# jamesmshihua/DiffusionPolicyOptimization

Measured on NVIDIA B200. Metric: ppo_logprob_update_samples_per_sec, higher is better.
Workload: dtype bf16x3

## Files before the change

diffusionpolicyoptimization_b200/csrc/common.cuh:

```cuda
#pragma once
#include <cuda_runtime.h>
#include <cuda_bf16.h>
#include <stdint.h>
#include <stdio.h>
#include <string.h>
#include <math.h>
#include <string>
#include <vector>
#include "../../include/dppo_b200.h"

void dppo_set_error(const char* fmt, ...);
#define DPPO_FAIL(code, ...) do { dppo_set_error(__VA_ARGS__); return (code); } while (0)
#define CUDA_TRY(expr) do { cudaError_t _e = (expr); if (_e != cudaSuccess) { \
    dppo_set_error("%s failed at %s:%d: %s", #expr, __FILE__, __LINE__, cudaGetErrorString(_e)); return -2; } } while (0)
#define DPPO_TRY(expr) do { int _r = (expr); if (_r != 0) return _r; } while (0)

enum { SCH_BETAS = 0, SCH_ACP, SCH_SQRT_ACP, SCH_SQRT_1M_ACP, SCH_SQRT_RECIP, SCH_SQRT_RECIPM1,
       SCH_LOGVAR, SCH_COEF1, SCH_COEF2, SCH_ROWS };

static inline int round_up(int x, int m) { return (x + m - 1) / m * m; }

__device__ __forceinline__ float softplus_f(float x) {
    return fmaxf(x, 0.f) + log1pf(expf(-fabsf(x)));
}
// ... 36 lines not shown
    c.x = (uint32_t)(a >> 2) | ((uint32_t)slot << 8);
    c.y = (uint32_t)offset;
    c.z = (uint32_t)(uint64_t)row;
    c.w = (uint32_t)((uint64_t)row >> 32);
    Philox4 r = philox4x32_10(c, (uint32_t)seed, (uint32_t)(seed >> 32) + (uint32_t)(offset >> 32));
    uint32_t b0 = (a & 2) ? r.z : r.x, b1 = (a & 2) ? r.w : r.y;
    float u0 = ((float)b0 + 0.5f) * 2.3283064365386963e-10f;
    float u1 = ((float)b1 + 0.5f) * 2.3283064365386963e-10f;
    u0 = fminf(fmaxf(u0, 1.1754944e-38f), 0.99999994f);
    float rad = sqrtf(-2.f * logf(u0));
    float sn, cs;
    sincospif(2.f * u1, &sn, &cs);
    return (a & 1) ? rad * sn : rad * cs;
}
__device__ __forceinline__ void philox_normal4(uint64_t seed, uint64_t offset, int64_t row, int slot, int blk, float (&out)[4]) {
    Philox4 c;
    c.x = (uint32_t)blk | ((uint32_t)slot << 8);
    c.y = (uint32_t)offset;
    c.z = (uint32_t)(uint64_t)row;
    c.w = (uint32_t)((uint64_t)row >> 32);
    Philox4 r = philox4x32_10(c, (uint32_t)seed, (uint32_t)(seed >> 32) + (uint32_t)(offset >> 32));
#pragma unroll
    for (int hlf = 0; hlf < 2; ++hlf) {
        const uint32_t b0 = hlf ? r.z : r.x, b1 = hlf ? r.w : r.y;
        float u0 = ((float)b0 + 0.5f) * 2.3283064365386963e-10f;
        float u1 = ((float)b1 + 0.5f) * 2.3283064365386963e-10f;
        u0 = fminf(fmaxf(u0, 1.1754944e-38f), 0.99999994f);
        float rad = sqrtf(-2.f * logf(u0));
        float sn, cs;
        sincospif(2.f * u1, &sn, &cs);
        out[hlf * 2 + 0] = rad * cs; out[hlf * 2 + 1] = rad * sn;
    }
}
__device__ __forceinline__ uint32_t philox_uint(uint64_t seed, uint64_t offset, int64_t row, int slot) {
    Philox4 c;
    c.x = ((uint32_t)slot << 8);
    c.y = (uint32_t)offset;
    c.z = (uint32_t)(uint64_t)row;
    c.w = (uint32_t)((uint64_t)row >> 32);
    Philox4 r = philox4x32_10(c, (uint32_t)seed, (uint32_t)(seed >> 32) + (uint32_t)(offset >> 32));
    return r.x;
}

struct ActorOff {
    size_t tw1, tb1, tw2, tb2, win, bin, w1, b1, w2, b2, w3, b3, n;
};
struct CriticOff { size_t win, bin, w1, b1, w2, b2, w3, b3, n; };

struct Geom {
    int Do, A, T, K, td, H, Hc, Din, KP, KPc;
    ActorOff ao; CriticOff co;
};

struct ActorDerived {
    float* sinemb;
    float* thpre;
    float* temb;
    float* bt;
    float* w0p;
    float* w23;
    float* b23;
};

struct OptState { float* m; float* v; int64_t step; size_t n; };

struct Workspace {
    char* base = nullptr; size_t cap = 0, used = 0;
};

struct dppo_handle {
    dppo_cfg cfg; int device; Geom g;
    int sm_count;
    float* params;
    float* net_w[4];
    size_t net_n[4];
    ActorDerived ad[4];
    float* sched;
    float  sched_host[SCH_ROWS * 1024];
    OptState opt[2];
    float* grads;
    float* scalars;
    Workspace ws;
    char* pin = nullptr; size_t pin_cap = 0;
    char* dstage = nullptr; size_t dstage_cap = 0;
    cudaStream_t copy_stream = nullptr; cudaEvent_t copy_ev[9];
    void* comm = nullptr; int rank = 0, world = 1;
    float* grads_buf[2] = {nullptr, nullptr}; int grads_cur = 0; float* gsum = nullptr; size_t grads_floats = 0;
    unsigned long long* flags = nullptr;
    float* peer_grads[2][8] = {}; unsigned long long* peer_flags[8] = {}; int peers_attached = 0;
    unsigned long long epoch = 0;
    int* comm_status = nullptr;
    long long peer_timeout_cycles = 0;
    const int* skip_update = nullptr;
    int64_t launches = 0;
    int64_t tc_launches = 0;
    int w0p_dirty[4] = {1, 1, 1, 1};
    int w23_dirty[4] = {1, 1, 1, 1};
    int peer_two_shot = -1;
    float* peer_gsum[8] = {nullptr};
    cudaStream_t aux_stream = nullptr; cudaEvent_t aux_ev[3] = {nullptr, nullptr, nullptr};
    float grad_clip_norm = 0.f;
    int deterministic = 0;
    int chain_dbg_idx = 0;
    long long* chain_dbg = nullptr;
    int64_t fused_launches = 0;
    int cluster_max = -1;
    int last_path = 0;
    int force_path = 0;
    struct TcState* tc = nullptr;
    float* env_norm = nullptr;
    struct TsState* ts = nullptr;
// ... 19 lines not shown
```

diffusionpolicyoptimization_b200/csrc/dppo_api.cu:

```cuda
#include "common.cuh"
#include "simt_kernels.cuh"
#include "sample_cluster.cuh"
#include "tc_path.cuh"
#include "ts_path.cuh"
#include <stdarg.h>
#include <dlfcn.h>
#include <cmath>

static thread_local char g_err[1024] = "";
void dppo_set_error(const char* fmt, ...) {
    va_list ap; va_start(ap, fmt); vsnprintf(g_err, sizeof(g_err), fmt, ap); va_end(ap);
}
extern "C" const char* dppo_last_error(void) { return g_err; }
extern "C" int dppo_abi_version(void) { return DPPO_ABI_VERSION; }
extern "C" size_t dppo_cfg_size(void) { return sizeof(dppo_cfg); }

#define KLAUNCH(h) do { (h)->launches++; } while (0)
#define KCHECK() do { cudaError_t _e = cudaGetLastError(); if (_e != cudaSuccess) { \
    dppo_set_error("kernel launch failed at %s:%d: %s", __FILE__, __LINE__, cudaGetErrorString(_e)); return -3; } } while (0)

extern "C" void dppo_cfg_default(dppo_cfg* c) {
    memset(c, 0, sizeof(*c));
    c->obs_dim = 11; c->action_dim = 3; c->horizon_steps = 4; c->cond_steps = 1;
    c->denoising_steps = 20; c->ft_denoising_steps = 10; c->time_dim = 16;
// ... 194 lines not shown
    h->w0p_dirty[net] = 1; h->w23_dirty[net] = 1;
    if (net != DPPO_NET_CRITIC) {
        ActorDerived& d = h->ad[net];
        int threads = g.H < 64 ? 64 : (g.H > 512 ? 512 : round_up(g.H, 32));
        if (threads < 2 * g.td) threads = round_up(2 * g.td, 32);
        actor_prep_kernel<<<g.T, threads, 4 * g.td * sizeof(float), s>>>(h->net_w[net], g.ao, g.A, g.td, g.H, d.sinemb, d.thpre, d.temb, d.bt);
        KLAUNCH(h); KCHECK();
    }
    if (h->cfg.precision == DPPO_PREC_FP32) DPPO_TRY(ensure_w0p(h, net, s));
    DPPO_TRY(ts_refresh_net(h, net, s));
    return tc_refresh_net(h, net, s);
}

static int dppo_create_impl(const dppo_cfg* cfg, int device, dppo_handle** out, dppo_handle** partial);
extern "C" int dppo_create(const dppo_cfg* cfg, int device, dppo_handle** out) {
    if (!cfg || !out) DPPO_FAIL(-1, "dppo_create: null argument");
    dppo_handle* partial = nullptr;
    const int r = dppo_create_impl(cfg, device, out, &partial);
    if (r != 0 && partial) { std::string msg = dppo_last_error(); dppo_destroy(partial); dppo_set_error("%s", msg.c_str()); }
    return r;
}
static int dppo_create_impl(const dppo_cfg* cfg, int device, dppo_handle** out, dppo_handle** partial) {
    Geom g;
    if (make_geom(cfg, &g)) DPPO_FAIL(-1, "dppo_create: invalid configuration");
    int ndev = 0;
    cudaError_t e = cudaGetDeviceCount(&ndev);
    if (e != cudaSuccess || ndev == 0) DPPO_FAIL(-4, "dppo_create: no CUDA device (%s); this library has no CPU fallback", cudaGetErrorString(e));
    if (device < 0 || device >= ndev) DPPO_FAIL(-1, "dppo_create: device %d out of range (%d devices)", device, ndev);
    CUDA_TRY(cudaSetDevice(device));
    cudaDeviceProp prop; CUDA_TRY(cudaGetDeviceProperties(&prop, device));
    if (prop.major != 10) DPPO_FAIL(-4, "dppo_create: device %d is sm_%d%d; this library is built for sm_100a (B200) only", device, prop.major, prop.minor);
    dppo_handle* h = new dppo_handle();
    *partial = h;
    h->cfg = *cfg; h->device = device; h->g = g; h->sm_count = prop.multiProcessorCount;
    { const char* tv = getenv("DPPO_PEER_TIMEOUT_S"); double sec = tv ? atof(tv) : 600.0; if (!(sec > 0)) sec = 600.0;
      h->peer_timeout_cycles = (long long)(sec * 1e3 * (double)prop.clockRate); }
    { const char* dv = getenv("DPPO_DETERMINISTIC"); h->deterministic = (dv && dv[0] == '1') ? 1 : 0; }
    const size_t nA = g.ao.n, nC = g.co.n;
    const size_t total = 3 * nA + nC;
    CUDA_TRY(cudaMalloc(&h->params, total * sizeof(float)));
    CUDA_TRY(cudaMemset(h->params, 0, total * sizeof(float)));
    h->net_w[DPPO_NET_ACTOR] = h->params; h->net_n[DPPO_NET_ACTOR] = nA;
    h->net_w[DPPO_NET_ACTOR_FT] = h->params + nA; h->net_n[DPPO_NET_ACTOR_FT] = nA;
    h->net_w[DPPO_NET_CRITIC] = h->params + 2 * nA; h->net_n[DPPO_NET_CRITIC] = nC;
    h->net_w[DPPO_NET_ACTOR_EMA] = h->params + 2 * nA + nC; h->net_n[DPPO_NET_ACTOR_EMA] = nA;
    for (int net = 0; net < 4; ++net) {
        ActorDerived& d = h->ad[net];
        memset(&d, 0, sizeof(d));
        if (net == DPPO_NET_CRITIC) { CUDA_TRY(cudaMalloc(&d.w0p, (size_t)g.KPc * g.Hc * sizeof(float))); continue; }
        CUDA_TRY(cudaMalloc(&d.sinemb, (size_t)g.T * g.td * sizeof(float)));
        CUDA_TRY(cudaMalloc(&d.thpre, (size_t)g.T * 2 * g.td * sizeof(float)));
        CUDA_TRY(cudaMalloc(&d.temb, (size_t)g.T * g.td * sizeof(float)));
        CUDA_TRY(cudaMalloc(&d.bt, (size_t)g.T * g.H * sizeof(float)));
        CUDA_TRY(cudaMalloc(&d.w23, (size_t)g.H * g.A * sizeof(float))); CUDA_TRY(cudaMalloc(&d.b23, (size_t)g.A * sizeof(float)));
        CUDA_TRY(cudaMalloc(&d.w0p, (size_t)g.KP * g.H * sizeof(float)));
    }
    DPPO_TRY(dppo_ddpm_schedule(g.T, h->sched_host));
    CUDA_TRY(cudaMalloc(&h->sched, SCH_ROWS * g.T * sizeof(float)));
    CUDA_TRY(cudaMemcpy(h->sched, h->sched_host, SCH_ROWS * g.T * sizeof(float), cudaMemcpyHostToDevice));
    size_t on[2] = {nA, nA + nC};
    for (int i = 0; i < 2; ++i) {
        h->opt[i].n = on[i]; h->opt[i].step = 0;
        CUDA_TRY(cudaMalloc(&h->opt[i].m, on[i] * sizeof(float))); CUDA_TRY(cudaMemset(h->opt[i].m, 0, on[i] * sizeof(float)));
        CUDA_TRY(cudaMalloc(&h->opt[i].v, on[i] * sizeof(float))); CUDA_TRY(cudaMemset(h->opt[i].v, 0, on[i] * sizeof(float)));
    }
    CUDA_TRY(cudaMalloc(&h->grads, (nA + nC + 16) * sizeof(float)));
    CUDA_TRY(cudaMemset(h->grads, 0, (nA + nC + 16) * sizeof(float)));
    h->grads_buf[0] = h->grads; h->grads_floats = nA + nC + 16;
    CUDA_TRY(cudaMalloc(&h->scalars, 64 * sizeof(float)));
    CUDA_TRY(cudaMemset(h->scalars, 0, 64 * sizeof(float)));
    h->comm_status = reinterpret_cast<int*>(h->scalars + 32);
    DPPO_TRY(tc_init(h));
    DPPO_TRY(ts_init(h));
    for (int net = 0; net < 4; ++net) DPPO_TRY(prep_net(h, net, 0));
    CUDA_TRY(cudaDeviceSynchronize());
    *out = h; *partial = nullptr;
    return 0;
}
extern "C" void dppo_destroy(dppo_handle* h) {
    if (!h) return;
    cudaSetDevice(h->device);
    cudaDeviceSynchronize();
    tc_plan_free(h);
    tc_destroy(h);
    ts_destroy(h);
    for (cudaEvent_t e : h->prof_ev) cudaEventDestroy(e);
    if (h->comm) {
        void* lib = dlopen("libnccl.so.2", RTLD_NOW | RTLD_NOLOAD);
        if (lib) { typedef int (*fn_t)(void*); fn_t f = (fn_t)dlsym(lib, "ncclCommDestroy"); if (f) f(h->comm); }
    }
    if (h->peers_attached) {
        for (int p = 0; p < h->world; ++p) if (p != h->rank) {
            cudaIpcCloseMemHandle(h->peer_grads[0][p]); cudaIpcCloseMemHandle(h->peer_grads[1][p]); cudaIpcCloseMemHandle(h->peer_flags[p]);
        }
    }
    cudaFree(h->env_norm);
    cudaFree(h->params); cudaFree(h->sched); cudaFree(h->grads_buf[0]); cudaFree(h->grads_buf[1]);  cudaFree(h->flags); cudaFree(h->scalars);
    for (int i = 0; i < 2; ++i) { cudaFree(h->opt[i].m); cudaFree(h->opt[i].v); }
    for (int net = 0; net < 4; ++net) { ActorDerived& d = h->ad[net]; cudaFree(d.sinemb); cudaFree(d.thpre); cudaFree(d.temb); cudaFree(d.bt); cudaFree(d.w0p); cudaFree(d.w23); cudaFree(d.b23); }
    if (h->ws.base) cudaFree(h->ws.base);
    if (h->copy_stream) { cudaStreamDestroy(h->copy_stream); for (int i = 0; i < 9; ++i) cudaEventDestroy(h->copy_ev[i]); }
    if (h->aux_stream) { cudaStreamDestroy(h->aux_stream); for (int i = 0; i < 3; ++i) if (h->aux_ev[i]) cudaEventDestroy(h->aux_ev[i]); }
    if (h->pin) cudaFreeHost(h->pin);
    if (h->dstage) cudaFree(h->dstage);
    delete h;
}

#define ENTER(h) do { if (!(h)) DPPO_FAIL(-1, "null handle"); CUDA_TRY(cudaSetDevice((h)->device)); } while (0)

extern "C" int dppo_set_weights(dppo_handle* h, int net, const float* src, size_t n, int is_device, dppo_stream_t st) {
    ENTER(h); cudaStream_t s = (cudaStream_t)st;
    if (net < 0 || net > 3 || !src) DPPO_FAIL(-1, "dppo_set_weights: bad net %d", net);
    if (n != h->net_n[net]) DPPO_FAIL(-1, "dppo_set_weights: net %d has %zu parameters, got %zu", net, h->net_n[net], n);
    CUDA_TRY(cudaMemcpyAsync(h->net_w[net], src, n * sizeof(float), is_device ? cudaMemcpyDeviceToDevice : cudaMemcpyHostToDevice, s));
    if (!is_device) CUDA_TRY(cudaStreamSynchronize(s));
    return prep_net(h, net, s);
}
extern "C" int dppo_get_weights(dppo_handle* h, int net, float* dst, size_t n, int is_device, dppo_stream_t st) {
    ENTER(h); cudaStream_t s = (cudaStream_t)st;
    if (net < 0 || net > 3 || !dst) DPPO_FAIL(-1, "dppo_get_weights: bad net %d", net);
    if (n != h->net_n[net]) DPPO_FAIL(-1, "dppo_get_weights: net %d has %zu parameters, got %zu", net, h->net_n[net], n);
    CUDA_TRY(cudaMemcpyAsync(dst, h->net_w[net], n * sizeof(float), is_device ? cudaMemcpyDeviceToDevice : cudaMemcpyDeviceToHost, s));
    if (!is_device) CUDA_TRY(cudaStreamSynchronize(s));
    return 0;
}
extern "C" int dppo_set_opt_state(dppo_handle* h, int opt, const float* m, const float* v, size_t n, int64_t step, int is_device, dppo_stream_t st) {
    ENTER(h); cudaStream_t s = (cudaStream_t)st;
    if (opt < 0 || opt > 1 || n != h->opt[opt].n) DPPO_FAIL(-1, "dppo_set_opt_state: bad slot/size");
    cudaMemcpyKind k = is_device ? cudaMemcpyDeviceToDevice : cudaMemcpyHostToDevice;
    if (m) CUDA_TRY(cudaMemcpyAsync(h->opt[opt].m, m, n * sizeof(float), k, s));
    if (v) CUDA_TRY(cudaMemcpyAsync(h->opt[opt].v, v, n * sizeof(float), k, s));
    h->opt[opt].step = step;
    if (!is_device) CUDA_TRY(cudaStreamSynchronize(s));
    return 0;
}
extern "C" int dppo_get_opt_state(dppo_handle* h, int opt, float* m, float* v, size_t n, int64_t* step, int is_device, dppo_stream_t st) {
    ENTER(h); cudaStream_t s = (cudaStream_t)st;
    if (opt < 0 || opt > 1 || n != h->opt[opt].n) DPPO_FAIL(-1, "dppo_get_opt_state: bad slot/size");
    cudaMemcpyKind k = is_device ? cudaMemcpyDeviceToDevice : cudaMemcpyDeviceToHost;
    if (m) CUDA_TRY(cudaMemcpyAsync(m, h->opt[opt].m, n * sizeof(float), k, s));
    if (v) CUDA_TRY(cudaMemcpyAsync(v, h->opt[opt].v, n * sizeof(float), k, s));
    if (step) *step = h->opt[opt].step;
    if (!is_device) CUDA_TRY(cudaStreamSynchronize(s));
    return 0;
}
extern "C" int dppo_set_ft_denoising_steps(dppo_handle* h, int K) {
    if (!h) DPPO_FAIL(-1, "null handle");
    if (K < 0 || K > h->g.T) DPPO_FAIL(-1, "dppo_set_ft_denoising_steps: K=%d outside [0,%d]", K, h->g.T);
    h->g.K = K; h->cfg.ft_denoising_steps = K;
    return 0;
}
extern "C" int dppo_set_grad_clip_norm(dppo_handle* h, float clip_norm) {
// ... 63 lines not shown
    int rpb = (N + nb - 1) / nb; nb = (N + rpb - 1) / rpb;
    size_t sm = (size_t)nseg * ncols * sizeof(float);
    if (sm > 48 * 1024) {
        if (sm > 200 * 1024) DPPO_FAIL(-1, "colsum: %d segments x %d columns does not fit in shared memory", nseg, ncols);
        CUDA_TRY(cudaFuncSetAttribute(colsum_kernel, cudaFuncAttributeMaxDynamicSharedMemorySize, (int)sm));
    }
    colsum_kernel<<<nb, 256, sm, s>>>(D, ld, N, ncols, seg, nseg, rpb, part); KLAUNCH(h); KCHECK();
    size_t n = (size_t)nseg * ncols;
    tc_reduce_cols_kernel<<<nblk(n, 8), 256, 0, s>>>(part, nb, n, (int)n, out); KLAUNCH(h); KCHECK();
    return 0;
}
static int gemm_dw(dppo_handle* h, cudaStream_t s, const float* X, int ldx, int aop, const float* D, int ldd,
                   int rows, int M, int N, float* part, float* out) {
    int tiles = ((M + 127) / 128) * ((N + (N <= 32 ? 31 : 127)) / (N <= 32 ? 32 : 128));
    int splits = (2 * h->sm_count + tiles - 1) / tiles;
    if (splits > 40) splits = 40;
    int maxs = (rows + 255) / 256; if (splits > maxs) splits = maxs; if (splits < 1) splits = 1;
    GemmP p = gp(X, ldx, D, ldd, part, N, M, N, rows); p.aop = aop; p.cstride = (size_t)M * N;
    int S = gemm(h, s, true, false, p, splits);
    if (S < 0) return -3;
    size_t n = (size_t)M * N;
    reduce_partials_kernel<<<nblk(n, 256), 256, 0, s>>>(part, S, n, n, out, 1.f); KLAUNCH(h); KCHECK();
    return 0;
}
static int mlp_bwd_fp32(dppo_handle* h, cudaStream_t s, const float* w, size_t ow1, size_t ob1, size_t ow2, size_t ob2,
                        size_t ow3, size_t ob3, int act1, const FwdBufs& f, const float* dout, int N, int KP, int H, int NO,
                        const int* seg, int nseg, BwdBufs& b, float* gnet, float* dw0p, float* Gseg) {
    GemmP p = gp(dout, NO, w + ow3, NO, b.dv, H, N, H, NO);
    DPPO_TRY(gemm(h, s, false, true, p) < 0 ? -3 : 0);
    p = gp(b.dv, H, w + ow2, H, b.dh1, H, N, H, H); p.mask = f.h1; p.ldm = H; p.mask_act = act1;
    DPPO_TRY(gemm(h, s, false, true, p) < 0 ? -3 : 0);
    p = gp(b.dh1, H, w + ow1, H, b.du, H, N, H, H); p.mask = f.u; p.ldm = H; p.mask_act = act1; p.add = b.dv; p.ldadd = H;
    DPPO_TRY(gemm(h, s, false, true, p) < 0 ? -3 : 0);
    DPPO_TRY(gemm_dw(h, s, f.v, H, 0, dout, NO, N, H, NO, b.part, gnet + ow3));
    DPPO_TRY(gemm_dw(h, s, f.h1, H, act1, b.dv, H, N, H, H, b.part, gnet + ow2));
    DPPO_TRY(gemm_dw(h, s, f.u, H, act1, b.dh1, H, N, H, H, b.part, gnet + ow1));
    DPPO_TRY(gemm_dw(h, s, f.h0p, KP, 0, b.du, H, N, KP, H, b.part, dw0p));
    DPPO_TRY(colsum(h, s, dout, NO, N, NO, nullptr, 1, b.part, gnet + ob3));
    DPPO_TRY(colsum(h, s, b.dv, H, N, H, nullptr, 1, b.part, gnet + ob2));
    DPPO_TRY(colsum(h, s, b.dh1, H, N, H, nullptr, 1, b.part, gnet + ob1));
    DPPO_TRY(colsum(h, s, b.du, H, N, H, seg, nseg, b.part, Gseg));
    return 0;
}
static void bwd_take(dppo_handle* h, int N, int KP, int H, int nseg, BwdBufs& b, float** Gseg, float** dw0p) {
    b.dv = ws_take<float>(h, (size_t)N * H); b.dh1 = ws_take<float>(h, (size_t)N * H); b.du = ws_take<float>(h, (size_t)N * H);
    size_t colpart = (size_t)320 * (size_t)nseg * H, gemm_part = (size_t)40 * (size_t)H * H;
    b.part_floats = colpart > gemm_part ? colpart : gemm_part;
    b.part = ws_take<float>(h, b.part_floats);
    *Gseg = ws_take<float>(h, (size_t)nseg * H);
    *dw0p = ws_take<float>(h, (size_t)KP * H);
}
static int actor_bwd_fp32(dppo_handle* h, cudaStream_t s, int net, const FwdBufs& f, const float* deps, int N, const int* trow,
                          BwdBufs& b, float* Gseg, float* dw0p, float* gnet) {
    const Geom& g = h->g; const float* w = h->net_w[net]; const ActorDerived& d = h->ad[net];
    DPPO_TRY(mlp_bwd_fp32(h, s, w, g.ao.w1, g.ao.b1, g.ao.w2, g.ao.b2, g.ao.w3, g.ao.b3, h->cfg.actor_act + 1, f, deps, N,
                          g.KP, g.H, g.A, trow, g.T, b, gnet, dw0p, Gseg));
    size_t sm = (size_t)(g.T * g.td * 3) * sizeof(float);
    time_backward_kernel<<<1, 512, sm, s>>>(w, g.ao, g.A, g.td, g.H, g.T, Gseg, d.sinemb, d.thpre, d.temb, gnet); KLAUNCH(h); KCHECK();
    unpack_dw0_kernel<<<nblk((size_t)(g.A + g.Do) * g.H, 256), 256, 0, s>>>(dw0p, g.A, g.td, g.Do, g.H, gnet + g.ao.win); KLAUNCH(h); KCHECK();
    return 0;
}
static int critic_bwd_fp32(dppo_handle* h, cudaStream_t s, const FwdBufs& f, const float* dval, int N,
                           BwdBufs& b, float* Gseg, float* dw0p, float* gnet) {
    const Geom& g = h->g; const float* w = h->net_w[DPPO_NET_CRITIC];
    DPPO_TRY(mlp_bwd_fp32(h, s, w, g.co.w1, g.co.b1, g.co.w2, g.co.b2, g.co.w3, g.co.b3, h->cfg.critic_act + 1, f, dval, N,
                          g.KPc, g.Hc, 1, nullptr, 1, b, gnet, dw0p, Gseg));
    CUDA_TRY(cudaMemcpyAsync(gnet + g.co.bin, Gseg, g.Hc * sizeof(float), cudaMemcpyDeviceToDevice, s));
    unpack_dw0_kernel<<<nblk((size_t)g.Do * g.Hc, 256), 256, 0, s>>>(dw0p, 0, 0, g.Do, g.Hc, gnet + g.co.win); KLAUNCH(h); KCHECK();
    return 0;
}

static const int ROW_CHUNK = 1 << 18;

extern "C" int dppo_actor_forward(dppo_handle* h, int net, const float* x, const int32_t* t, const float* obs,
                                  int N, float* eps, dppo_stream_t st) {
    ENTER(h); cudaStream_t s = (cudaStream_t)st; const Geom& g = h->g;
    if (net < 0 || net > 3 || net == DPPO_NET_CRITIC || !x || !t || !obs || !eps || N < 0) DPPO_FAIL(-1, "dppo_actor_forward: bad arguments");
    for (int r0 = 0; r0 < N; r0 += ROW_CHUNK) {
        int n = N - r0 < ROW_CHUNK ? N - r0 : ROW_CHUNK;
        if (tc_eligible(h, n)) {
            DPPO_TRY(ws_reserve(h, tc_actor_forward_ws(h, n), s));
            DPPO_TRY(tc_actor_forward(h, s, net, x + (size_t)r0 * g.A, obs + (size_t)r0 * g.Do, 1, n, t + r0, 0, eps + (size_t)r0 * g.A));
            continue;
        }
        if (ts_eligible(h, n)) {
            DPPO_TRY(ws_reserve(h, ts_actor_forward_ws(h, n), s));
            DPPO_TRY(ts_actor_forward(h, s, net, x + (size_t)r0 * g.A, obs + (size_t)r0 * g.Do, 1, n, t + r0, 0, eps + (size_t)r0 * g.A));
            continue;
        }
        DPPO_TRY(ws_reserve(h, fwd_ws_bytes(n, g.KP, g.H, g.A), s));
        FwdBufs b; fwd_take(h, n, g.KP, g.H, g.A, b);
        DPPO_TRY(actor_fwd_fp32(h, s, net, x + (size_t)r0 * g.A, obs + (size_t)r0 * g.Do, 1, n, t + r0, 0, b));
        CUDA_TRY(cudaMemcpyAsync(eps + (size_t)r0 * g.A, b.out, (size_t)n * g.A * sizeof(float), cudaMemcpyDeviceToDevice, s));
    }
    return 0;
}
extern "C" int dppo_value(dppo_handle* h, const float* obs, int N, float* v, dppo_stream_t st) {
    ENTER(h); cudaStream_t s = (cudaStream_t)st; const Geom& g = h->g;
    if (!obs || !v || N < 0) DPPO_FAIL(-1, "dppo_value: bad arguments");
    for (int r0 = 0; r0 < N; r0 += ROW_CHUNK) {
        int n = N - r0 < ROW_CHUNK ? N - r0 : ROW_CHUNK;
        if (tc_eligible(h, n)) { DPPO_TRY(tc_value(h, s, obs + (size_t)r0 * g.Do, n, v + r0)); continue; }
        if (ts_eligible(h, n)) { DPPO_TRY(ts_value(h, s, obs + (size_t)r0 * g.Do, n, v + r0)); continue; }
        DPPO_TRY(ws_reserve(h, fwd_ws_bytes(n, g.KPc, g.Hc, 1), s));
        FwdBufs b; fwd_take(h, n, g.KPc, g.Hc, 1, b);
        DPPO_TRY(critic_fwd_fp32(h, s, obs + (size_t)r0 * g.Do, n, b));
        CUDA_TRY(cudaMemcpyAsync(v + r0, b.out, (size_t)n * sizeof(float), cudaMemcpyDeviceToDevice, s));
    }
    return 0;
}

// ... 330 lines not shown
            if (e != cudaSuccess) DPPO_FAIL(-6, "cudaIpcOpenMemHandle(rank %d, buffer %d) failed: %s", p, k, cudaGetErrorString(e));
        }
        h->peer_grads[0][p] = (float*)ptr[0]; h->peer_grads[1][p] = (float*)ptr[1]; h->peer_flags[p] = (unsigned long long*)ptr[2];
        h->peer_gsum[p] = (float*)ptr[1] + gf4;
    }
    h->rank = rank; h->world = world; h->peers_attached = 1;
    if (h->peer_two_shot < 0) { const char* tv = getenv("DPPO_PEER_TWO_SHOT"); h->peer_two_shot = tv ? (tv[0] == '1') : (world >= 4); }
    return 0;
}
static int peer_allreduce_adamw(dppo_handle* h, cudaStream_t s, int opt, float* w, size_t n_param, size_t n_total, float lr, float wd) {
    OptState& o = h->opt[opt];
    o.step += 1;
    const float b1 = h->cfg.adam_beta1, b2 = h->cfg.adam_beta2;
    const float b1p = powf(b1, (float)o.step), b2p = powf(b2, (float)o.step);
    const float alpha = lr * sqrtf(1.f - b2p) / (1.f - b1p);
    PeerPtrs pp; memset(&pp, 0, sizeof(pp));
    for (int p = 0; p < h->world; ++p) { pp.g[p] = h->peer_grads[h->grads_cur][p]; pp.flags[p] = h->peer_flags[p]; }
    h->epoch += 1;
    peer_barrier_kernel<<<1, 32, 0, s>>>(pp, h->flags, h->rank, h->world, h->epoch, h->peer_timeout_cycles, h->comm_status); KLAUNCH(h); KCHECK();
    if (h->peer_two_shot == 1) {
        PeerSums ps; memset(&ps, 0, sizeof(ps));
        for (int p = 0; p < h->world; ++p) ps.s[p] = h->peer_gsum[p];
        const size_t n4 = (n_total + 3) / 4, per = (n4 + h->world - 1) / h->world;
        int grid = (int)((per + 255) / 256); if (grid > 2 * h->sm_count) grid = 2 * h->sm_count; if (grid < 1) grid = 1;
        peer_reduce_scatter_bcast_kernel<<<grid, 256, 0, s>>>(pp, ps, h->rank, h->world, n4, h->comm_status); KLAUNCH(h); KCHECK();
        h->epoch += 1;
        peer_barrier_kernel<<<1, 32, 0, s>>>(pp, h->flags, h->rank, h->world, h->epoch, h->peer_timeout_cycles, h->comm_status); KLAUNCH(h); KCHECK();
        adamw_kernel<<<nblk(n_param, 256), 256, 0, s>>>(w, h->gsum, o.m, o.v, n_param, lr, alpha, b1, b2, h->cfg.adam_eps, wd, h->skip_update, h->comm_status); KLAUNCH(h); KCHECK();
    } else {
        peer_allreduce_adamw_kernel<<<2 * h->sm_count, 256, 0, s>>>(pp, h->world, h->gsum, w, o.m, o.v, n_param, n_total, lr, alpha, b1, b2, h->cfg.adam_eps, wd,
                                                                  h->skip_update, h->comm_status);
        KLAUNCH(h); KCHECK();
    }
    h->grads_cur ^= 1; h->grads = h->grads_buf[h->grads_cur];
    return 0;
}
static int allreduce_sum(dppo_handle* h, float* buf, size_t n, cudaStream_t s) {
    if (h->world <= 1) return 0;
    if (!h->comm || !g_allreduce) DPPO_FAIL(-6, "all-reduce requested but no communicator attached");
    int r = g_allreduce(buf, buf, n, 7 , 0 , h->comm, s);
    if (r) DPPO_FAIL(-6, "ncclAllReduce failed (%d)", r);
    return 0;
}

extern "C" int dppo_comm_status(dppo_handle* h) {
    ENTER(h);
    int st = 0;
    CUDA_TRY(cudaDeviceSynchronize());
    CUDA_TRY(cudaMemcpy(&st, h->comm_status, sizeof(int), cudaMemcpyDeviceToHost));
    if (st) DPPO_FAIL(-6, "peer-memory gradient exchange: a flag barrier timed out; weights and optimizer state were left untouched since");
    return 0;
}

static int adam_apply(dppo_handle* h, cudaStream_t s, int opt, float* w, const float* g, size_t n, float lr, float wd) {
    OptState& o = h->opt[opt];
    o.step += 1;
    const float b1 = h->cfg.adam_beta1, b2 = h->cfg.adam_beta2;
    float b1p = powf(b1, (float)o.step), b2p = powf(b2, (float)o.step);
    float alpha = lr * sqrtf(1.f - b2p) / (1.f - b1p);
    adamw_kernel<<<nblk(n, 256), 256, 0, s>>>(w, g, o.m, o.v, n, lr, alpha, b1, b2, h->cfg.adam_eps, wd, h->skip_update, nullptr); KLAUNCH(h); KCHECK();
    return 0;
}

static int prep_net(dppo_handle* h, int net, cudaStream_t s);
static int ppo_apply_tail(dppo_handle* h, cudaStream_t s, float lr, int apply, float* metrics8, float* grads_out) {
    const size_t nA = h->g.ao.n, nC = h->g.co.n; float* gr = h->grads;
    if (apply) {
        if (h->grad_clip_norm > 0.f) {
            DPPO_TRY(allreduce_sum(h, gr, nA + nC + 8, s));
            if (grads_out) { CUDA_TRY(cudaMemcpyAsync(grads_out, gr, (nA + nC) * sizeof(float), cudaMemcpyDeviceToDevice, s)); grads_out = nullptr; }
            const ActorOff& a = h->g.ao; const CriticOff& c = h->g.co;
            const size_t offs[21] = {a.tw1, a.tb1, a.tw2, a.tb2, a.win, a.bin, a.w1, a.b1, a.w2, a.b2, a.w3, a.b3,
                                     nA + c.win, nA + c.bin, nA + c.w1, nA + c.b1, nA + c.w2, nA + c.b2, nA + c.w3, nA + c.b3, nA + nC};
            VarSegs segs; segs.n = 20;
            for (int i = 0; i <= 20; ++i) segs.off[i] = (unsigned int)offs[i];
            clip_by_norm_kernel<<<segs.n, 1024, 0, s>>>(gr, segs, h->grad_clip_norm); KLAUNCH(h); KCHECK();
            DPPO_TRY(adam_apply(h, s, DPPO_OPT_FINETUNE, h->net_w[DPPO_NET_ACTOR_FT], gr, nA + nC, lr, h->cfg.weight_decay));
        } else if (h->peers_attached && h->world > 1) {
            DPPO_TRY(peer_allreduce_adamw(h, s, DPPO_OPT_FINETUNE, h->net_w[DPPO_NET_ACTOR_FT], nA + nC, nA + nC + 8, lr, h->cfg.weight_decay));
            gr = h->gsum;
        } else {
            DPPO_TRY(allreduce_sum(h, gr, nA + nC + 8, s));
            DPPO_TRY(adam_apply(h, s, DPPO_OPT_FINETUNE, h->net_w[DPPO_NET_ACTOR_FT], gr, nA + nC, lr, h->cfg.weight_decay));
        }
        if (h->cfg.precision == DPPO_PREC_BF16 && tc_shapes_ok(h) && 2 * h->g.td <= 256) {
            DPPO_TRY(tc_prep_pack_ft_critic(h, s));
        } else {
            DPPO_TRY(prep_net(h, DPPO_NET_ACTOR_FT, s));
            DPPO_TRY(prep_net(h, DPPO_NET_CRITIC, s));
        }
    }
    else if (h->world > 1) {
        DPPO_TRY(allreduce_sum(h, gr, nA + nC + 8, s));
    }
    if (metrics8) CUDA_TRY(cudaMemcpyAsync(metrics8, gr + nA + nC, 8 * sizeof(float), cudaMemcpyDeviceToDevice, s));
    if (grads_out) CUDA_TRY(cudaMemcpyAsync(grads_out, gr, (nA + nC) * sizeof(float), cudaMemcpyDeviceToDevice, s));
    return 0;
}
extern "C" int dppo_ppo_step(dppo_handle* h, const float* obs, const float* prev, const float* nxt,
                             const int32_t* inds, const float* returns, const float* oldvalues,
                             const float* advantages, const float* oldlogp, int N, int64_t N_global,
                             float adv_mean, float adv_std, float lr, int apply,
                             float* metrics8, float* grads_out, dppo_stream_t st) {
    ENTER(h); cudaStream_t s = (cudaStream_t)st; const Geom& g = h->g;
    if (!obs || !prev || !nxt || !inds || !returns || !oldvalues || !advantages || !oldlogp || N < 1 || N_global < N)
        DPPO_FAIL(-1, "dppo_ppo_step: bad arguments");
    if (g.K < 1) DPPO_FAIL(-1, "dppo_ppo_step: ft_denoising_steps must be >= 1");
    if (adv_std < 0.f && N_global != N) DPPO_FAIL(-1, "dppo_ppo_step: global advantage statistics are required when rows are sharded");
    const size_t nA = g.ao.n, nC = g.co.n;
    float* gr = h->grads;
    if (tc_eligible(h, N)) {
        DPPO_TRY(tc_ppo_step(h, s, obs, prev, nxt, inds, returns, oldvalues, advantages, oldlogp, N, N_global, adv_mean, adv_std));
    } else if (ts_eligible(h, N)) {
        DPPO_TRY(ts_ppo_step(h, s, obs, prev, nxt, inds, returns, oldvalues, advantages, oldlogp, N, N_global, adv_mean, adv_std));
    } else {
        const int nlb = nblk(N, 128);
        size_t need = fwd_ws_bytes(N, g.KP, g.H, g.A) + fwd_ws_bytes(N, g.KPc, g.Hc, 1)
                    + bwd_ws_bytes(h, N, g.KP, g.H, g.A, g.T) + bwd_ws_bytes(h, N, g.KPc, g.Hc, 1, 1)
                    + ws_bytes(N, 4) + ws_bytes((size_t)N * g.A, 4) + ws_bytes(N, 4) + ws_bytes((size_t)nlb * 5, 8);
        DPPO_TRY(ws_reserve(h, need, s));
        FwdBufs fa, fc; fwd_take(h, N, g.KP, g.H, g.A, fa); fwd_take(h, N, g.KPc, g.Hc, 1, fc);
        BwdBufs ba, bc; float *Ga, *Gc, *dw0a, *dw0c;
        bwd_take(h, N, g.KP, g.H, g.T, ba, &Ga, &dw0a); bwd_take(h, N, g.KPc, g.Hc, 1, bc, &Gc, &dw0c);
        int* trow = ws_take<int>(h, N);
        float* deps = ws_take<float>(h, (size_t)N * g.A);
        float* dval = ws_take<float>(h, N);
        double* bsum = ws_take<double>(h, (size_t)nlb * 5);

        make_trow_kernel<<<nblk(N, 256), 256, 0, s>>>(inds, N, g.K, 0, trow); KLAUNCH(h); KCHECK();
        if (adv_std < 0.f) { adv_stats_kernel<<<1, 1024, 0, s>>>(advantages, N, h->scalars); KLAUNCH(h); KCHECK(); }
        else { set_scalars_kernel<<<1, 1, 0, s>>>(h->scalars, adv_mean, adv_std); KLAUNCH(h); KCHECK(); }
        DPPO_TRY(actor_fwd_fp32(h, s, DPPO_NET_ACTOR_FT, prev, obs, 1, N, trow, 0, fa));
        DPPO_TRY(critic_fwd_fp32(h, s, obs, N, fc));
        PpoHyper hp;
        hp.A = g.A; hp.Da = h->cfg.action_dim; hp.K = g.K; hp.T = g.T; hp.reward_horizon = h->cfg.reward_horizon; hp.norm_adv = h->cfg.norm_adv;
        hp.dcv = h->cfg.denoised_clip_value; hp.min_lp_std = h->cfg.min_logprob_denoising_std;
        hp.lp_lo = h->cfg.logprob_clip_lo; hp.lp_hi = h->cfg.logprob_clip_hi; hp.gamma_d = h->cfg.gamma_denoising;
        hp.clip_coef = h->cfg.clip_ploss_coef; hp.clip_base = h->cfg.clip_ploss_coef_base; hp.clip_rate = h->cfg.clip_ploss_coef_rate;
// ... 347 lines not shown
```

diffusionpolicyoptimization_b200/csrc/simt_kernels.cuh:

```cuda
#pragma once
#include "common.cuh"

struct GemmP {
    const float* A; int lda;
    const float* B; int ldb;
    float* C; int ldc;
    int M, N, K;
    int kchunk; size_t cstride;
    int vecA, vecB, vecC;
    int aop;
    const float* bias;
    const float* btab; int ldbt;
    const int* trow; int tconst;
    const float* mask; int ldm; int mask_act;
    const float* add; int ldadd;
};

template <bool A_KM, bool B_NK, int BN>
__global__ void __launch_bounds__(256, 2) sgemm_kernel(const GemmP p) {
    constexpr int BM = 128, BK = 16, TN = BN / 16;
    __shared__ __align__(16) float As[2][BK][BM + 4];
    __shared__ __align__(16) float Bs[2][BK][BN + 4];

    const int tid = threadIdx.x, tx = tid & 15, ty = tid >> 4;
// ... 141 lines not shown
            }
#pragma unroll
            for (int i = 0; i < 8; ++i)
#pragma unroll
                for (int j = 0; j < TN; ++j) acc[i][j] = fmaf(a[i], b[j], acc[i][j]);
        }
        if (kt + 1 < nk) { store_a(buf ^ 1); store_b(buf ^ 1); }
        __syncthreads();
    }

#pragma unroll
    for (int i = 0; i < 8; ++i) {
        const int m = m0 + (i < 4 ? ty * 4 + i : 64 + ty * 4 + (i - 4));
        if (m >= p.M) continue;
        const float* btrow = nullptr;
        if (p.btab) { int t = p.trow ? p.trow[m] : p.tconst; btrow = p.btab + (size_t)t * p.ldbt; }
#pragma unroll
        for (int jb = 0; jb < TN; jb += (TN == 8 ? 4 : 2)) {
            constexpr int W = (TN == 8 ? 4 : 2);
            const int n = n0 + (TN == 8 ? (jb < 4 ? tx * 4 : 64 + tx * 4) : tx * 2);
            float v[W];
#pragma unroll
            for (int e = 0; e < W; ++e) {
                float x = acc[i][jb + e];
                int nn = n + e;
                if (nn < p.N) {
                    if (p.bias) x += p.bias[nn];
                    if (btrow) x += btrow[nn];
                    if (p.mask) x *= act_grad_rt(p.mask[(size_t)m * p.ldm + nn], p.mask_act);
                    if (p.add) x += p.add[(size_t)m * p.ldadd + nn];
                }
                v[e] = x;
            }
            float* dst = C + (size_t)m * p.ldc + n;
            if (W == 4 && p.vecC && n + 3 < p.N) {
                *reinterpret_cast<float4*>(dst) = make_float4(v[0], v[1], v[2], v[3]);
            } else {
#pragma unroll
                for (int e = 0; e < W; ++e) if (n + e < p.N) dst[e] = v[e];
            }
        }
    }
}

__global__ void reduce_partials_kernel(const float* __restrict__ part, int S, size_t stride, size_t n,
                                       float* __restrict__ out, float scale) {
    size_t i = (size_t)blockIdx.x * blockDim.x + threadIdx.x;
    if (i >= n) return;
    float s = 0.f;
    for (int k = 0; k < S; ++k) s += part[(size_t)k * stride + i];
    out[i] = s * scale;
}

__device__ __forceinline__ void actor_prep_body(const int t, float* sm, const float* __restrict__ w, ActorOff o, int A, int td, int H,
                                  float* __restrict__ sinemb, float* __restrict__ thpre,
                                  float* __restrict__ temb, float* __restrict__ bt, __nv_bfloat16* __restrict__ bt16) {
    float* se = sm;
    float* hp = se + td;
    float* te = hp + 2 * td;
    const int tid = threadIdx.x;
    const int half = td / 2;
    if (tid < td) {
        int i = tid % half;
        float f = expf((float)i * -(logf(10000.f) / (float)(half - 1)));
        float e = (float)t * f;
        float v = tid < half ? sinf(e) : cosf(e);
        se[tid] = v; sinemb[t * td + tid] = v;
    }
    __syncthreads();
    if (tid < 2 * td) {
        float s = w[o.tb1 + tid];
        for (int j = 0; j < td; ++j) s = fmaf(se[j], w[o.tw1 + (size_t)j * 2 * td + tid], s);
        thpre[t * 2 * td + tid] = s;
        hp[tid] = mish_f(s);
    }
    __syncthreads();
    if (tid < td) {
        float s = w[o.tb2 + tid];
        for (int j = 0; j < 2 * td; ++j) s = fmaf(hp[j], w[o.tw2 + (size_t)j * td + tid], s);
        te[tid] = s; temb[t * td + tid] = s;
    }
    __syncthreads();
    for (int c = tid; c < H; c += blockDim.x) {
        float s = w[o.bin + c];
        for (int j = 0; j < td; ++j) s = fmaf(te[j], w[o.win + (size_t)(A + j) * H + c], s);
        bt[(size_t)t * H + c] = s;
        if (bt16) bt16[(size_t)t * H + c] = __float2bfloat16(s);
    }
}
__global__ void actor_prep_kernel(const float* __restrict__ w, ActorOff o, int A, int td, int H,
                                  float* __restrict__ sinemb, float* __restrict__ thpre,
                                  float* __restrict__ temb, float* __restrict__ bt) {
    extern __shared__ float sm[];
    actor_prep_body(blockIdx.x, sm, w, o, A, td, H, sinemb, thpre, temb, bt, nullptr);
}
__global__ void fold_output_kernel(const float* __restrict__ w2, const float* __restrict__ b2, const float* __restrict__ w3, const float* __restrict__ b3,
                                   int H, int A, float* __restrict__ w23, float* __restrict__ b23) {
    const int i = blockIdx.x * blockDim.x + threadIdx.x;
    if (i >= (H + 1) * A) return;
    const int k = i / A, a = i % A;
    const float* row = k < H ? w2 + (size_t)k * H : b2;
    double acc = k < H ? 0.0 : (double)b3[a];
    for (int j = 0; j < H; ++j) acc += (double)row[j] * (double)w3[(size_t)j * A + a];
    if (k < H) w23[(size_t)k * A + a] = (float)acc; else b23[a] = (float)acc;
}
__global__ void pack_w0_kernel(const float* __restrict__ win, int A, int skip, int Do, int KP, int H,
                               float* __restrict__ w0p) {
    int i = blockIdx.x * blockDim.x + threadIdx.x;
    if (i >= KP * H) return;
    int k = i / H, c = i % H;
    float v = 0.f;
    if (k < A) v = win[(size_t)k * H + c];
    else if (k < A + Do) v = win[(size_t)(k + skip) * H + c];
    w0p[i] = v;
}
__global__ void pack_h0_kernel(const float* __restrict__ x, const float* __restrict__ obs, int N, int A, int Do,
                               int KP, int obs_div, float* __restrict__ h0p) {
    size_t i = (size_t)blockIdx.x * blockDim.x + threadIdx.x;
    if (i >= (size_t)N * KP) return;
    int r = (int)(i / KP), k = (int)(i % KP);
    float v = 0.f;
    if (k < A) v = x[(size_t)r * A + k];
    else if (k < A + Do) v = obs[(size_t)(r / obs_div) * Do + (k - A)];
    h0p[i] = v;
}
__global__ void make_trow_kernel(const int* __restrict__ inds, int N, int K, int mode, int* __restrict__ trow) {
    int r = blockIdx.x * blockDim.x + threadIdx.x;
    if (r >= N) return;
    trow[r] = mode == 0 ? (K - 1 - inds[r]) : (K - 1 - (r % K));
}

struct SampleHyper {
    float dcv, rcv, facv, min_std; int deterministic;
};
struct StepConst { float sr, srm1, c1, c2, sd; };
__device__ __forceinline__ StepConst step_const(const float* __restrict__ sch, int T, int t) {
    StepConst c;
    c.sr = sch[SCH_SQRT_RECIP * T + t]; c.srm1 = sch[SCH_SQRT_RECIPM1 * T + t];
    c.c1 = sch[SCH_COEF1 * T + t]; c.c2 = sch[SCH_COEF2 * T + t];
    c.sd = expf(0.5f * sch[SCH_LOGVAR * T + t]);
    return c;
}
__device__ __forceinline__ float sample_std(const StepConst& c, int t, const SampleHyper& hp) {
    if (hp.deterministic) return (t == 0) ? 0.f : fminf(fmaxf(c.sd, 1e-3f), 1e6f);
    return fminf(fmaxf(c.sd, hp.min_std), 1e6f);
}
__device__ __forceinline__ float ddpm_step_elem_c(float x, float eps, float noise, const StepConst& c, float sd, const SampleHyper& hp, bool last) {
// ... 236 lines not shown
    }
}

__global__ void pretrain_prep_kernel(const float* __restrict__ x0, const int* __restrict__ t_in, const float* __restrict__ noise_in,
                                     int N, int A, int T, const float* __restrict__ sch, uint64_t seed, uint64_t offset,
                                     int64_t row_offset, int* __restrict__ trow, float* __restrict__ noise, float* __restrict__ xn) {
    size_t i = (size_t)blockIdx.x * blockDim.x + threadIdx.x;
    if (i >= (size_t)N * A) return;
    int r = (int)(i / A), a = (int)(i % A);
    int t = t_in ? t_in[r] : (int)(((uint64_t)philox_uint(seed, offset, row_offset + r, 255) * (uint64_t)T) >> 32);
    float nz = noise_in ? noise_in[i] : philox_normal(seed, offset, row_offset + r, 0, a);
    if (a == 0) trow[r] = t;
    noise[i] = nz;
    xn[i] = sch[SCH_SQRT_ACP * T + t] * x0[i] + sch[SCH_SQRT_1M_ACP * T + t] * nz;
}
__global__ void __launch_bounds__(256) mse_loss_kernel(const float* __restrict__ eps, const float* __restrict__ noise, size_t n,
                                                       float scale, float* __restrict__ deps, double* __restrict__ block_sums) {
    size_t i = (size_t)blockIdx.x * blockDim.x + threadIdx.x;
    double a = 0;
    if (i < n) { float d = eps[i] - noise[i]; deps[i] = 2.f * d * scale; a = (double)d * d; }
    __shared__ double red[256];
    red[threadIdx.x] = a;
    __syncthreads();
    for (int o = 128; o > 0; o >>= 1) { if (threadIdx.x < o) red[threadIdx.x] += red[threadIdx.x + o]; __syncthreads(); }
    if (threadIdx.x == 0) block_sums[blockIdx.x] = red[0];
}
__global__ void sum_blocks_kernel(const double* __restrict__ block_sums, int nblocks, float scale, float* __restrict__ dst) {
    __shared__ double red[256];
    double a = 0;
    for (int b = threadIdx.x; b < nblocks; b += blockDim.x) a += block_sums[b];
    red[threadIdx.x] = a;
    __syncthreads();
    for (int o = 128; o > 0; o >>= 1) { if (threadIdx.x < o) red[threadIdx.x] += red[threadIdx.x + o]; __syncthreads(); }
    if (threadIdx.x == 0) dst[0] = (float)(red[0] * scale);
}

__global__ void __launch_bounds__(256) colsum_kernel(const float* __restrict__ D, int ld, int N, int ncols,
                                                     const int* __restrict__ seg, int nseg, int rows_per_block,
                                                     float* __restrict__ part) {
    extern __shared__ float sm[];
    for (int i = threadIdx.x; i < nseg * ncols; i += blockDim.x) sm[i] = 0.f;
    __syncthreads();
    const int r0 = blockIdx.x * rows_per_block, r1 = min(N, r0 + rows_per_block);
    for (int c = threadIdx.x; c < ncols; c += blockDim.x) {
        for (int r = r0; r < r1; ++r) {
            int s = seg ? seg[r] : 0;
            sm[s * ncols + c] += D[(size_t)r * ld + c];
        }
    }
    __syncthreads();
    for (int i = threadIdx.x; i < nseg * ncols; i += blockDim.x) part[(size_t)blockIdx.x * nseg * ncols + i] = sm[i];
}

__device__ __forceinline__ void time_backward_body(const int bid, const int nblk, float* sm, const bool staged,
                                     const float* __restrict__ w, ActorOff o, int A, int td, int H, int T,
                                     const float* __restrict__ G, const float* __restrict__ sinemb,
                                     const float* __restrict__ thpre, const float* __restrict__ temb,
                                     float* __restrict__ g) {
    float* dte = sm;
    float* dh = dte + T * td;
    const int tid = threadIdx.x, nt = blockDim.x;
    if (nblk == 1 || bid > 0) {
        const int c0 = nblk == 1 ? 0 : (bid - 1) * 128, c1 = nblk == 1 ? H : min(H, c0 + 128);
        const int lanes = nblk == 1 ? 1 : 4;
        for (int i = tid; i < (c1 - c0) * lanes; i += nt) {
            const int c = c0 + i / lanes, part = i % lanes;
            float bsum = 0.f;
            float acc[16];
#pragma unroll
            for (int q = 0; q < 16; ++q) acc[q] = 0.f;
            for (int t0 = 0; t0 < T; t0 += 32) {
                float gc[32];
#pragma unroll
                for (int q = 0; q < 32; ++q) gc[q] = (t0 + q < T) ? G[(size_t)(t0 + q) * H + c] : 0.f;
#pragma unroll
                for (int q = 0; q < 32; ++q) bsum += gc[q];
#pragma unroll
                for (int jj = 0; jj < 16; ++jj) {
                    const int j = part + jj * lanes;
                    if (j < td) {
#pragma unroll
                        for (int q = 0; q < 32; ++q) if (t0 + q < T) acc[jj] = fmaf(temb[(t0 + q) * td + j], gc[q], acc[jj]);
                    }
                }
            }
            if (part == 0) g[o.bin + c] = bsum;
            for (int jj = 0; jj < 16; ++jj) {
                const int j = part + jj * lanes;
                if (j < td) g[o.win + (size_t)(A + j) * H + c] = acc[jj];
            }
            for (int j = part + 16 * lanes; j < td; j += lanes) {
                float a = 0.f;
                for (int t = 0; t < T; ++t) a = fmaf(temb[t * td + j], G[(size_t)t * H + c], a);
                g[o.win + (size_t)(A + j) * H + c] = a;
            }
        }
        if (nblk > 1) return;
    }
    if (staged) {
        float* sG = dh + T * 2 * td;
        float* sW = sG + T * H;
        for (int i = tid; i < T * H; i += nt) sG[i] = G[i];
        for (int i = tid; i < td * H; i += nt) sW[i] = w[o.win + (size_t)A * H + i];
        __syncthreads();
        const int lane = tid & 31;
        for (int p = tid >> 5; p < T * td; p += nt >> 5) {
            const int t = p / td, j = p % td;
            float s = 0.f;
            for (int c = lane; c < H; c += 32) s = fmaf(sW[j * H + c], sG[t * H + c], s);
#pragma unroll
            for (int off = 16; off > 0; off >>= 1) s += __shfl_xor_sync(0xffffffffu, s, off);
            if (lane == 0) dte[t * td + j] = s;
        }
    } else
    for (int j = tid >> 5; j < td; j += nt >> 5) {
        const int lane = tid & 31;
        float wr[32];
#pragma unroll
        for (int q = 0; q < 32; ++q) { const int c = lane + q * 32; wr[q] = c < H ? w[o.win + (size_t)(A + j) * H + c] : 0.f; }
        for (int t = 0; t < T; ++t) {
            float s = 0.f;
#pragma unroll
            for (int q = 0; q < 32; ++q) { const int c = lane + q * 32; if (c < H) s = fmaf(wr[q], G[(size_t)t * H + c], s); }
#pragma unroll
            for (int off = 16; off > 0; off >>= 1) s += __shfl_xor_sync(0xffffffffu, s, off);
            if (lane == 0) dte[t * td + j] = s;
        }
    }
    __syncthreads();
    for (int i = tid; i < T * 2 * td; i += nt) {
        int t = i / (2 * td), k = i % (2 * td);
        float s = 0.f;
        for (int j = 0; j < td; ++j) s = fmaf(w[o.tw2 + (size_t)k * td + j], dte[t * td + j], s);
        dh[i] = s * mish_grad_f(thpre[i]);
    }
    __syncthreads();
    for (int i = tid; i < 2 * td * td; i += nt) {
        int k = i / td, j = i % td;
        float s = 0.f;
        for (int t = 0; t < T; ++t) s = fmaf(mish_f(thpre[t * 2 * td + k]), dte[t * td + j], s);
        g[o.tw2 + i] = s;
        int ss = i / (2 * td), kk = i % (2 * td);
        float a = 0.f;
        for (int t = 0; t < T; ++t) a = fmaf(sinemb[t * td + ss], dh[t * 2 * td + kk], a);
        g[o.tw1 + i] = a;
    }
    for (int j = tid; j < td; j += nt) { float s = 0.f; for (int t = 0; t < T; ++t) s += dte[t * td + j]; g[o.tb2 + j] = s; }
    for (int k = tid; k < 2 * td; k += nt) { float s = 0.f; for (int t = 0; t < T; ++t) s += dh[t * 2 * td + k]; g[o.tb1 + k] = s; }
}
__global__ void __launch_bounds__(512) time_backward_kernel(const float* __restrict__ w, ActorOff o, int A, int td, int H, int T,
                                     const float* __restrict__ G, const float* __restrict__ sinemb,
                                     const float* __restrict__ thpre, const float* __restrict__ temb,
                                     float* __restrict__ g) {
    extern __shared__ float sm[];
    time_backward_body(blockIdx.x, gridDim.x, sm, false, w, o, A, td, H, T, G, sinemb, thpre, temb, g);
}
__device__ __forceinline__ void unpack_dw0_body(const int bid, const float* __restrict__ dw0p, int A, int skip, int Do, int H, float* __restrict__ gwin) {
    int i = bid * blockDim.x + threadIdx.x;
    if (i >= (A + Do) * H) return;
    int k = i / H, c = i % H;
    gwin[(size_t)(k < A ? k : k + skip) * H + c] = dw0p[i];
}
__global__ void unpack_dw0_kernel(const float* __restrict__ dw0p, int A, int skip, int Do, int H, float* __restrict__ gwin) {
    unpack_dw0_body(blockIdx.x, dw0p, A, skip, Do, H, gwin);
}

__global__ void adamw_kernel(float* __restrict__ w, const float* __restrict__ g, float* __restrict__ m, float* __restrict__ v,
                             size_t n, float lr, float alpha, float b1, float b2, float eps, float wd,
                             const int* __restrict__ skip0 = nullptr, const int* __restrict__ skip1 = nullptr) {
    size_t i = (size_t)blockIdx.x * blockDim.x + threadIdx.x;
    if (i >= n) return;
    if ((skip0 && *skip0) || (skip1 && *skip1)) return;
    float p = w[i], gi = g[i], mi = m[i], vi = v[i];
    if (wd != 0.f) p = p - p * (wd * lr);
    mi = mi + (gi - mi) * (1.f - b1);
    vi = vi + (gi * gi - vi) * (1.f - b2);
    p = p - mi * alpha / (sqrtf(vi) + eps);
    w[i] = p; m[i] = mi; v[i] = vi;
}
struct VarSegs { unsigned int off[24]; int n; };
__global__ void __launch_bounds__(1024) clip_by_norm_kernel(float* __restrict__ g, VarSegs segs, float clip) {
    const unsigned int b = segs.off[blockIdx.x], e = segs.off[blockIdx.x + 1];
    float acc = 0.f;
    for (unsigned int i = b + threadIdx.x; i < e; i += blockDim.x) { const float x = g[i]; acc = fmaf(x, x, acc); }
    __shared__ float part[32];
    __shared__ float denom;
    for (int o = 16; o; o >>= 1) acc += __shfl_xor_sync(0xffffffffu, acc, o);
    if ((threadIdx.x & 31) == 0) part[threadIdx.x >> 5] = acc;
    __syncthreads();
    if (threadIdx.x < 32) {
        float t = threadIdx.x < (blockDim.x >> 5) ? part[threadIdx.x] : 0.f;
        for (int o = 16; o; o >>= 1) t += __shfl_xor_sync(0xffffffffu, t, o);
        if (threadIdx.x == 0) denom = fmaxf(sqrtf(t > 0.f ? t : 1.f), clip);
    }
    __syncthreads();
    const float d = denom;
    if (d == clip) return;
    for (unsigned int i = b + threadIdx.x; i < e; i += blockDim.x) g[i] = g[i] * clip / d;
}
struct PeerPtrs { const float* g[8]; unsigned long long* flags[8]; };
__global__ void peer_barrier_kernel(PeerPtrs pp, unsigned long long* my_flags, int rank, int world, unsigned long long epoch,
                                    long long timeout_cycles, int* __restrict__ status) {
    const int p = threadIdx.x;
    if (p >= world) return;
    if (*((volatile int*)status)) return;
    __threadfence_system();
    *((volatile unsigned long long*)(pp.flags[p] + rank)) = epoch;
    const long long t0 = clock64();
    while (*((volatile unsigned long long*)(my_flags + p)) < epoch) {
        if (clock64() - t0 > timeout_cycles) {
            printf("peer barrier timed out: rank %d waiting for rank %d (epoch %llu)\n", rank, p, epoch);
            atomicExch(status, 1);
            break;
        }
        __nanosleep(64);
    }
    __threadfence_system();
}
__global__ void __launch_bounds__(256) peer_allreduce_adamw_kernel(PeerPtrs pp, int world, float* __restrict__ g_sum, float* __restrict__ w,
                                                                  float* __restrict__ m, float* __restrict__ v, size_t n_param, size_t n_total,
                                                                  float lr, float alpha, float b1, float b2, float eps, float wd,
                                                                  const int* __restrict__ skip0 = nullptr, const int* __restrict__ skip1 = nullptr) {
    const bool no_update = (skip0 && *skip0) || (skip1 && *skip1);
    if (skip1 && *skip1) return;
    const size_t n4 = n_total / 4;
    for (size_t i = (size_t)blockIdx.x * blockDim.x + threadIdx.x; i < n4 + (n_total & 3); i += (size_t)gridDim.x * blockDim.x) {
        float s[4] = {0.f, 0.f, 0.f, 0.f};
        const bool vec = i < n4;
        const size_t e0 = vec ? i * 4 : n4 * 4 + (i - n4);
        const int cnt = vec ? 4 : 1;
// ... 36 lines not shown
```

diffusionpolicyoptimization_b200/csrc/tc_path.cuh:

```cuda
#pragma once
#include "common.cuh"
#include "simt_kernels.cuh"
#include "tc_gemm.cuh"
#include "fused_chain.cuh"
#include "tc_dw_pair.cuh"

typedef __nv_bfloat16 bf16;

struct TcNetW {
    bf16 *w2w0, *w1, *w3t, *w3p;
    bf16 *w1t, *w2t;
    float* bias2;
    int H;
};
struct TcPpoPlan;
struct TcState {
    TcNetW net[4];
    int KP0;
    TcPpoPlan* plan;
};

__device__ __forceinline__ void tc_pack_actor_body(const size_t i0, const size_t stride, const float* __restrict__ w, ActorOff o, int A, int td, int Do, int T, int H, int KP0,
                                     const float* __restrict__ bt, bf16* __restrict__ w2w0, bf16* __restrict__ w1,
                                     bf16* __restrict__ w3t, bf16* __restrict__ w3p, bf16* __restrict__ w1t, bf16* __restrict__ w2t) {
// ... 6 lines not shown
        int k = (int)(i / H), c = (int)(i % H);
        float v = 0.f;
        if (k < A) v = w[o.win + (size_t)k * H + c];
        else if (k < A + Do) v = w[o.win + (size_t)(k + td) * H + c];
        else if (k < A + Do + T) { if (!bt) continue; v = bt[(size_t)(k - A - Do) * H + c]; }
        w2w0[(size_t)H * H + i] = __float2bfloat16(v);
    }
    for (size_t i = i0; i < (size_t)64 * H; i += stride) {
        int a = (int)(i / H), k = (int)(i % H);
        w3t[i] = __float2bfloat16(a < A ? w[o.w3 + (size_t)k * A + a] : 0.f);
    }
    for (size_t i = i0; i < (size_t)H * 128; i += stride) {
        int k = (int)(i / 128), a = (int)(i % 128);
        w3p[i] = __float2bfloat16(a < A ? w[o.w3 + (size_t)k * A + a] : 0.f);
    }
}
__global__ void tc_pack_actor_kernel(const float* __restrict__ w, ActorOff o, int A, int td, int Do, int T, int H, int KP0,
                                     const float* __restrict__ bt, bf16* __restrict__ w2w0, bf16* __restrict__ w1,
                                     bf16* __restrict__ w3t, bf16* __restrict__ w3p, bf16* __restrict__ w1t, bf16* __restrict__ w2t) {
    tc_pack_actor_body((size_t)blockIdx.x * blockDim.x + threadIdx.x, (size_t)gridDim.x * blockDim.x, w, o, A, td, Do, T, H, KP0, bt, w2w0, w1, w3t, w3p, w1t, w2t);
}
__device__ __forceinline__ void tc_pack_critic_body(const size_t i0, const size_t stride, const float* __restrict__ w, CriticOff o, int A, int Do, int Hc, int KP0,
                                      bf16* __restrict__ w2w0, bf16* __restrict__ w1, bf16* __restrict__ w3t,
                                      bf16* __restrict__ w3p, float* __restrict__ bias2, bf16* __restrict__ w1t, bf16* __restrict__ w2t) {
    for (size_t i = i0; i < (size_t)Hc * Hc; i += stride) {
        w2w0[i] = __float2bfloat16(w[o.w2 + i]); w1[i] = __float2bfloat16(w[o.w1 + i]);
        const size_t r = i / Hc, c = i % Hc;
        w1t[i] = __float2bfloat16(w[o.w1 + c * Hc + r]); w2t[i] = __float2bfloat16(w[o.w2 + c * Hc + r]);
    }
    for (size_t i = i0; i < (size_t)KP0 * Hc; i += stride) {
        int k = (int)(i / Hc), c = (int)(i % Hc);
        float v = (k >= A && k < A + Do) ? w[o.win + (size_t)(k - A) * Hc + c] : 0.f;
        w2w0[(size_t)Hc * Hc + i] = __float2bfloat16(v);
    }
    for (size_t i = i0; i < (size_t)64 * Hc; i += stride) { int a = (int)(i / Hc), k = (int)(i % Hc); w3t[i] = __float2bfloat16(a == 0 ? w[o.w3 + k] : 0.f); }
    for (size_t i = i0; i < (size_t)Hc * 128; i += stride) { int k = (int)(i / 128), a = (int)(i % 128); w3p[i] = __float2bfloat16(a == 0 ? w[o.w3 + k] : 0.f); }
    for (size_t i = i0; i < (size_t)Hc; i += stride) bias2[i] = w[o.b2 + i] + w[o.bin + i];
}
__global__ void tc_pack_critic_kernel(const float* __restrict__ w, CriticOff o, int A, int Do, int Hc, int KP0,
                                      bf16* __restrict__ w2w0, bf16* __restrict__ w1, bf16* __restrict__ w3t,
                                      bf16* __restrict__ w3p, float* __restrict__ bias2, bf16* __restrict__ w1t, bf16* __restrict__ w2t) {
    tc_pack_critic_body((size_t)blockIdx.x * blockDim.x + threadIdx.x, (size_t)gridDim.x * blockDim.x, w, o, A, Do, Hc, KP0, w2w0, w1, w3t, w3p, bias2, w1t, w2t);
}
struct TcPrepPackArgs {
    const float* wa; ActorOff ao; const float* wc; CriticOff co; int A, td, Do, T, H, Hc, KP0, na, nc;
    float* sinemb; float* thpre; float* temb; float* bt;
    bf16 *a_w2w0, *a_w1, *a_w3t, *a_w3p, *a_w1t, *a_w2t;
    bf16 *c_w2w0, *c_w1, *c_w3t, *c_w3p, *c_w1t, *c_w2t; float* c_bias2;
};
__global__ void __launch_bounds__(256) tc_prep_pack_kernel(const TcPrepPackArgs a) {
    extern __shared__ float prep_sm[];
    const int b = blockIdx.x;
    if (b < a.T)
        actor_prep_body(b, prep_sm, a.wa, a.ao, a.A, a.td, a.H, a.sinemb, a.thpre, a.temb, a.bt, a.a_w2w0 + (size_t)a.H * a.H + (size_t)(a.A + a.Do) * a.H);
    else if (b < a.T + a.na)
        tc_pack_actor_body((size_t)(b - a.T) * blockDim.x + threadIdx.x, (size_t)a.na * blockDim.x, a.wa, a.ao, a.A, a.td, a.Do, a.T, a.H, a.KP0, nullptr,
                           a.a_w2w0, a.a_w1, a.a_w3t, a.a_w3p, a.a_w1t, a.a_w2t);
    else
        tc_pack_critic_body((size_t)(b - a.T - a.na) * blockDim.x + threadIdx.x, (size_t)a.nc * blockDim.x, a.wc, a.co, a.A, a.Do, a.Hc, a.KP0,
                            a.c_w2w0, a.c_w1, a.c_w3t, a.c_w3p, a.c_bias2, a.c_w1t, a.c_w2t);
}
struct TcIdxView {
    const int* flat; int K; long long P;
    const float *chains, *obs, *olp, *ret, *val, *adv;
    int* bad;
};
__global__ void tc_pack_h0_kernel(const float* __restrict__ x, const float* __restrict__ obs, const int* __restrict__ trow, int tconst,
                                  int N, int A, int Do, int T, int KP0, int obs_div, bf16* __restrict__ h0, int chainK = 0,
                                  const int* __restrict__ flat = nullptr, int flatK = 1, long long flatP = 0, int* __restrict__ bad = nullptr) {
    const int g8 = KP0 / 8;
    size_t i = (size_t)blockIdx.x * blockDim.x + threadIdx.x;
    if (i >= (size_t)N * g8) return;
    const int r = (int)(i / g8), k0 = (int)(i % g8) * 8;
    int t = trow ? (tconst < 0 ? -tconst - 1 - trow[r] : trow[r]) : tconst;
    size_t xrow = chainK > 0 ? (size_t)(r / chainK) * (chainK + 1) + (r % chainK) : (size_t)r;
    size_t orow = (size_t)(r / obs_div);
    if (flat) {
        int f = flat[r];
        if (f < 0 || (long long)f >= flatP * flatK) { if (bad && k0 == 0) atomicOr(bad, 1); f = 0; }
        const int b = f / flatK, k = f % flatK;
        xrow = (size_t)b * (flatK + 1) + k; orow = (size_t)b; t = flatK - 1 - k;
    }
    __align__(16) bf16 o[8];
#pragma unroll
    for (int j = 0; j < 8; ++j) {
        const int k = k0 + j;
        float v = 0.f;
        if (k < A) v = x ? x[xrow * A + k] : 0.f;
        else if (k < A + Do) v = obs[orow * Do + (k - A)];
        else if (k < A + Do + T) v = (k - A - Do == t) ? 1.f : 0.f;
        else if (k == A + Do + T) v = 1.f;
        o[j] = __float2bfloat16(v);
    }
    *reinterpret_cast<uint4*>(h0 + (size_t)r * KP0 + k0) = *reinterpret_cast<const uint4*>(o);
}
__global__ void tc_pad64_kernel(const float* __restrict__ src, int N, int ncols, bf16* __restrict__ dst) {
    size_t i = (size_t)blockIdx.x * blockDim.x + threadIdx.x;
    if (i >= (size_t)N * 8) return;
    const int r = (int)(i >> 3), k0 = (int)(i & 7) * 8;
    __align__(16) bf16 o[8];
#pragma unroll
    for (int j = 0; j < 8; ++j) o[j] = __float2bfloat16(k0 + j < ncols ? src[(size_t)r * ncols + k0 + j] : 0.f);
    *reinterpret_cast<uint4*>(dst + (size_t)r * 64 + k0) = *reinterpret_cast<const uint4*>(o);
}
__global__ void __launch_bounds__(256) tc_colsum_kernel(const bf16* __restrict__ D, int N, int ncols, int rows_per_block, float* __restrict__ part) {
    __shared__ float2 red[256];
    const int tpr = ncols / 2, groups = 256 / tpr;
// ... 22 lines not shown
    if (i >= (size_t)rows * cols) return;
    const int r = (int)(i / cols), c = (int)(i % cols);
    float s = 0.f;
    for (int k = 0; k < S; ++k) s += part[(size_t)k * stride + (size_t)r * ld_in + c];
    out[(size_t)r * ld_out + c] = s;
}

__device__ __forceinline__ void tc_reduce_cols_body(const int bid, const float* __restrict__ part, int nb, size_t stride, int ncols,
                                                    float* __restrict__ out, int split, float* __restrict__ out2) {
    const int c = bid * (blockDim.x >> 5) + (threadIdx.x >> 5), lane = threadIdx.x & 31;
    if (c >= ncols) return;
    float s = 0.f;
    for (int b = lane; b < nb; b += 32) s += part[(size_t)b * stride + c];
#pragma unroll
    for (int o = 16; o > 0; o >>= 1) s += __shfl_xor_sync(0xffffffffu, s, o);
    if (lane == 0) { if (out2 && c >= split) out2[c - split] = s; else out[c] = s; }
}
__device__ __forceinline__ void tc_reduce_cols_wide_body(const int bid, const float* __restrict__ part, int nb, size_t stride, int ncols,
                                                         float* __restrict__ out, int split, float* __restrict__ out2) {
    __shared__ float red[16][33];
    const int lane = threadIdx.x & 31, rg = threadIdx.x >> 5, c = bid * 32 + lane;
    float sacc[8];
#pragma unroll
    for (int q = 0; q < 8; ++q) sacc[q] = 0.f;
    if (c < ncols) {
        int b = rg;
        for (; b + 112 < nb; b += 128) {
#pragma unroll
            for (int q = 0; q < 8; ++q) sacc[q] += part[(size_t)(b + 16 * q) * stride + c];
        }
        for (; b < nb; b += 16) sacc[0] += part[(size_t)b * stride + c];
    }
    red[rg][lane] = ((sacc[0] + sacc[1]) + (sacc[2] + sacc[3])) + ((sacc[4] + sacc[5]) + (sacc[6] + sacc[7]));
    __syncthreads();
    if (rg == 0 && c < ncols) {
        float s = 0.f;
#pragma unroll
        for (int g = 0; g < 16; ++g) s += red[g][lane];
        if (out2 && c >= split) out2[c - split] = s; else out[c] = s;
    }
}
__global__ void __launch_bounds__(256) tc_reduce_cols_kernel(const float* __restrict__ part, int nb, size_t stride, int ncols, float* __restrict__ out,
                                                             int split = 0, float* __restrict__ out2 = nullptr) {
    tc_reduce_cols_body(blockIdx.x, part, nb, stride, ncols, out, split, out2);
}

struct TcTailArgs {
    int first[9];
    const double* bsum; int blocks_done; float inv_nglobal, frac_local; float* metrics;
    int wide, wide3;
    const float* colb3; int ncol3; float* b3a; int split3; float* b3c;
    const float* cpa; int rows_a; int HA; float* b2a; float* b1a;
    const float* cpc; int rows_c; int HC; float* b2c; float* b1c;
    const float* w; ActorOff ao; int A, td, T, Do; int tb_staged; const float* Gt; const float* sinemb; const float* thpre; const float* temb; float* gr;
    const float* dw0a; float* gwin_a; const float* dw0c_obs; float* gwin_c; const float* dw0c_bias; float* gbin_c;
};
__global__ void __launch_bounds__(512) tc_ppo_tail_kernel(const TcTailArgs a) {
    extern __shared__ float tail_sm[];
    const int b = blockIdx.x;
    if (b < a.first[1]) ppo_metrics_body(a.bsum, a.blocks_done, a.inv_nglobal, a.frac_local, a.metrics);
    else if (b < a.first[2]) {
        if (a.wide3) tc_reduce_cols_wide_body(b - a.first[1], a.colb3, a.blocks_done, (size_t)a.ncol3, a.ncol3, a.b3a, a.split3, a.b3c);
        else tc_reduce_cols_body(b - a.first[1], a.colb3, a.blocks_done, (size_t)a.ncol3, a.ncol3, a.b3a, a.split3, a.b3c);
    }
    else if (b < a.first[3]) {
        if (a.wide) tc_reduce_cols_wide_body(b - a.first[2], a.cpa, a.rows_a, (size_t)2 * a.HA, 2 * a.HA, a.b2a, a.HA, a.b1a);
        else tc_reduce_cols_body(b - a.first[2], a.cpa, a.rows_a, (size_t)2 * a.HA, 2 * a.HA, a.b2a, a.HA, a.b1a);
    } else if (b < a.first[4]) {
        if (a.wide) tc_reduce_cols_wide_body(b - a.first[3], a.cpc, a.rows_c, (size_t)2 * a.HC, 2 * a.HC, a.b2c, a.HC, a.b1c);
        else tc_reduce_cols_body(b - a.first[3], a.cpc, a.rows_c, (size_t)2 * a.HC, 2 * a.HC, a.b2c, a.HC, a.b1c);
    }
    else if (b < a.first[5]) time_backward_body(b - a.first[4], a.first[5] - a.first[4], tail_sm, a.tb_staged != 0, a.w, a.ao, a.A, a.td, a.HA, a.T,
                                                a.Gt, a.sinemb, a.thpre, a.temb, a.gr);
    else if (b < a.first[6]) unpack_dw0_body(b - a.first[5], a.dw0a, a.A, a.td, a.Do, a.HA, a.gwin_a);
    else if (b < a.first[7]) unpack_dw0_body(b - a.first[6], a.dw0c_obs, 0, 0, a.Do, a.HC, a.gwin_c);
    else { const int i = (b - a.first[7]) * blockDim.x + threadIdx.x; if (i < a.HC) a.gbin_c[i] = a.dw0c_bias[i]; }
}

__global__ void __launch_bounds__(128) tc_ppo_loss_kernel(
    const float* __restrict__ prev, const float* __restrict__ nxt, const float* __restrict__ eps,
    const int* __restrict__ inds, const float* __restrict__ returns, const float* __restrict__ oldvalues,
    const float* __restrict__ advantages, const float* __restrict__ oldlogp, const float* __restrict__ newvalues,
    const float* __restrict__ advstats, const float* __restrict__ sch, PpoHyper hp, int N,
    bf16* __restrict__ depsb, bf16* __restrict__ dvalb, double* __restrict__ block_sums, float* __restrict__ col_part ) {
    const int r = blockIdx.x * blockDim.x + threadIdx.x;
    const int A = hp.A;
    double acc[5] = {0, 0, 0, 0, 0};
    float gout[32];
#pragma unroll
    for (int a = 0; a < 32; ++a) gout[a] = 0.f;
    float dv_out = 0.f;
    if (r < N) {
        const int ind = inds[r], t = hp.K - 1 - ind;
        const int nuse = min(hp.reward_horizon, A / hp.Da) * hp.Da;
        const StepConst sc = step_const(sch, hp.T, t);
        const float sd = logprob_std(sc, hp.min_lp_std);
        const float lgs = 0.91893853320467274f + logf(sd);
        float newm = 0.f, oldm = 0.f;
        float zs[32]; uint32_t live = 0u;
#pragma unroll
        for (int a = 0; a < 32; ++a) {
            zs[a] = 0.f;
            if (a < nuse) {
                const size_t i = (size_t)r * A + a;
                float z; bool in;
                const float lp = logprob_elem_c(prev[i], eps[i], nxt[i], sc, sd, lgs, hp.dcv, &z, &in);
                newm += fminf(fmaxf(lp, hp.lp_lo), hp.lp_hi);
                oldm += fminf(fmaxf(oldlogp[i], hp.lp_lo), hp.lp_hi);
                zs[a] = z;
                if (lp >= hp.lp_lo && lp <= hp.lp_hi && in) live |= 1u << a;
            }
        }
        newm /= (float)nuse; oldm /= (float)nuse;
        float adv = advantages[r];
        if (hp.norm_adv) adv = (adv - advstats[0]) / (advstats[1] + 1e-8f);
        adv *= powf(hp.gamma_d, (float)(hp.K - ind - 1));
        const float logratio = newm - oldm, ratio = expf(logratio);
        const float tt = hp.K > 1 ? (float)ind / (float)(hp.K - 1) : (float)ind;
        const float clipc = hp.K > 1 ? hp.clip_base + (hp.clip_coef - hp.clip_base) * (expf(hp.clip_rate * tt) - 1.f) / (expf(hp.clip_rate) - 1.f) : tt;
        const float rc = fminf(fmaxf(ratio, 1.f - clipc), 1.f + clipc);
        const float pg1 = -adv * ratio, pg2 = -adv * rc;
        const float pg = fmaxf(pg1, pg2);
        const float dpg = (pg1 >= pg2) ? -adv : ((ratio >= 1.f - clipc && ratio <= 1.f + clipc) ? -adv : 0.f);
        const float gscale = dpg * ratio * hp.inv_nglobal / (float)nuse / sd * sc.c1 * (-sc.srm1);
#pragma unroll
        for (int a = 0; a < 32; ++a) gout[a] = ((live >> a) & 1u) ? gscale * zs[a] : 0.f;
// ... 548 lines not shown
    m.W = &h->tc->net[DPPO_NET_CRITIC]; m.H = g.Hc; m.NO = 1; m.act1 = h->cfg.critic_act + 1; m.KP0 = h->tc->KP0;
    m.fused = fc_critic_ok(h) ? 1 : 0; m.net = DPPO_NET_CRITIC; m.din = g.Do; m.cpart = nullptr;
    m.b0 = w + g.co.bin; m.b1 = w + g.co.b1; m.b2 = m.W->bias2; m.b3 = w + g.co.b3;
}

static int tc_actor_forward(dppo_handle* h, cudaStream_t s, int net, const float* x, const float* obs, int obs_div, int N,
                            const int* trow, int tconst, float* eps) {
    const Geom& g = h->g; const int KP0 = h->tc->KP0;
    if (fc_ok(h)) {
        const size_t need = h->ws.used + ws_bytes((size_t)N * KP0, 2);
        if (need > h->ws.cap) DPPO_FAIL(-7, "tc_actor_forward: workspace too small (%zu > %zu)", need, h->ws.cap);
        const size_t mark = h->ws.used;
        bf16* h0 = ws_take<bf16>(h, (size_t)N * KP0);
        tc_pack_h0_kernel<<<tc_nblk((size_t)N * (KP0 / 8), 256), 256, 0, s>>>(x, obs, trow, tconst, N, g.A, g.Do, g.T, KP0, obs_div, h0);
        TC_KCHECK(h);
        int r = fc_actor_infer(h, s, net, h0, N, fc::FINAL_EPS, eps, nullptr, nullptr, nullptr, nullptr);
        h->ws.used = mark;
        return r;
    }
    const size_t need = h->ws.used + ws_bytes((size_t)N * KP0, 2) + tc_mlp_ws_bytes(N, g.H, h->cfg.actor_act == DPPO_ACT_MISH, false);
    if (need > h->ws.cap) DPPO_FAIL(-7, "tc_actor_forward: workspace too small (%zu > %zu)", need, h->ws.cap);
    const size_t mark = h->ws.used;
    TcMlp m; tc_actor_mlp(h, net, m);
    bf16* h0 = ws_take<bf16>(h, (size_t)N * KP0);
    tc_mlp_take(h, N, m, false);
    m.h0 = h0; m.out = eps;
    tc_pack_h0_kernel<<<tc_nblk((size_t)N * (KP0 / 8), 256), 256, 0, s>>>(x, obs, trow, tconst, N, g.A, g.Do, g.T, KP0, obs_div, h0);
    TC_KCHECK(h);
    int r = tc_mlp_forward(h, s, m, N);
    h->ws.used = mark;
    return r;
}
static size_t tc_actor_forward_ws(const dppo_handle* h, int N) {
    return ws_bytes((size_t)N * h->tc->KP0, 2) + tc_mlp_ws_bytes(N, h->g.H, h->cfg.actor_act == DPPO_ACT_MISH, false);
}
static int tc_value(dppo_handle* h, cudaStream_t s, const float* obs, int N, float* v) {
    const Geom& g = h->g; const int KP0 = h->tc->KP0;
    DPPO_TRY(ws_reserve(h, ws_bytes((size_t)N * KP0, 2) + tc_mlp_ws_bytes(N, g.Hc, h->cfg.critic_act == DPPO_ACT_MISH, false), s));
    TcMlp m; tc_critic_mlp(h, m);
    bf16* h0 = ws_take<bf16>(h, (size_t)N * KP0);
    tc_mlp_take(h, N, m, false);
    m.h0 = h0; m.out = v;
    tc_pack_h0_kernel<<<tc_nblk((size_t)N * (KP0 / 8), 256), 256, 0, s>>>(nullptr, obs, nullptr, -1, N, g.A, g.Do, g.T, KP0, 1, h0);
    TC_KCHECK(h);
    if (fc_critic_ok(h)) return fc_infer(h, s, fc_critic_net(h), h0, N, fc::FINAL_EPS, v, nullptr, nullptr, nullptr, nullptr);
    return tc_mlp_forward(h, s, m, N);
}

static int colsum(dppo_handle* h, cudaStream_t s, const float* D, int ld, int N, int ncols, const int* seg, int nseg,
                  float* part, float* out);

static int tc_actor_grads(dppo_handle* h, cudaStream_t s, int net, const TcMlp& m, const float* deps, const bf16* depsb, int N,
                          float* part, float* dw0, float* gnet) {
    const Geom& g = h->g; const float* w = h->net_w[net]; const ActorDerived& d = h->ad[net];
    DPPO_TRY(tc_mlp_backward(h, s, m, depsb, N, part, gnet, g.ao.w1, g.ao.b1, g.ao.w2, g.ao.b2, g.ao.w3, dw0));
    if (deps) DPPO_TRY(colsum(h, s, deps, g.A, N, g.A, nullptr, 1, part, gnet + g.ao.b3));
    const size_t sm = (size_t)(g.T * g.td * 3) * sizeof(float);
    time_backward_kernel<<<1, 512, sm, s>>>(w, g.ao, g.A, g.td, g.H, g.T, dw0 + (size_t)(g.A + g.Do) * g.H, d.sinemb, d.thpre, d.temb, gnet);
    TC_KCHECK(h);
    unpack_dw0_kernel<<<tc_nblk((size_t)(g.A + g.Do) * g.H, 256), 256, 0, s>>>(dw0, g.A, g.td, g.Do, g.H, gnet + g.ao.win);
    TC_KCHECK(h);
    return 0;
}
static int tc_critic_grads(dppo_handle* h, cudaStream_t s, const TcMlp& m, const float* dval, const bf16* dvalb, int N,
                           float* part, float* dw0, float* gnet) {
    const Geom& g = h->g;
    DPPO_TRY(tc_mlp_backward(h, s, m, dvalb, N, part, gnet, g.co.w1, g.co.b1, g.co.w2, g.co.b2, g.co.w3, dw0));
    if (dval) DPPO_TRY(colsum(h, s, dval, 1, N, 1, nullptr, 1, part, gnet + g.co.b3));
    unpack_dw0_kernel<<<tc_nblk((size_t)g.Do * g.Hc, 256), 256, 0, s>>>(dw0 + (size_t)g.A * g.Hc, 0, 0, g.Do, g.Hc, gnet + g.co.win);
    TC_KCHECK(h);
    CUDA_TRY(cudaMemcpyAsync(gnet + g.co.bin, dw0 + (size_t)(g.A + g.Do + g.T) * g.Hc, g.Hc * sizeof(float), cudaMemcpyDeviceToDevice, s));
    return 0;
}

struct TcPpoPlan {
    int N, nchunks, chunk_rows, lead_rows, blocks_done, max_blocks;
    int full_rows, rows_done, dw_done, dw_flush_chunk;
    TcIdxView idx;
    int64_t N_global;
    float *part, *dw0a, *dw0c, *colb3, *cpa, *cpc;
    double* bsum;
    TcMlp ma, mc;
    bf16 *h0, *depsb, *dvalb; float *eps, *val;
    PpoHyper hp;
};
static TcPpoPlan& tc_plan(dppo_handle* h) { if (!h->tc->plan) { h->tc->plan = new TcPpoPlan(); memset(h->tc->plan, 0, sizeof(TcPpoPlan)); } return *h->tc->plan; }
static void tc_plan_free(dppo_handle* h) { if (h->tc && h->tc->plan) { delete h->tc->plan; h->tc->plan = nullptr; } }

static int tc_ppo_begin(dppo_handle* h, cudaStream_t s, int N, int chunk_rows, int64_t N_global, int lead_rows = 0) {
    const Geom& g = h->g; const int KP0 = h->tc->KP0;
    const size_t nA = g.ao.n, nC = g.co.n;
    TcPpoPlan& P = tc_plan(h);
    if (h->deterministic || chunk_rows <= 0 || chunk_rows >= N) chunk_rows = N;
    chunk_rows = round_up(chunk_rows, 128);
    if (lead_rows <= 0 || lead_rows >= chunk_rows || chunk_rows >= N) lead_rows = 0;
    const int nchunks = lead_rows ? 1 + (N - lead_rows + chunk_rows - 1) / chunk_rows : (N + chunk_rows - 1) / chunk_rows;
    P.N = N; P.nchunks = nchunks; P.N_global = N_global; P.blocks_done = 0;
    memset(&P.idx, 0, sizeof(P.idx));
    P.chunk_rows = chunk_rows; P.lead_rows = lead_rows;
    P.full_rows = nchunks > 1 ? 1 : 0; P.rows_done = 0; P.dw_done = 0; P.dw_flush_chunk = nchunks / 2 - 1;
    const int NC = P.full_rows ? N : (P.chunk_rows < N ? P.chunk_rows : N);
    P.max_blocks = tc_nblk(N, LOSS8_ROWS) + nchunks;
    const bool amish = h->cfg.actor_act == DPPO_ACT_MISH, cmish = h->cfg.critic_act == DPPO_ACT_MISH;
    const size_t pf = tc_part_floats(h, g.H);
    const size_t n_cpa = (size_t)nchunks * h->sm_count * 2 * g.H, n_cpc = (size_t)nchunks * h->sm_count * 2 * g.Hc;
    size_t need = ws_bytes((size_t)NC * KP0, 2) + tc_mlp_ws_bytes(NC, g.H, amish, true) + tc_mlp_ws_bytes(NC, g.Hc, cmish, true)
                + ws_bytes((size_t)NC * g.A, 4) + ws_bytes(NC, 4) + 2 * ws_bytes((size_t)NC * 64, 2)
                + ws_bytes(pf, 4) + ws_bytes((size_t)KP0 * g.H, 4) + ws_bytes((size_t)KP0 * g.Hc, 4)
                + ws_bytes((size_t)P.max_blocks * 5, 8) + ws_bytes((size_t)P.max_blocks * (g.A + 1), 4) + ws_bytes(n_cpa, 4) + ws_bytes(n_cpc, 4);
    DPPO_TRY(ws_reserve(h, need, s));
    tc_actor_mlp(h, DPPO_NET_ACTOR_FT, P.ma); tc_critic_mlp(h, P.mc);
// ... 73 lines not shown
    else
        tc_pack_h0_kernel<<<tc_nblk((size_t)n * (KP0 / 8), 256), 256, 0, s>>>(prev, obs, inds, -g.K, n, g.A, g.Do, g.T, KP0, 1, P.h0 + r0 * KP0);
    TC_KCHECK(h);
    const bool overlap = defer && !h->prof_on;
    if (overlap && !h->aux_stream) {
        CUDA_TRY(cudaStreamCreateWithFlags(&h->aux_stream, cudaStreamNonBlocking));
        for (int i = 0; i < 2; ++i) CUDA_TRY(cudaEventCreateWithFlags(&h->aux_ev[i], cudaEventDisableTiming));
    }
    auto fork = [&]() -> int { CUDA_TRY(cudaEventRecord(h->aux_ev[0], s)); CUDA_TRY(cudaStreamWaitEvent(h->aux_stream, h->aux_ev[0], 0)); return 0; };
    auto join = [&]() -> int { CUDA_TRY(cudaEventRecord(h->aux_ev[1], h->aux_stream)); CUDA_TRY(cudaStreamWaitEvent(s, h->aux_ev[1], 0)); return 0; };
    if (overlap) DPPO_TRY(fork());
    DPPO_TRY(tc_mlp_forward(h, s, ma, n));
    DPPO_TRY(tc_mlp_forward(h, overlap ? h->aux_stream : s, mc, n));
    if (overlap) DPPO_TRY(join());
    if (loss8)
        tc_ppo_loss8_kernel<<<nlb, 256, 0, s>>>(prev, nxt, ma.out, inds, returns, oldvalues, advantages, oldlogp, mc.out,
                                               h->scalars, h->sched, P.hp, n, depsb, dvalb, P.bsum + (size_t)P.blocks_done * 5,
                                               P.colb3 + (size_t)P.blocks_done * (g.A + 1), iv);
    else
        tc_ppo_loss_kernel<<<nlb, 128, 0, s>>>(prev, nxt, ma.out, inds, returns, oldvalues, advantages, oldlogp, mc.out,
                                              h->scalars, h->sched, P.hp, n, depsb, dvalb, P.bsum + (size_t)P.blocks_done * 5,
                                              P.colb3 + (size_t)P.blocks_done * (g.A + 1));
    TC_KCHECK(h);
    P.blocks_done += nlb;
    if (defer) {
        if (overlap) DPPO_TRY(fork());
        DPPO_TRY(tc_mlp_backward_dx(h, s, ma, depsb, n, P.part, h->grads, g.ao.b1, g.ao.b2));
        DPPO_TRY(tc_mlp_backward_dx(h, overlap ? h->aux_stream : s, mc, dvalb, n, P.part, h->grads + nA, g.co.b1, g.co.b2));
        if (overlap) DPPO_TRY(join());
        P.rows_done += n;
        if (P.full_rows && chunk != P.dw_flush_chunk && P.rows_done < P.N) return 0;
        const size_t d0 = P.full_rows ? (size_t)P.dw_done : r0;
        const int dn = (int)((P.full_rows ? (size_t)P.rows_done : r0 + (size_t)n) - d0);
        const TcMlp da = tc_mlp_at(P.ma, d0), dc = tc_mlp_at(P.mc, d0);
        const bf16* const dd = P.depsb + d0 * 64; const bf16* const dvd = P.dvalb + d0 * 64;
        P.dw_done = P.rows_done;
        tcp::PairDesc pd[10];
        tc_mlp_dw_pair_descs(da, dd, dn, h->grads, g.ao.w1, g.ao.w2, g.ao.w3, P.dw0a, pd);
        tc_mlp_dw_pair_descs(dc, dvd, dn, h->grads + nA, g.co.w1, g.co.w2, g.co.w3, P.dw0c, pd + 5);
        return tcp::launch_group_pair(h, s, pd, 10, dn);
    }
    DPPO_TRY(tc_mlp_backward(h, s, ma, depsb, n, P.part, h->grads, g.ao.w1, g.ao.b1, g.ao.w2, g.ao.b2, g.ao.w3, P.dw0a));
    DPPO_TRY(tc_mlp_backward(h, s, mc, dvalb, n, P.part, h->grads + nA, g.co.w1, g.co.b1, g.co.w2, g.co.b2, g.co.w3, P.dw0c));
    P.rows_done += n;
    return 0;
}
static int tc_launch_tail(dppo_handle* h, cudaStream_t s, const double* bsum, int blocks_done, float inv_nglobal, float frac_local, const float* colb3,
                          const float* cpa, int rows_a, const float* cpc, int rows_c, const float* dw0a, const float* dw0c,
                          float* b2a_out = nullptr, float* b2c_out = nullptr) {
    const Geom& g = h->g;
    const size_t nA = g.ao.n, nC = g.co.n;
    float* gr = h->grads;
    const float* w = h->net_w[DPPO_NET_ACTOR_FT]; const ActorDerived& d = h->ad[DPPO_NET_ACTOR_FT];
    const size_t sm = (size_t)(g.T * g.td * 3) * sizeof(float);
    const size_t sm_staged = sm + (size_t)(g.T + g.td) * g.H * sizeof(float);
    const bool staged = sm_staged <= 160 * 1024;
    static bool attr_set_dev[64] = {};
    bool& attr_set = attr_set_dev[h->device & 63];
    if (!attr_set) { CUDA_TRY(cudaFuncSetAttribute(tc_ppo_tail_kernel, cudaFuncAttributeMaxDynamicSharedMemorySize, 160 * 1024)); attr_set = true; }
    TcTailArgs a;
    const int nthr = 512, wpb = nthr / 32;
    const bool wide = rows_a >= 256;
    const int cpb = wide ? 32 : wpb;
    const bool wide3 = blocks_done >= 256;
    a.wide = wide ? 1 : 0; a.wide3 = wide3 ? 1 : 0;
    const int nb[8] = {1, tc_nblk(g.A + 1, wide3 ? 32 : wpb), tc_nblk(2 * g.H, cpb), tc_nblk(2 * g.Hc, cpb), 1 + (g.H + 127) / 128,
                       tc_nblk((size_t)(g.A + g.Do) * g.H, nthr), tc_nblk((size_t)g.Do * g.Hc, nthr), tc_nblk(g.Hc, nthr)};
    a.first[0] = 0;
    for (int r = 0; r < 8; ++r) a.first[r + 1] = a.first[r] + nb[r];
    a.bsum = bsum; a.blocks_done = blocks_done; a.inv_nglobal = inv_nglobal; a.frac_local = frac_local; a.metrics = gr + nA + nC;
    a.colb3 = colb3; a.ncol3 = g.A + 1; a.b3a = gr + g.ao.b3; a.split3 = g.A; a.b3c = gr + nA + g.co.b3;
    a.cpa = cpa; a.rows_a = rows_a; a.HA = g.H; a.b2a = b2a_out ? b2a_out : gr + g.ao.b2; a.b1a = gr + g.ao.b1;
    a.cpc = cpc; a.rows_c = rows_c; a.HC = g.Hc; a.b2c = b2c_out ? b2c_out : gr + nA + g.co.b2; a.b1c = gr + nA + g.co.b1;
    a.w = w; a.ao = g.ao; a.A = g.A; a.td = g.td; a.T = g.T; a.Do = g.Do; a.tb_staged = staged ? 1 : 0;
    a.Gt = dw0a + (size_t)(g.A + g.Do) * g.H; a.sinemb = d.sinemb; a.thpre = d.thpre; a.temb = d.temb; a.gr = gr;
    a.dw0a = dw0a; a.gwin_a = gr + g.ao.win; a.dw0c_obs = dw0c + (size_t)g.A * g.Hc; a.gwin_c = gr + nA + g.co.win;
    a.dw0c_bias = dw0c + (size_t)(g.A + g.Do + g.T) * g.Hc; a.gbin_c = gr + nA + g.co.bin;
    tc_ppo_tail_kernel<<<a.first[8], nthr, staged ? sm_staged : sm, s>>>(a); TC_KCHECK(h);
    return 0;
}
static int tc_ppo_finish(dppo_handle* h, cudaStream_t s) {
    const Geom& g = h->g;
    const size_t nA = g.ao.n, nC = g.co.n;
    TcPpoPlan& P = tc_plan(h);
    float* gr = h->grads;
    const bool defer = P.ma.fused && P.mc.fused && !h->deterministic;
    const float* w = h->net_w[DPPO_NET_ACTOR_FT]; const ActorDerived& d = h->ad[DPPO_NET_ACTOR_FT];
    const size_t sm = (size_t)(g.T * g.td * 3) * sizeof(float);
    if (defer) return tc_launch_tail(h, s, P.bsum, P.blocks_done, P.hp.inv_nglobal, (float)((double)P.N / (double)P.N_global), P.colb3,
                                     P.cpa, P.nchunks * h->sm_count, P.cpc, P.nchunks * h->sm_count, P.dw0a, P.dw0c);
    ppo_metrics_kernel<<<1, 256, 0, s>>>(P.bsum, P.blocks_done, P.hp.inv_nglobal, (float)((double)P.N / (double)P.N_global), gr + nA + nC); TC_KCHECK(h);
    tc_reduce_cols_kernel<<<tc_nblk(g.A + 1, 8), 256, 0, s>>>(P.colb3, P.blocks_done, (size_t)(g.A + 1), g.A + 1, gr + g.ao.b3, g.A, gr + nA + g.co.b3); TC_KCHECK(h);
    time_backward_kernel<<<1 + (g.H + 127) / 128, 512, sm, s>>>(w, g.ao, g.A, g.td, g.H, g.T, P.dw0a + (size_t)(g.A + g.Do) * g.H, d.sinemb, d.thpre, d.temb, gr);
    TC_KCHECK(h);
    unpack_dw0_kernel<<<tc_nblk((size_t)(g.A + g.Do) * g.H, 256), 256, 0, s>>>(P.dw0a, g.A, g.td, g.Do, g.H, gr + g.ao.win); TC_KCHECK(h);
    unpack_dw0_kernel<<<tc_nblk((size_t)g.Do * g.Hc, 256), 256, 0, s>>>(P.dw0c + (size_t)g.A * g.Hc, 0, 0, g.Do, g.Hc, gr + nA + g.co.win); TC_KCHECK(h);
    CUDA_TRY(cudaMemcpyAsync(gr + nA + g.co.bin, P.dw0c + (size_t)(g.A + g.Do + g.T) * g.Hc, g.Hc * sizeof(float), cudaMemcpyDeviceToDevice, s));
    return 0;
}
static int tc_ppo_step(dppo_handle* h, cudaStream_t s, const float* obs, const float* prev, const float* nxt, const int32_t* inds,
                       const float* returns, const float* oldvalues, const float* advantages, const float* oldlogp,
                       int N, int64_t N_global, float adv_mean, float adv_std) {
    DPPO_TRY(tc_ppo_begin(h, s, N, 0, N_global));
    DPPO_TRY(tc_ppo_adv_stats(h, s, advantages, N, adv_mean, adv_std));
    DPPO_TRY(tc_ppo_chunk(h, s, 0, obs, prev, nxt, inds, returns, oldvalues, advantages, oldlogp, N));
    return tc_ppo_finish(h, s);
}

static bool tc_ppo_indexed_ok(const dppo_handle* h, const TcIdxView& v) {
    return (h->g.A % 4 == 0) && h->g.A <= 32 && ((((uintptr_t)v.chains | (uintptr_t)v.olp) & 15) == 0) && !h->deterministic &&
           fc_ok(h) && fc_critic_ok(h);
}
static int tc_ppo_step_indexed(dppo_handle* h, cudaStream_t s, const TcIdxView& view, int N, int64_t N_global, float adv_mean, float adv_std) {
    DPPO_TRY(tc_ppo_begin(h, s, N, 0, N_global));
    tc_plan(h).idx = view;
    DPPO_TRY(tc_ppo_adv_stats(h, s, nullptr, N, adv_mean, adv_std));
    DPPO_TRY(tc_ppo_chunk(h, s, 0, nullptr, nullptr, nullptr, nullptr, nullptr, nullptr, nullptr, nullptr, N));
    tc_plan(h).idx.flat = nullptr;
    return tc_ppo_finish(h, s);
}

static int tc_pretrain_grads(dppo_handle* h, cudaStream_t s, const float* actions, const float* obs, int N, int64_t N_global,
                             int64_t row_offset, const int32_t* t_in, const float* noise_in, uint64_t seed, uint64_t offset) {
    const Geom& g = h->g; const int KP0 = h->tc->KP0;
    const size_t nA = g.ao.n; float* gr = h->grads;
    const size_t ne = (size_t)N * g.A;
    const int nlb = tc_nblk(ne, 256);
    const size_t pf = tc_part_floats(h, g.H);
    size_t need = ws_bytes((size_t)N * KP0, 2) + tc_mlp_ws_bytes(N, g.H, h->cfg.actor_act == DPPO_ACT_MISH, true)
                + 4 * ws_bytes(ne, 4) + ws_bytes(N, 4) + ws_bytes((size_t)N * 64, 2) + ws_bytes(pf, 4)
                + ws_bytes((size_t)KP0 * g.H, 4) + ws_bytes(nlb, 8);
    DPPO_TRY(ws_reserve(h, need, s));
    TcMlp ma; tc_actor_mlp(h, DPPO_NET_ACTOR, ma);
    bf16* h0 = ws_take<bf16>(h, (size_t)N * KP0);
    tc_mlp_take(h, N, ma, true);
    float* eps = ws_take<float>(h, ne); float* deps = ws_take<float>(h, ne); float* noise = ws_take<float>(h, ne); float* xn = ws_take<float>(h, ne);
    int* trow = ws_take<int>(h, N);
    bf16* depsb = ws_take<bf16>(h, (size_t)N * 64);
    float* part = ws_take<float>(h, pf);
    float* dw0 = ws_take<float>(h, (size_t)KP0 * g.H);
    double* bsum = ws_take<double>(h, nlb);
    ma.h0 = h0; ma.out = eps;
    if (!h->deterministic) {
        CUDA_TRY(cudaMemsetAsync(gr, 0, nA * sizeof(float), s));
        CUDA_TRY(cudaMemsetAsync(dw0, 0, (size_t)KP0 * g.H * sizeof(float), s));
    }
// ... 11 lines not shown
```

diffusionpolicyoptimization_b200/csrc/ts_path.cuh:

```cuda
#pragma once
#include "tc_path.cuh"

namespace ts {
using namespace tc;

constexpr int SBM = 128, SBK = 64, STHREADS = 192;
constexpr int MAXP = 3;

struct Epi {
    int M, N;
    const float* bias;
    float* out_f32; int ld_f32; size_t split_stride;
    float scale;
};
struct Params {
    int m_blocks, n_blocks, splits;
    int kblocks, kb_per_split;
    int ka_blocks;
    Epi epi;
};
struct Maps { CUtensorMap a[2][MAXP], b[2][MAXP]; };

template <int BN, int P> __host__ __device__ constexpr int stage_bytes() { return P * (SBM * SBK * 2 + BN * SBK * 2); }
template <int BN, int P> __host__ __device__ constexpr int stages() { return (220 * 1024) / stage_bytes<BN, P>() > 4 ? 4 : (220 * 1024) / stage_bytes<BN, P>(); }
// ... 1006 lines not shown
    }
}
__global__ void ts_pad64_kernel(const float* __restrict__ src, int N, int ncols, bf16* __restrict__ hi, bf16* __restrict__ lo) {
    const size_t i = (size_t)blockIdx.x * blockDim.x + threadIdx.x;
    if (i >= (size_t)N * 8) return;
    const int r = (int)(i >> 3), k0 = (int)(i & 7) * 8;
    __align__(16) bf16 oh[8]; __align__(16) bf16 ol[8];
#pragma unroll
    for (int j = 0; j < 8; ++j) ts::split_bf16(k0 + j < ncols ? src[(size_t)r * ncols + k0 + j] : 0.f, oh[j], ol[j]);
    *reinterpret_cast<uint4*>(hi + (size_t)r * 64 + k0) = *reinterpret_cast<const uint4*>(oh);
    *reinterpret_cast<uint4*>(lo + (size_t)r * 64 + k0) = *reinterpret_cast<const uint4*>(ol);
}
__global__ void __launch_bounds__(256) ts_colsum_kernel(const bf16* __restrict__ Dh, const bf16* __restrict__ Dl, int N, int ncols, int rows_per_block,
                                                        float* __restrict__ part) {
    __shared__ float2 red[256];
    const int tpr = ncols / 2, groups = 256 / tpr;
    const int cg = threadIdx.x % tpr, rg = threadIdx.x / tpr;
    const int r0 = blockIdx.x * rows_per_block, r1 = min(N, r0 + rows_per_block);
    float2 acc = make_float2(0.f, 0.f);
    if (rg < groups) {
        for (int r = r0 + rg; r < r1; r += groups) {
            const float2 fh = __bfloat1622float2(*reinterpret_cast<const __nv_bfloat162*>(Dh + (size_t)r * ncols + 2 * cg));
            const float2 fl = __bfloat1622float2(*reinterpret_cast<const __nv_bfloat162*>(Dl + (size_t)r * ncols + 2 * cg));
            acc.x += fh.x + fl.x; acc.y += fh.y + fl.y;
        }
    }
    red[threadIdx.x] = acc;
    __syncthreads();
    if (threadIdx.x < tpr) {
        float2 sacc = red[threadIdx.x];
        for (int g = 1; g < groups; ++g) { const float2 o = red[g * tpr + threadIdx.x]; sacc.x += o.x; sacc.y += o.y; }
        part[(size_t)blockIdx.x * ncols + 2 * threadIdx.x] = sacc.x;
        part[(size_t)blockIdx.x * ncols + 2 * threadIdx.x + 1] = sacc.y;
    }
}

static int ensure_w23(dppo_handle* h, int net, cudaStream_t s) {
    const Geom& g = h->g;
    if (!h->w23_dirty[net] || net == DPPO_NET_CRITIC) return 0;
    const float* w = h->net_w[net]; ActorDerived& d = h->ad[net];
    fold_output_kernel<<<tc_nblk((size_t)(g.H + 1) * g.A, 128), 128, 0, s>>>(w + g.ao.w2, w + g.ao.b2, w + g.ao.w3, w + g.ao.b3, g.H, g.A, d.w23, d.b23);
    TC_KCHECK(h);
    h->w23_dirty[net] = 0;
    return 0;
}
struct TsFoldArgs {
    const float *w2, *w3, *b2, *b3, *b0;
    const float *win; int x_rows, x_skip;
    int obs_skip;
    const float* bt;
    int A, Do, T, H, NO, KP0, f16;
};
__global__ void __launch_bounds__(256) ts_fold_kernel(const TsFoldArgs f, const TsW F, float* __restrict__ bfold, const TsW B23) {
    extern __shared__ float w3t[];
    const int H = f.H, NO = f.NO, ld = f.H + f.KP0, HP = f.H + 1;
    for (int i0 = threadIdx.x; i0 < H * NO; i0 += blockDim.x * 8) {
        float t8[8];
#pragma unroll
        for (int u = 0; u < 8; ++u) { const int i = i0 + u * blockDim.x; t8[u] = i < H * NO ? __ldg(f.w3 + i) : 0.f; }
#pragma unroll
        for (int u = 0; u < 8; ++u) { const int i = i0 + u * blockDim.x; if (i < H * NO) w3t[(size_t)(i % NO) * HP + i / NO] = t8[u]; }
    }
    __syncthreads();
    const int lane = threadIdx.x & 31, k = blockIdx.x * (blockDim.x >> 5) + (threadIdx.x >> 5);
    if (k > ld) return;
    const float* row = nullptr; bool bias_row = false;
    if (k < H) row = f.w2 + (size_t)k * H;
    else if (k < ld) {
        const int k0 = k - H;
        if (k0 < f.A) { if (k0 < f.x_rows) row = f.win + (size_t)(k0 + f.x_skip) * H; }
        else if (k0 < f.A + f.Do) row = f.win + (size_t)(k0 - f.A + f.obs_skip) * H;
        else if (k0 < f.A + f.Do + f.T) { if (f.bt) row = f.bt + (size_t)(k0 - f.A - f.Do) * H; }
    } else { row = f.b2; bias_row = true; }
    float rv[32];
#pragma unroll
    for (int q = 0; q < 32; ++q) {
        const int j = lane + 32 * q;
        rv[q] = (row && j < H) ? row[j] : 0.f;
        if (bias_row && f.b0 && j < H) rv[q] += f.b0[j];
    }
    for (int a0 = 0; a0 < 64; a0 += 8) {
        float acc[8];
#pragma unroll
        for (int q = 0; q < 8; ++q) acc[q] = 0.f;
        if (row && a0 < NO) {
#pragma unroll
            for (int qq = 0; qq < 32; ++qq) {
                const int j = lane + 32 * qq;
                if (j < H) {
#pragma unroll
                    for (int q = 0; q < 8; ++q) if (a0 + q < NO) acc[q] = fmaf(rv[qq], w3t[(size_t)(a0 + q) * HP + j], acc[q]);
                }
            }
#pragma unroll
            for (int off = 16; off > 0; off >>= 1) {
#pragma unroll
                for (int q = 0; q < 8; ++q) acc[q] += __shfl_xor_sync(0xffffffffu, acc[q], off);
            }
        }
        if (lane < 8) {
            const int a = a0 + lane;
            float v = 0.f;
#pragma unroll
            for (int q = 0; q < 8; ++q) if (q == lane) v = acc[q];
            if (bias_row) bfold[a] = a < NO ? v + f.b3[a] : 0.f;
            else if (f.f16) ts_put_f16(F, (size_t)a * ld + k, v);
            else ts_put(F, (size_t)a * ld + k, v);
            if (!bias_row && k < H) ts_put(B23, (size_t)k * 128 + a, v);
        }
    }
}
static const int TS_MIN_ROWS = 2048;
static bool ts_shapes_ok(const dppo_handle* h) { return h->ts && h->ts->net[0].w1.p[0] != nullptr; }
static bool ts_eligible(const dppo_handle* h, int rows) {
    return h->cfg.precision == DPPO_PREC_BF16X3 && ts_shapes_ok(h) && rows >= TS_MIN_ROWS;
}
static int ts_alloc_w(TsW& w, size_t n) {
    CUDA_TRY(cudaMalloc(&w.p[0], 2 * n * sizeof(bf16)));
    w.p[1] = w.p[0] + n; w.p[2] = nullptr;
    return 0;
}
static int ts_init(dppo_handle* h) {
    if (h->cfg.precision != DPPO_PREC_BF16X3) return 0;
    const Geom& g = h->g;
    TsState* st = new TsState();
    memset(st, 0, sizeof(*st));
    h->ts = st;
    st->KP0 = round_up(g.A + g.Do + g.T + 1, 64);
    if ((g.H % 64) || (g.Hc % 64) || g.A > 32) return 0;
    for (int net = 0; net < 4; ++net) {
        TsNetW& w = st->net[net];
        const size_t H = net == DPPO_NET_CRITIC ? g.Hc : g.H;
        DPPO_TRY(ts_alloc_w(w.w0, st->KP0 * H)); DPPO_TRY(ts_alloc_w(w.w1, H * H));
        DPPO_TRY(ts_alloc_w(w.fw0, st->KP0 * H)); DPPO_TRY(ts_alloc_w(w.fw1, H * H));
        DPPO_TRY(ts_alloc_w(w.ffold, 64 * (H + st->KP0)));
        CUDA_TRY(cudaMalloc(&w.bfold, 64 * sizeof(float)));
        DPPO_TRY(ts_alloc_w(w.w23p, H * 128)); CUDA_TRY(cudaMemset(w.w23p.p[0], 0, 2 * H * 128 * sizeof(bf16)));
        st->fold_dirty[net] = 1;
    }
    return 0;
}
static void ts_destroy(dppo_handle* h) {
    if (!h->ts) return;
    cudaFree(h->ts->dw3_buf);
    for (int net = 0; net < 4; ++net) { TsNetW& w = h->ts->net[net]; cudaFree(w.w0.p[0]); cudaFree(w.w1.p[0]); cudaFree(w.fw0.p[0]); cudaFree(w.fw1.p[0]); cudaFree(w.ffold.p[0]); cudaFree(w.bfold); cudaFree(w.w23p.p[0]); }
    delete h->ts; h->ts = nullptr;
}
static int ts_refresh_net(dppo_handle* h, int net, cudaStream_t s) {
    if (h->cfg.precision != DPPO_PREC_BF16X3 || !ts_shapes_ok(h)) return 0;
    const Geom& g = h->g; const TsNetW& w = h->ts->net[net];
    h->ts->fold_dirty[net] = 1;
    if (net == DPPO_NET_CRITIC) ts_pack_critic_kernel<<<128, 256, 0, s>>>(h->net_w[net], g.co, g.A, g.Do, g.Hc, h->ts->KP0, w);
    else ts_pack_actor_kernel<<<256, 256, 0, s>>>(h->net_w[net], g.ao, g.A, g.td, g.Do, g.T, g.H, h->ts->KP0, h->ad[net].bt, w);
    TC_KCHECK(h);
    return 0;
}

struct TsMlp {
    const TsNetW* W; int H, NO, act1, KP0, net, din;
    int fp;
    const float *b0, *b1;
    SplitT h0, a0, a1, g0, g1, dh1, du;
    SplitT h0b, a0b, a1b;
    cudaEvent_t fold_ev;
    uint32_t *m0, *m1;
    float* out;
};
static int ts_ensure_fold(dppo_handle* h, int net, cudaStream_t s) {
    if (!h->ts->fold_dirty[net]) return 0;
    const Geom& g = h->g; const TsNetW& W = h->ts->net[net]; const float* w = h->net_w[net];
    TsFoldArgs f; memset(&f, 0, sizeof(f));
    f.A = g.A; f.Do = g.Do; f.T = g.T; f.KP0 = h->ts->KP0;
    if (net == DPPO_NET_CRITIC) {
        f.H = g.Hc; f.NO = 1; f.w2 = w + g.co.w2; f.w3 = w + g.co.w3; f.b2 = w + g.co.b2; f.b3 = w + g.co.b3; f.b0 = w + g.co.bin;
        f.win = w + g.co.win; f.x_rows = 0; f.obs_skip = 0; f.bt = nullptr;
        f.f16 = h->cfg.critic_act == DPPO_ACT_RELU ? 1 : 0;
    } else {
        f.H = g.H; f.NO = g.A; f.w2 = w + g.ao.w2; f.w3 = w + g.ao.w3; f.b2 = w + g.ao.b2; f.b3 = w + g.ao.b3; f.b0 = nullptr;
        f.win = w + g.ao.win; f.x_rows = g.A; f.x_skip = 0; f.obs_skip = g.A + g.td; f.bt = h->ad[net].bt;
        f.f16 = 1;
    }
    static bool attr_set_dev[64] = {};
    if (!attr_set_dev[h->device & 63]) { CUDA_TRY(cudaFuncSetAttribute(ts_fold_kernel, cudaFuncAttributeMaxDynamicSharedMemorySize, 96 * 1024)); attr_set_dev[h->device & 63] = true; }
    const size_t sm = (size_t)(f.H + 1) * f.NO * sizeof(float);
    if (sm > 96 * 1024 || f.H > 1024) DPPO_FAIL(-7, "ts_ensure_fold: output layer too wide for the fold kernel");
    ts_fold_kernel<<<tc_nblk((size_t)(f.H + f.KP0 + 1), 8), 256, sm, s>>>(f, W.ffold, W.bfold, W.w23p);
    TC_KCHECK(h);
    h->ts->fold_dirty[net] = 0;
    return 0;
}
static void ts_actor_mlp(const dppo_handle* h, int net, TsMlp& m) {
    const Geom& g = h->g; const float* w = h->net_w[net];
    memset(&m, 0, sizeof(m));
    m.W = &h->ts->net[net]; m.H = g.H; m.NO = g.A; m.act1 = h->cfg.actor_act + 1; m.KP0 = h->ts->KP0; m.net = net; m.din = g.Din;
    m.fp = 4;
    m.b0 = nullptr; m.b1 = w + g.ao.b1;
}
static void ts_critic_mlp(const dppo_handle* h, TsMlp& m) {
    const Geom& g = h->g; const float* w = h->net_w[DPPO_NET_CRITIC];
    memset(&m, 0, sizeof(m));
    m.W = &h->ts->net[DPPO_NET_CRITIC]; m.H = g.Hc; m.NO = 1; m.act1 = h->cfg.critic_act + 1; m.KP0 = h->ts->KP0; m.net = DPPO_NET_CRITIC; m.din = g.Do;
    m.fp = h->cfg.critic_act == DPPO_ACT_RELU ? 4 : 2;
    m.b0 = w + g.co.bin; m.b1 = w + g.co.b1;
}
static size_t ts_mlp_ws_bytes(int N, int H, int KP0, bool mish, bool bwd) {
    return 2 * (2 * ws_bytes((size_t)N * KP0, 2) + 2 * ws_bytes((size_t)N * H, 2)) + 2 * ws_bytes((size_t)N * H, 2) * (size_t)((mish ? 2 : 0) + (bwd ? 4 : 0))
         + 2 * ws_bytes((size_t)N * (H / 32), 4);
}
static SplitT ts_take(dppo_handle* h, size_t n, int planes) {
    SplitT t = split_null();
    for (int pl = 0; pl < planes; ++pl) t.p[pl] = ws_take<bf16>(h, n);
    return t;
}
static void ts_mlp_take(dppo_handle* h, int N, TsMlp& m, bool bwd) {
    const size_t n = (size_t)N * m.H;
    m.h0 = ts_take(h, (size_t)N * m.KP0, 2);
    m.a0 = ts_take(h, n, 2); m.a1 = ts_take(h, n, 2);
    if (m.act1 == 2) { m.g0 = ts_take(h, n, 2); m.g1 = ts_take(h, n, 2); }
    if (bwd) { m.dh1 = ts_take(h, n, 2); m.du = ts_take(h, n, 2); }
    if (bwd && m.fp == 4) { m.h0b = ts_take(h, (size_t)N * m.KP0, 2); m.a0b = ts_take(h, n, 2); m.a1b = ts_take(h, n, 2); }
    m.m0 = ws_take<uint32_t>(h, (size_t)N * (m.H / 32)); m.m1 = ws_take<uint32_t>(h, (size_t)N * (m.H / 32));
}
static ts::Operand ts_op(const bf16* const* p, size_t off, bool mn_major, int64_t mn, int64_t k, int64_t ld) {
    ts::Operand o; o.mn_major = mn_major; o.mn = mn; o.k = k; o.ld = ld;
    for (int pl = 0; pl < ts::MAXP; ++pl) o.p[pl] = p[pl] ? p[pl] + off : nullptr;
    return o;
}
static ts::Operand tsK(const SplitT& t, int64_t mn, int64_t k, int64_t ld) { return ts_op(t.p, 0, false, mn, k, ld); }
static ts::Operand tsMN(const SplitT& t, int64_t mn, int64_t k, int64_t ld) { return ts_op(t.p, 0, true, mn, k, ld); }
static ts::Operand tswK(const TsW& w, size_t off, int64_t mn, int64_t k, int64_t ld) { return ts_op(w.p, off, false, mn, k, ld); }
static ts::Operand tswMN(const TsW& w, size_t off, int64_t mn, int64_t k, int64_t ld) { return ts_op(w.p, off, true, mn, k, ld); }
static ts::Gemm ts_gemm_of(ts::Operand A, ts::Operand B, int M, int N, int planes, int dual = 0) {
    ts::Gemm g; memset(&g, 0, sizeof(g));
    g.A = A; g.B = B; g.M = M; g.N = N; g.splits = 1; g.planes = planes; g.dual = dual; g.epi.M = M; g.epi.N = N;
    return g;
}
static int ts_run(dppo_handle* h, cudaStream_t s, const ts::Gemm& g) { const int r = ts::launch(h, s, g); return r < 0 ? r : 0; }
static tsp::Gemm tsp_gemm_of(ts::Operand A, ts::Operand B, int M, int N, int planes, const SplitT& out, int out_planes, int ld_out) {
    tsp::Gemm g; memset(&g, 0, sizeof(g));
// ... 139 lines not shown
        for (int q = 0; q < DW3_KS; ++q) s += __ldcg(part + ((size_t)jc * DW3_KS + q) * 32 * NO + i);
        const float bias = f.b2[jj] + (f.b0 ? f.b0[jj] : 0.f);
        f.out[(size_t)jj * NO + a] = fmaf(bias, ones[a], s);
    }
    if (threadIdx.x == 0) done[jc] = 0;
}
constexpr int DW3_RB = 8;
__device__ __forceinline__ void ts_rank_rows_body(const TsDw3Args& f, int bid, float* sm, int row_begin, int row_end) {
    const int H = f.H, NO = f.NO, nrows = min(H + f.KP0 + 1, row_end), q0 = row_begin + bid * DW3_RB;
    const int ones = f.A + f.Do + f.T;
    for (int i = threadIdx.x; i < DW3_RB * NO; i += blockDim.x) {
        const int q = q0 + i / NO, a = i % NO;
        float v = 0.f;
        if (q < H) v = f.g1[(size_t)q * NO + a];
        else if (q < H + f.KP0) v = f.g0[(size_t)(q - H) * NO + a];
        else if (q == H + f.KP0) v = f.g0[(size_t)ones * NO + a];
        sm[i] = v;
    }
    float* w3s = sm + DW3_RB * NO;
    const int n3 = H * NO;
    for (int i0 = threadIdx.x; i0 < n3; i0 += blockDim.x * 8) {
        float t8[8];
#pragma unroll
        for (int u = 0; u < 8; ++u) { const int i = i0 + u * blockDim.x; t8[u] = i < n3 ? __ldg(f.w3 + i) : 0.f; }
#pragma unroll
        for (int u = 0; u < 8; ++u) { const int i = i0 + u * blockDim.x; if (i < n3) w3s[(i / NO) * (NO + 1) + i % NO] = t8[u]; }
    }
    __syncthreads();
    for (int j = threadIdx.x; j < H; j += blockDim.x) {
        float w3r[32];
#pragma unroll
        for (int a = 0; a < 32; ++a) w3r[a] = a < NO ? w3s[j * (NO + 1) + a] : 0.f;
        float old[DW3_RB];
#pragma unroll
        for (int r = 0; r < DW3_RB; ++r) {
            const int q = q0 + r;
            old[r] = (q >= H && q < H + f.KP0 && q < nrows) ? f.dw0[(size_t)(q - H) * H + j] : 0.f;
        }
#pragma unroll
        for (int r = 0; r < DW3_RB; ++r) {
            const int q = q0 + r;
            if (q >= nrows) break;
            float acc = 0.f;
#pragma unroll
            for (int a = 0; a < 32; ++a) if (a < NO) acc = fmaf(sm[r * NO + a], w3r[a], acc);
            if (q < H) f.dw2[(size_t)q * H + j] = acc;
            else if (q < H + f.KP0) f.dw0[(size_t)(q - H) * H + j] = old[r] + acc;
            else f.db2[j] = acc;
        }
    }
}
__global__ void __launch_bounds__(512) ts_dw3_assemble_kernel(const TsDw3Args fa, int blocks_a, const TsDw3Args fc, int blocks_c,
                                                              float* __restrict__ part, int* __restrict__ done, int rank_a, int rank_c, int phase) {
    extern __shared__ float dw3_sm[];
    int b = blockIdx.x;
    if (phase == 1) {
        if (b < blocks_a) { ts_dw3_assemble_body(fa, b, dw3_sm, part, done); return; }
        b -= blocks_a;
        if (b < blocks_c) { ts_dw3_assemble_body(fc, b, dw3_sm, part + (size_t)blocks_a * 32 * fa.NO, done + blocks_a / DW3_KS); return; }
        b -= blocks_c;
    }
    const int ra0 = phase == 0 ? fa.H : 0, ra1 = phase == 0 ? fa.H + fa.KP0 + 1 : fa.H;
    const int rc0 = phase == 0 ? fc.H : 0, rc1 = phase == 0 ? fc.H + fc.KP0 + 1 : fc.H;
    if (b < rank_a) { ts_rank_rows_body(fa, b, dw3_sm, ra0, ra1); return; }
    b -= rank_a;
    if (b < rank_c) ts_rank_rows_body(fc, b, dw3_sm, rc0, rc1);
}
static inline int tsDW3KS() { return DW3_KS; }
static TsDw3Args ts_dw3_args(const dppo_handle* h, int net, const float* g1, const float* g0, float* gnet, float* dw0) {
    const Geom& g = h->g; const float* w = h->net_w[net];
    TsDw3Args f; memset(&f, 0, sizeof(f));
    f.A = g.A; f.Do = g.Do; f.T = g.T; f.KP0 = h->ts->KP0; f.g1 = g1; f.g0 = g0; f.dw0 = dw0;
    if (net == DPPO_NET_CRITIC) {
        f.H = g.Hc; f.NO = 1; f.w2 = w + g.co.w2; f.b2 = w + g.co.b2; f.b0 = w + g.co.bin; f.win = w + g.co.win; f.x_rows = 0; f.obs_skip = 0; f.bt = nullptr;
        f.w3 = w + g.co.w3; f.out = gnet + g.co.w3; f.dw2 = gnet + g.co.w2; f.db2 = gnet + g.co.b2;
    } else {
        f.H = g.H; f.NO = g.A; f.w2 = w + g.ao.w2; f.b2 = w + g.ao.b2; f.b0 = nullptr; f.win = w + g.ao.win; f.x_rows = g.A; f.x_skip = 0;
        f.obs_skip = g.A + g.td; f.bt = h->ad[net].bt;
        f.w3 = w + g.ao.w3; f.out = gnet + g.ao.w3; f.dw2 = gnet + g.ao.w2; f.db2 = gnet + g.ao.b2;
    }
    return f;
}
static int ts_dw3_assemble(dppo_handle* h, cudaStream_t s, int actor_net, const float* ga1, const float* ga0, float* gneta, float* dw0a,
                           const float* gc1, const float* gc0, float* gnetc, float* dw0c, int phase = -1) {
    if (phase < 0) {
        DPPO_TRY(ts_dw3_assemble(h, s, actor_net, ga1, ga0, gneta, dw0a, gc1, gc0, gnetc, dw0c, 0));
        return ts_dw3_assemble(h, s, actor_net, ga1, ga0, gneta, dw0a, gc1, gc0, gnetc, dw0c, 1);
    }
    const Geom& g = h->g;
    const TsDw3Args fa = ts_dw3_args(h, actor_net, ga1, ga0, gneta, dw0a);
    TsDw3Args fc = fa; int nbc = 0, nrc = 0;
    const int KP0r = h->ts->KP0 + 1;
    const int nra = phase == 0 ? tc_nblk((size_t)KP0r, DW3_RB) : tc_nblk((size_t)g.H, DW3_RB);
    if (gc1) {
        fc = ts_dw3_args(h, DPPO_NET_CRITIC, gc1, gc0, gnetc, dw0c); nbc = tc_nblk((size_t)g.Hc, 32) * tsDW3KS();
        nrc = phase == 0 ? tc_nblk((size_t)KP0r, DW3_RB) : tc_nblk((size_t)g.Hc, DW3_RB);
    }
    const int nba = tc_nblk((size_t)g.H, 32) * tsDW3KS();
    auto smf = [&](const TsDw3Args& f) {
        const int K = f.H + f.A + f.Do + f.T;
        const size_t a = (size_t)(((K + DW3_KS - 1) / DW3_KS) * f.NO + 16 * 32 * f.NO), b = (size_t)(DW3_RB * f.NO + f.H * (f.NO + 1));
        return (a > b ? a : b) * sizeof(float);
    };
    auto kper = [&](const TsDw3Args& f) { return (f.H + f.A + f.Do + f.T + DW3_KS - 1) / DW3_KS; };
    const size_t sm = smf(fa) > smf(fc) ? smf(fa) : smf(fc);
    static bool attr_set_dev[64] = {};
    if (!attr_set_dev[h->device & 63]) { CUDA_TRY(cudaFuncSetAttribute(ts_dw3_assemble_kernel, cudaFuncAttributeMaxDynamicSharedMemorySize, 100 * 1024)); attr_set_dev[h->device & 63] = true; }
    if (sm > 100 * 1024 || g.A > 32 || kper(fa) > 128 || kper(fc) > 128) DPPO_FAIL(-7, "ts_dw3_assemble: shape not covered");
    TsState* st = h->ts;
    const size_t need = 1024 + ((size_t)nba * 32 * g.A + (size_t)nbc * 32) * sizeof(float);
    if ((nba + nbc) / DW3_KS > 256) DPPO_FAIL(-7, "ts_dw3_assemble: too many column chunks");
    if (st->dw3_bytes < need) {
        CUDA_TRY(cudaStreamSynchronize(s));
        if (st->dw3_buf) cudaFree(st->dw3_buf);
        CUDA_TRY(cudaMalloc(&st->dw3_buf, need)); CUDA_TRY(cudaMemsetAsync(st->dw3_buf, 0, need, s));
        st->dw3_bytes = need;
    }
    int* done = reinterpret_cast<int*>(st->dw3_buf);
    float* partb = reinterpret_cast<float*>(st->dw3_buf + 1024);
    ts_dw3_assemble_kernel<<<(phase == 1 ? nba + nbc : 0) + nra + nrc, 512, sm, s>>>(fa, nba, fc, nbc, partb, done, nra, nrc, phase);
    TC_KCHECK(h);
    return 0;
}
static size_t ts_part_floats(const dppo_handle* h, int H) {
    const size_t a = tc_part_floats(h, H), b = (size_t)(h->sm_count / 2 + 1) * 65536;
    return a > b ? a : b;
}
static size_t ts_actor_forward_ws(const dppo_handle* h, int N) { return ts_mlp_ws_bytes(N, h->g.H, h->ts->KP0, h->cfg.actor_act == DPPO_ACT_MISH, false); }
static int ts_actor_forward(dppo_handle* h, cudaStream_t s, int net, const float* x, const float* obs, int obs_div, int N,
                            const int* trow, int tconst, float* eps, int chainK = 0) {
    const Geom& g = h->g; const int KP0 = h->ts->KP0;
    const size_t need = h->ws.used + ts_actor_forward_ws(h, N);
    if (need > h->ws.cap) DPPO_FAIL(-7, "ts_actor_forward: workspace too small (%zu > %zu)", need, h->ws.cap);
    const size_t mark = h->ws.used;
    TsMlp m; ts_actor_mlp(h, net, m);
    ts_mlp_take(h, N, m, false);
    m.out = eps;
    DPPO_TRY(ts_ensure_fold(h, net, s));
    ts_pack_h0_kernel<<<tc_nblk((size_t)N * (KP0 / 8), 256), 256, 0, s>>>(x, obs, trow, tconst, N, g.A, g.Do, g.T, KP0, obs_div, m.h0, split_null(), chainK);
    TC_KCHECK(h);
    const int r = ts_mlp_forward(h, s, m, N);
    h->ws.used = mark;
    return r;
}
static int ts_value(dppo_handle* h, cudaStream_t s, const float* obs, int N, float* v) {
    const Geom& g = h->g; const int KP0 = h->ts->KP0;
    DPPO_TRY(ws_reserve(h, ts_mlp_ws_bytes(N, g.Hc, KP0, h->cfg.critic_act == DPPO_ACT_MISH, false), s));
    TsMlp m; ts_critic_mlp(h, m);
    ts_mlp_take(h, N, m, false);
    m.out = v;
    DPPO_TRY(ts_ensure_fold(h, DPPO_NET_CRITIC, s));
    ts_pack_h0_kernel<<<tc_nblk((size_t)N * (KP0 / 8), 256), 256, 0, s>>>(nullptr, obs, nullptr, -1, N, g.A, g.Do, g.T, KP0, 1,
                                                                          m.fp == 4 ? m.h0 : split_null(), m.fp == 4 ? split_null() : m.h0, 0);
    TC_KCHECK(h);
    return ts_mlp_forward(h, s, m, N);
}

static bool ts_ppo_indexed_ok(const dppo_handle* h, const TcIdxView& v) {
    return (h->g.A % 4 == 0) && h->g.A <= 32 && ((((uintptr_t)v.chains | (uintptr_t)v.olp) & 15) == 0);
}
static int ts_ppo_step(dppo_handle* h, cudaStream_t s, const float* obs, const float* prev, const float* nxt, const int32_t* inds,
                       const float* returns, const float* oldvalues, const float* advantages, const float* oldlogp,
                       int N, int64_t N_global, float adv_mean, float adv_std, const TcIdxView* idx = nullptr) {
    const Geom& g = h->g; const int KP0 = h->ts->KP0;
    const size_t nA = g.ao.n, nC = g.co.n;
    float* gr = h->grads;
    const bool amish = h->cfg.actor_act == DPPO_ACT_MISH, cmish = h->cfg.critic_act == DPPO_ACT_MISH;
    const bool loss8 = idx ? true : (g.A % 4 == 0) && g.A <= 32 && ((((uintptr_t)prev | (uintptr_t)nxt | (uintptr_t)oldlogp) & 15) == 0);
    const int nlb = loss8 ? tc_nblk(N, LOSS8_ROWS) : tc_nblk(N, 128);
    const int nrb = (N + 31) / 32;
    const size_t pf = ts_part_floats(h, g.H);
    const size_t need = ts_mlp_ws_bytes(N, g.H, KP0, amish, true) + ts_mlp_ws_bytes(N, g.Hc, KP0, cmish, true)
                      + 2 * ws_bytes((size_t)N * g.A, 4) + 2 * ws_bytes(N, 4) + 4 * ws_bytes((size_t)N * 64, 2)
// ... 42 lines not shown
    DPPO_TRY(ts_ensure_fold(h, DPPO_NET_ACTOR_FT, sc)); DPPO_TRY(ts_ensure_fold(h, DPPO_NET_CRITIC, sc));
    if (side) { CUDA_TRY(cudaEventRecord(h->aux_ev[2], sc)); ma.fold_ev = h->aux_ev[2]; }
    if (adv_std < 0.f) {
        if (idx) adv_stats_kernel<<<1, 1024, 0, sc>>>(idx->adv, N, h->scalars, idx->flat, idx->K, idx->P);
        else adv_stats_kernel<<<1, 1024, 0, sc>>>(advantages, N, h->scalars);
        TC_KCHECK(h);
    }
    else { set_scalars_kernel<<<1, 1, 0, sc>>>(h->scalars, adv_mean, adv_std); TC_KCHECK(h); }
    DPPO_TRY(ts_mlp_forward(h, s, ma, N, side ? 2 : 0));
    DPPO_TRY(ts_mlp_forward(h, sc, mc, N));
    DPPO_TRY(join());
    PpoHyper hp;
    hp.A = g.A; hp.Da = h->cfg.action_dim; hp.K = g.K; hp.T = g.T; hp.reward_horizon = h->cfg.reward_horizon; hp.norm_adv = h->cfg.norm_adv;
    hp.dcv = h->cfg.denoised_clip_value; hp.min_lp_std = h->cfg.min_logprob_denoising_std;
    hp.lp_lo = h->cfg.logprob_clip_lo; hp.lp_hi = h->cfg.logprob_clip_hi; hp.gamma_d = h->cfg.gamma_denoising;
    hp.clip_coef = h->cfg.clip_ploss_coef; hp.clip_base = h->cfg.clip_ploss_coef_base; hp.clip_rate = h->cfg.clip_ploss_coef_rate;
    hp.clip_v = h->cfg.clip_vloss_coef; hp.vf_coef = h->cfg.vf_coef; hp.inv_nglobal = 1.0f / (float)N_global;
    const float frac_local = (float)((double)N / (double)N_global);
    if (loss8) {
        TcIdxView iv; memset(&iv, 0, sizeof(iv));
        if (idx) iv = *idx;
        tc_ppo_loss8_kernel<<<nlb, 256, 0, s>>>(prev, nxt, eps, inds, returns, oldvalues, advantages, oldlogp, val, h->scalars, h->sched, hp, N,
                                               depsb.p[0], dvalb.p[0], bsum, colb3, iv, depsb.p[1], dvalb.p[1]);
        TC_KCHECK(h);
    } else {
        ppo_loss_kernel<<<nlb, 128, 0, s>>>(prev, nxt, eps, inds, returns, oldvalues, advantages, oldlogp, val, h->scalars, h->sched, hp, N, deps, dval, bsum);
        TC_KCHECK(h);
        ts_pad64_kernel<<<tc_nblk((size_t)N * 8, 256), 256, 0, s>>>(deps, N, g.A, depsb.p[0], depsb.p[1]); TC_KCHECK(h);
        ts_pad64_kernel<<<tc_nblk((size_t)N * 8, 256), 256, 0, s>>>(dval, N, 1, dvalb.p[0], dvalb.p[1]); TC_KCHECK(h);
    }
    DPPO_TRY(fork());
    DPPO_TRY(ts_mlp_backward_dx(h, s, ma, depsb, N, cpa));
    DPPO_TRY(ts_mlp_backward_dx(h, sc, mc, dvalb, N, cpc));
    DPPO_TRY(join());
    tsp::DwDesc dd[10];
    const int nda = ts_mlp_dw_descs(ma, depsb, N, gr, g.ao.w1, dw0a, dd, ga1, ga0);
    const int ndc = ts_mlp_dw_descs(mc, dvalb, N, gr + nA, g.co.w1, dw0c, dd + nda, gc1, gc0);
    DPPO_TRY(tsp::launch_dw_pair(h, s, dd, nda + ndc, N, part, pf, ebeg));
    DPPO_TRY(ts_dw3_assemble(h, s, DPPO_NET_ACTOR_FT, ga1, ga0, gr, dw0a, gc1, gc0, gr + nA, dw0c, 0));
    DPPO_TRY(fork());
    DPPO_TRY(ts_dw3_assemble(h, sc, DPPO_NET_ACTOR_FT, ga1, ga0, gr, dw0a, gc1, gc0, gr + nA, dw0c, 1));
    float* b2scr = gfold + (size_t)(g.H + g.Hc + 2 * KP0) * 32;
    if (loss8) {
        DPPO_TRY(tc_launch_tail(h, s, bsum, nlb, hp.inv_nglobal, frac_local, colb3, cpa, nrb, cpc, nrb, dw0a, dw0c, b2scr, b2scr + g.H));
        DPPO_TRY(join());
        return 0;
    }
    DPPO_TRY(join());
    ppo_metrics_kernel<<<1, 256, 0, s>>>(bsum, nlb, hp.inv_nglobal, frac_local, gr + nA + nC); TC_KCHECK(h);
    DPPO_TRY(colsum(h, s, deps, g.A, N, g.A, nullptr, 1, part, gr + g.ao.b3));
    DPPO_TRY(colsum(h, s, dval, 1, N, 1, nullptr, 1, part, gr + nA + g.co.b3));
    tc_reduce_cols_kernel<<<tc_nblk(2 * g.H, 8), 256, 0, s>>>(cpa, nrb, (size_t)2 * g.H, 2 * g.H, b2scr, g.H, gr + g.ao.b1); TC_KCHECK(h);
    tc_reduce_cols_kernel<<<tc_nblk(2 * g.Hc, 8), 256, 0, s>>>(cpc, nrb, (size_t)2 * g.Hc, 2 * g.Hc, b2scr + g.H, g.Hc, gr + nA + g.co.b1); TC_KCHECK(h);
    const float* w = h->net_w[DPPO_NET_ACTOR_FT]; const ActorDerived& d = h->ad[DPPO_NET_ACTOR_FT];
    const size_t sm = (size_t)(g.T * g.td * 3) * sizeof(float);
    time_backward_kernel<<<1 + (g.H + 127) / 128, 512, sm, s>>>(w, g.ao, g.A, g.td, g.H, g.T, dw0a + (size_t)(g.A + g.Do) * g.H, d.sinemb, d.thpre, d.temb, gr); TC_KCHECK(h);
    unpack_dw0_kernel<<<tc_nblk((size_t)(g.A + g.Do) * g.H, 256), 256, 0, s>>>(dw0a, g.A, g.td, g.Do, g.H, gr + g.ao.win); TC_KCHECK(h);
    unpack_dw0_kernel<<<tc_nblk((size_t)g.Do * g.Hc, 256), 256, 0, s>>>(dw0c + (size_t)g.A * g.Hc, 0, 0, g.Do, g.Hc, gr + nA + g.co.win); TC_KCHECK(h);
    CUDA_TRY(cudaMemcpyAsync(gr + nA + g.co.bin, dw0c + (size_t)(g.A + g.Do + g.T) * g.Hc, g.Hc * sizeof(float), cudaMemcpyDeviceToDevice, s));
    return 0;
}

static int ts_pretrain_grads(dppo_handle* h, cudaStream_t s, const float* actions, const float* obs, int N, int64_t N_global,
                             int64_t row_offset, const int32_t* t_in, const float* noise_in, uint64_t seed, uint64_t offset) {
    const Geom& g = h->g; const int KP0 = h->ts->KP0;
    const size_t nA = g.ao.n; float* gr = h->grads;
    const size_t ne = (size_t)N * g.A;
    const int nlb = tc_nblk(ne, 256);
    const int nrb = (N + 31) / 32;
    const size_t pf = ts_part_floats(h, g.H);
    const size_t need = ts_mlp_ws_bytes(N, g.H, KP0, h->cfg.actor_act == DPPO_ACT_MISH, true) + 4 * ws_bytes(ne, 4) + ws_bytes(N, 4)
                      + 2 * ws_bytes((size_t)N * 64, 2) + ws_bytes(pf, 4) + ws_bytes((size_t)KP0 * g.H, 4) + ws_bytes(nlb, 8) + ws_bytes(16, 4)
                      + ws_bytes((size_t)nrb * 2 * g.H, 4) + ws_bytes((size_t)(g.H + KP0) * 32 + g.H, 4);
    DPPO_TRY(ws_reserve(h, need, s));
    TsMlp ma; ts_actor_mlp(h, DPPO_NET_ACTOR, ma);
    ts_mlp_take(h, N, ma, true);
    float* ga1 = ws_take<float>(h, (size_t)(g.H + KP0) * 32 + g.H); float* ga0 = ga1 + (size_t)g.H * g.A;
    DPPO_TRY(ts_ensure_fold(h, DPPO_NET_ACTOR, s));
    float* eps = ws_take<float>(h, ne); float* deps = ws_take<float>(h, ne); float* noise = ws_take<float>(h, ne); float* xn = ws_take<float>(h, ne);
    int* trow = ws_take<int>(h, N);
    SplitT depsb = ts_take(h, (size_t)N * 64, 2);
    float* part = ws_take<float>(h, pf);
    float* dw0 = ws_take<float>(h, (size_t)KP0 * g.H);
    double* bsum = ws_take<double>(h, nlb);
    int* ebeg = ws_take<int>(h, 16);
    float* cpa = ws_take<float>(h, (size_t)nrb * 2 * g.H);
    ma.out = eps;
    pretrain_prep_kernel<<<tc_nblk(ne, 256), 256, 0, s>>>(actions, t_in, noise_in, N, g.A, g.T, h->sched, seed, offset, row_offset, trow, noise, xn); TC_KCHECK(h);
    ts_pack_h0_kernel<<<tc_nblk((size_t)N * (KP0 / 8), 256), 256, 0, s>>>(xn, obs, trow, 0, N, g.A, g.Do, g.T, KP0, 1, ma.h0, ma.h0b, 0); TC_KCHECK(h);
    DPPO_TRY(ts_mlp_forward(h, s, ma, N));
    const float scale = 1.0f / ((float)N_global * (float)g.A);
    mse_loss_kernel<<<nlb, 256, 0, s>>>(eps, noise, ne, scale, deps, bsum); TC_KCHECK(h);
    sum_blocks_kernel<<<1, 256, 0, s>>>(bsum, nlb, scale, gr + nA); TC_KCHECK(h);
    ts_pad64_kernel<<<tc_nblk((size_t)N * 8, 256), 256, 0, s>>>(deps, N, g.A, depsb.p[0], depsb.p[1]); TC_KCHECK(h);
    DPPO_TRY(ts_mlp_backward_dx(h, s, ma, depsb, N, cpa));
    tsp::DwDesc dd[5];
    const int nd = ts_mlp_dw_descs(ma, depsb, N, gr, g.ao.w1, dw0, dd, ga1, ga0);
    DPPO_TRY(tsp::launch_dw_pair(h, s, dd, nd, N, part, pf, ebeg));
    DPPO_TRY(ts_dw3_assemble(h, s, DPPO_NET_ACTOR, ga1, ga0, gr, dw0, nullptr, nullptr, nullptr, nullptr));
    tc_reduce_cols_kernel<<<tc_nblk(2 * g.H, 8), 256, 0, s>>>(cpa, nrb, (size_t)2 * g.H, 2 * g.H, ga1 + (size_t)(g.H + KP0) * 32, g.H, gr + g.ao.b1); TC_KCHECK(h);
    DPPO_TRY(colsum(h, s, deps, g.A, N, g.A, nullptr, 1, part, gr + g.ao.b3));
    const float* w = h->net_w[DPPO_NET_ACTOR]; const ActorDerived& d = h->ad[DPPO_NET_ACTOR];
    const size_t sm = (size_t)(g.T * g.td * 3) * sizeof(float);
    time_backward_kernel<<<1 + (g.H + 127) / 128, 512, sm, s>>>(w, g.ao, g.A, g.td, g.H, g.T, dw0 + (size_t)(g.A + g.Do) * g.H, d.sinemb, d.thpre, d.temb, gr); TC_KCHECK(h);
    unpack_dw0_kernel<<<tc_nblk((size_t)(g.A + g.Do) * g.H, 256), 256, 0, s>>>(dw0, g.A, g.td, g.Do, g.H, gr + g.ao.win); TC_KCHECK(h);
    return 0;
}
```

Before: 71.97 million.

## Fuse Adam update with time-embedding table prep, parallelize time backward, add PDL launches

Adds a single ts_update_kernel that applies AdamW to all finetune parameters, writes packed/bf16-split weight copies, and recomputes the time-embedding tables from the updated weights. A last-block atomic counter handles the time-MLP parameters. This replaces the separate Adam launch and table re-prep on the bf16x3 path. The time backward kernel now spreads the per-timestep dte work across T blocks plus column blocks, using a global scratch buffer and a last-block reduction. Several launches use programmatic dependent launch to overlap launch latency. The cost is extra atomic counters and grid-wide completion logic.

```diff
diff --git a/diffusionpolicyoptimization_b200/csrc/common.cuh b/diffusionpolicyoptimization_b200/csrc/common.cuh
--- a/diffusionpolicyoptimization_b200/csrc/common.cuh
+++ b/diffusionpolicyoptimization_b200/csrc/common.cuh
@@ -112,11 +112,25 @@
     ActorOff ao; CriticOff co;
 };
 
+__device__ __forceinline__ void pdl_grid_begin() {
+    asm volatile("griddepcontrol.wait;" ::: "memory");
+    asm volatile("griddepcontrol.launch_dependents;" ::: "memory");
+}
+template <typename... KArgs, typename... Args>
+static cudaError_t launch_pdl(void (*kernel)(KArgs...), dim3 grid, dim3 block, size_t smem, cudaStream_t s, Args... args) {
+    cudaLaunchAttribute at[1];
+    at[0].id = cudaLaunchAttributeProgrammaticStreamSerialization; at[0].val.programmaticStreamSerializationAllowed = 1;
+    cudaLaunchConfig_t cfg = {};
+    cfg.gridDim = grid; cfg.blockDim = block; cfg.dynamicSmemBytes = smem; cfg.stream = s; cfg.attrs = at; cfg.numAttrs = 1;
+    return cudaLaunchKernelEx(&cfg, kernel, args...);
+}
+
 struct ActorDerived {
     float* sinemb;
     float* thpre;
     float* temb;
     float* bt;
+    float* dte;
     float* w0p;
     float* w23;
     float* b23;
diff --git a/diffusionpolicyoptimization_b200/csrc/dppo_api.cu b/diffusionpolicyoptimization_b200/csrc/dppo_api.cu
--- a/diffusionpolicyoptimization_b200/csrc/dppo_api.cu
+++ b/diffusionpolicyoptimization_b200/csrc/dppo_api.cu
@@ -270,6 +270,7 @@
         CUDA_TRY(cudaMalloc(&d.thpre, (size_t)g.T * 2 * g.td * sizeof(float)));
         CUDA_TRY(cudaMalloc(&d.temb, (size_t)g.T * g.td * sizeof(float)));
         CUDA_TRY(cudaMalloc(&d.bt, (size_t)g.T * g.H * sizeof(float)));
+        CUDA_TRY(cudaMalloc(&d.dte, ((size_t)g.T * g.td + 4) * sizeof(float))); CUDA_TRY(cudaMemset(d.dte, 0, ((size_t)g.T * g.td + 4) * sizeof(float)));
         CUDA_TRY(cudaMalloc(&d.w23, (size_t)g.H * g.A * sizeof(float))); CUDA_TRY(cudaMalloc(&d.b23, (size_t)g.A * sizeof(float)));
         CUDA_TRY(cudaMalloc(&d.w0p, (size_t)g.KP * g.H * sizeof(float)));
     }
@@ -315,7 +316,7 @@
     cudaFree(h->env_norm);
     cudaFree(h->params); cudaFree(h->sched); cudaFree(h->grads_buf[0]); cudaFree(h->grads_buf[1]);  cudaFree(h->flags); cudaFree(h->scalars);
     for (int i = 0; i < 2; ++i) { cudaFree(h->opt[i].m); cudaFree(h->opt[i].v); }
-    for (int net = 0; net < 4; ++net) { ActorDerived& d = h->ad[net]; cudaFree(d.sinemb); cudaFree(d.thpre); cudaFree(d.temb); cudaFree(d.bt); cudaFree(d.w0p); cudaFree(d.w23); cudaFree(d.b23); }
+    for (int net = 0; net < 4; ++net) { ActorDerived& d = h->ad[net]; cudaFree(d.sinemb); cudaFree(d.thpre); cudaFree(d.temb); cudaFree(d.bt); cudaFree(d.dte); cudaFree(d.w0p); cudaFree(d.w23); cudaFree(d.b23); }
     if (h->ws.base) cudaFree(h->ws.base);
     if (h->copy_stream) { cudaStreamDestroy(h->copy_stream); for (int i = 0; i < 9; ++i) cudaEventDestroy(h->copy_ev[i]); }
     if (h->aux_stream) { cudaStreamDestroy(h->aux_stream); for (int i = 0; i < 3; ++i) if (h->aux_ev[i]) cudaEventDestroy(h->aux_ev[i]); }
@@ -485,11 +486,10 @@
 }
 static int actor_bwd_fp32(dppo_handle* h, cudaStream_t s, int net, const FwdBufs& f, const float* deps, int N, const int* trow,
                           BwdBufs& b, float* Gseg, float* dw0p, float* gnet) {
-    const Geom& g = h->g; const float* w = h->net_w[net]; const ActorDerived& d = h->ad[net];
+    const Geom& g = h->g; const float* w = h->net_w[net];
     DPPO_TRY(mlp_bwd_fp32(h, s, w, g.ao.w1, g.ao.b1, g.ao.w2, g.ao.b2, g.ao.w3, g.ao.b3, h->cfg.actor_act + 1, f, deps, N,
                           g.KP, g.H, g.A, trow, g.T, b, gnet, dw0p, Gseg));
-    size_t sm = (size_t)(g.T * g.td * 3) * sizeof(float);
-    time_backward_kernel<<<1, 512, sm, s>>>(w, g.ao, g.A, g.td, g.H, g.T, Gseg, d.sinemb, d.thpre, d.temb, gnet); KLAUNCH(h); KCHECK();
+    CUDA_TRY(launch_time_backward(h, s, net, Gseg, gnet)); KLAUNCH(h);
     unpack_dw0_kernel<<<nblk((size_t)(g.A + g.Do) * g.H, 256), 256, 0, s>>>(dw0p, g.A, g.td, g.Do, g.H, gnet + g.ao.win); KLAUNCH(h); KCHECK();
     return 0;
 }
@@ -926,12 +926,16 @@
     return 0;
 }
 
+static float adam_next_alpha(dppo_handle* h, int opt, float lr) {
+    OptState& o = h->opt[opt];
+    o.step += 1;
+    const float b1p = powf(h->cfg.adam_beta1, (float)o.step), b2p = powf(h->cfg.adam_beta2, (float)o.step);
+    return lr * sqrtf(1.f - b2p) / (1.f - b1p);
+}
 static int adam_apply(dppo_handle* h, cudaStream_t s, int opt, float* w, const float* g, size_t n, float lr, float wd) {
     OptState& o = h->opt[opt];
-    o.step += 1;
     const float b1 = h->cfg.adam_beta1, b2 = h->cfg.adam_beta2;
-    float b1p = powf(b1, (float)o.step), b2p = powf(b2, (float)o.step);
-    float alpha = lr * sqrtf(1.f - b2p) / (1.f - b1p);
+    const float alpha = adam_next_alpha(h, opt, lr);
     adamw_kernel<<<nblk(n, 256), 256, 0, s>>>(w, g, o.m, o.v, n, lr, alpha, b1, b2, h->cfg.adam_eps, wd, h->skip_update, nullptr); KLAUNCH(h); KCHECK();
     return 0;
 }
@@ -940,6 +944,7 @@
 static int ppo_apply_tail(dppo_handle* h, cudaStream_t s, float lr, int apply, float* metrics8, float* grads_out) {
     const size_t nA = h->g.ao.n, nC = h->g.co.n; float* gr = h->grads;
     if (apply) {
+        bool tables_done = false;
         if (h->grad_clip_norm > 0.f) {
             DPPO_TRY(allreduce_sum(h, gr, nA + nC + 8, s));
             if (grads_out) { CUDA_TRY(cudaMemcpyAsync(grads_out, gr, (nA + nC) * sizeof(float), cudaMemcpyDeviceToDevice, s)); grads_out = nullptr; }
@@ -955,9 +960,15 @@
             gr = h->gsum;
         } else {
             DPPO_TRY(allreduce_sum(h, gr, nA + nC + 8, s));
-            DPPO_TRY(adam_apply(h, s, DPPO_OPT_FINETUNE, h->net_w[DPPO_NET_ACTOR_FT], gr, nA + nC, lr, h->cfg.weight_decay));
+            if (ts_update_ok(h)) {
+                DPPO_TRY(ts_apply_update(h, s, gr, lr, adam_next_alpha(h, DPPO_OPT_FINETUNE, lr), h->cfg.weight_decay, nullptr));
+                tables_done = true;
+            } else {
+                DPPO_TRY(adam_apply(h, s, DPPO_OPT_FINETUNE, h->net_w[DPPO_NET_ACTOR_FT], gr, nA + nC, lr, h->cfg.weight_decay));
+            }
         }
-        if (h->cfg.precision == DPPO_PREC_BF16 && tc_shapes_ok(h) && 2 * h->g.td <= 256) {
+        if (tables_done) {
+        } else if (h->cfg.precision == DPPO_PREC_BF16 && tc_shapes_ok(h) && 2 * h->g.td <= 256) {
             DPPO_TRY(tc_prep_pack_ft_critic(h, s));
         } else {
             DPPO_TRY(prep_net(h, DPPO_NET_ACTOR_FT, s));
diff --git a/diffusionpolicyoptimization_b200/csrc/simt_kernels.cuh b/diffusionpolicyoptimization_b200/csrc/simt_kernels.cuh
--- a/diffusionpolicyoptimization_b200/csrc/simt_kernels.cuh
+++ b/diffusionpolicyoptimization_b200/csrc/simt_kernels.cuh
@@ -217,7 +217,9 @@
     out[i] = s * scale;
 }
 
-__device__ __forceinline__ void actor_prep_body(const int t, float* sm, const float* __restrict__ w, ActorOff o, int A, int td, int H,
+struct WRead { const float* __restrict__ p; __device__ __forceinline__ float operator()(size_t i) const { return p[i]; } };
+template <class WF>
+__device__ __forceinline__ void actor_prep_body(const int t, float* sm, const WF w, ActorOff o, int A, int td, int H,
                                   float* __restrict__ sinemb, float* __restrict__ thpre,
                                   float* __restrict__ temb, float* __restrict__ bt, __nv_bfloat16* __restrict__ bt16) {
     float* se = sm;
@@ -234,21 +236,21 @@
     }
     __syncthreads();
     if (tid < 2 * td) {
-        float s = w[o.tb1 + tid];
-        for (int j = 0; j < td; ++j) s = fmaf(se[j], w[o.tw1 + (size_t)j * 2 * td + tid], s);
+        float s = w(o.tb1 + tid);
+        for (int j = 0; j < td; ++j) s = fmaf(se[j], w(o.tw1 + (size_t)j * 2 * td + tid), s);
         thpre[t * 2 * td + tid] = s;
         hp[tid] = mish_f(s);
     }
     __syncthreads();
     if (tid < td) {
-        float s = w[o.tb2 + tid];
-        for (int j = 0; j < 2 * td; ++j) s = fmaf(hp[j], w[o.tw2 + (size_t)j * td + tid], s);
+        float s = w(o.tb2 + tid);
+        for (int j = 0; j < 2 * td; ++j) s = fmaf(hp[j], w(o.tw2 + (size_t)j * td + tid), s);
         te[tid] = s; temb[t * td + tid] = s;
     }
     __syncthreads();
     for (int c = tid; c < H; c += blockDim.x) {
-        float s = w[o.bin + c];
-        for (int j = 0; j < td; ++j) s = fmaf(te[j], w[o.win + (size_t)(A + j) * H + c], s);
+        float s = w(o.bin + c);
+        for (int j = 0; j < td; ++j) s = fmaf(te[j], w(o.win + (size_t)(A + j) * H + c), s);
         bt[(size_t)t * H + c] = s;
         if (bt16) bt16[(size_t)t * H + c] = __float2bfloat16(s);
     }
@@ -257,7 +259,7 @@
                                   float* __restrict__ sinemb, float* __restrict__ thpre,
                                   float* __restrict__ temb, float* __restrict__ bt) {
     extern __shared__ float sm[];
-    actor_prep_body(blockIdx.x, sm, w, o, A, td, H, sinemb, thpre, temb, bt, nullptr);
+    actor_prep_body(blockIdx.x, sm, WRead{w}, o, A, td, H, sinemb, thpre, temb, bt, nullptr);
 }
 __global__ void fold_output_kernel(const float* __restrict__ w2, const float* __restrict__ b2, const float* __restrict__ w3, const float* __restrict__ b3,
                                    int H, int A, float* __restrict__ w23, float* __restrict__ b23) {
@@ -600,23 +602,21 @@
     for (int i = threadIdx.x; i < nseg * ncols; i += blockDim.x) part[(size_t)blockIdx.x * nseg * ncols + i] = sm[i];
 }
 
-__device__ __forceinline__ void time_backward_body(const int bid, const int nblk, float* sm, const bool staged,
+__device__ __forceinline__ void time_backward_body(const int bid, float* sm,
                                      const float* __restrict__ w, ActorOff o, int A, int td, int H, int T,
                                      const float* __restrict__ G, const float* __restrict__ sinemb,
                                      const float* __restrict__ thpre, const float* __restrict__ temb,
-                                     float* __restrict__ g) {
-    float* dte = sm;
-    float* dh = dte + T * td;
+                                     float* __restrict__ dte_g, float* __restrict__ g) {
     const int tid = threadIdx.x, nt = blockDim.x;
-    if (nblk == 1 || bid > 0) {
-        const int c0 = nblk == 1 ? 0 : (bid - 1) * 128, c1 = nblk == 1 ? H : min(H, c0 + 128);
-        const int lanes = nblk == 1 ? 1 : 4;
+    if (bid >= T) {
+        const int lanes = 16;
+        const int c0 = (bid - T) * (nt / lanes), c1 = min(H, c0 + nt / lanes);
         for (int i = tid; i < (c1 - c0) * lanes; i += nt) {
             const int c = c0 + i / lanes, part = i % lanes;
             float bsum = 0.f;
-            float acc[16];
-#pragma unroll
-            for (int q = 0; q < 16; ++q) acc[q] = 0.f;
+            float acc[2];
+#pragma unroll
+            for (int q = 0; q < 2; ++q) acc[q] = 0.f;
             for (int t0 = 0; t0 < T; t0 += 32) {
                 float gc[32];
 #pragma unroll
@@ -624,7 +624,7 @@
 #pragma unroll
                 for (int q = 0; q < 32; ++q) bsum += gc[q];
 #pragma unroll
-                for (int jj = 0; jj < 16; ++jj) {
+                for (int jj = 0; jj < 2; ++jj) {
                     const int j = part + jj * lanes;
                     if (j < td) {
 #pragma unroll
@@ -633,48 +633,52 @@
                 }
             }
             if (part == 0) g[o.bin + c] = bsum;
-            for (int jj = 0; jj < 16; ++jj) {
+            for (int jj = 0; jj < 2; ++jj) {
                 const int j = part + jj * lanes;
                 if (j < td) g[o.win + (size_t)(A + j) * H + c] = acc[jj];
             }
-            for (int j = part + 16 * lanes; j < td; j += lanes) {
+            for (int j = part + 2 * lanes; j < td; j += lanes) {
                 float a = 0.f;
                 for (int t = 0; t < T; ++t) a = fmaf(temb[t * td + j], G[(size_t)t * H + c], a);
                 g[o.win + (size_t)(A + j) * H + c] = a;
             }
         }
-        if (nblk > 1) return;
-    }
-    if (staged) {
-        float* sG = dh + T * 2 * td;
-        float* sW = sG + T * H;
-        for (int i = tid; i < T * H; i += nt) sG[i] = G[i];
-        for (int i = tid; i < td * H; i += nt) sW[i] = w[o.win + (size_t)A * H + i];
-        __syncthreads();
-        const int lane = tid & 31;
-        for (int p = tid >> 5; p < T * td; p += nt >> 5) {
-            const int t = p / td, j = p % td;
+        return;
+    }
+    {
+        const int t = bid, lane = tid & 31;
+        for (int j = tid >> 5; j < td; j += nt >> 5) {
             float s = 0.f;
-            for (int c = lane; c < H; c += 32) s = fmaf(sW[j * H + c], sG[t * H + c], s);
+#pragma unroll
+            for (int q0 = 0; q0 < 32; q0 += 16) {
+                float wr[16], gv[16];
+#pragma unroll
+                for (int q = 0; q < 16; ++q) {
+                    const int c = lane + (q0 + q) * 32;
+                    wr[q] = c < H ? w[o.win + (size_t)(A + j) * H + c] : 0.f;
+                    gv[q] = c < H ? G[(size_t)t * H + c] : 0.f;
+                }
+#pragma unroll
+                for (int q = 0; q < 16; ++q) { const int c = lane + (q0 + q) * 32; if (c < H) s = fmaf(wr[q], gv[q], s); }
+            }
 #pragma unroll
             for (int off = 16; off > 0; off >>= 1) s += __shfl_xor_sync(0xffffffffu, s, off);
-            if (lane == 0) dte[t * td + j] = s;
-        }
-    } else
-    for (int j = tid >> 5; j < td; j += nt >> 5) {
-        const int lane = tid & 31;
-        float wr[32];
-#pragma unroll
-        for (int q = 0; q < 32; ++q) { const int c = lane + q * 32; wr[q] = c < H ? w[o.win + (size_t)(A + j) * H + c] : 0.f; }
-        for (int t = 0; t < T; ++t) {
-            float s = 0.f;
-#pragma unroll
-            for (int q = 0; q < 32; ++q) { const int c = lane + q * 32; if (c < H) s = fmaf(wr[q], G[(size_t)t * H + c], s); }
-#pragma unroll
-            for (int off = 16; off > 0; off >>= 1) s += __shfl_xor_sync(0xffffffffu, s, off);
-            if (lane == 0) dte[t * td + j] = s;
-        }
-    }
+            if (lane == 0) dte_g[t * td + j] = s;
+        }
+    }
+    __shared__ int last_flag;
+    int* done = reinterpret_cast<int*>(dte_g + T * td);
+    __threadfence();
+    __syncthreads();
+    if (tid == 0) last_flag = (atomicAdd(done, 1) == T - 1) ? 1 : 0;
+    __syncthreads();
+    if (!last_flag) return;
+    __threadfence();
+    float* dte = sm;
+    float* dh = dte + T * td;
+    float* mt = dh + T * 2 * td;
+    for (int i = tid; i < T * td; i += nt) dte[i] = __ldcg(dte_g + i);
+    for (int i = tid; i < T * 2 * td; i += nt) mt[i] = mish_f(thpre[i]);
     __syncthreads();
     for (int i = tid; i < T * 2 * td; i += nt) {
         int t = i / (2 * td), k = i % (2 * td);
@@ -686,7 +690,7 @@
     for (int i = tid; i < 2 * td * td; i += nt) {
         int k = i / td, j = i % td;
         float s = 0.f;
-        for (int t = 0; t < T; ++t) s = fmaf(mish_f(thpre[t * 2 * td + k]), dte[t * td + j], s);
+        for (int t = 0; t < T; ++t) s = fmaf(mt[t * 2 * td + k], dte[t * td + j], s);
         g[o.tw2 + i] = s;
         int ss = i / (2 * td), kk = i % (2 * td);
         float a = 0.f;
@@ -695,13 +699,28 @@
     }
     for (int j = tid; j < td; j += nt) { float s = 0.f; for (int t = 0; t < T; ++t) s += dte[t * td + j]; g[o.tb2 + j] = s; }
     for (int k = tid; k < 2 * td; k += nt) { float s = 0.f; for (int t = 0; t < T; ++t) s += dh[t * 2 * td + k]; g[o.tb1 + k] = s; }
+    if (tid == 0) *done = 0;
 }
 __global__ void __launch_bounds__(512) time_backward_kernel(const float* __restrict__ w, ActorOff o, int A, int td, int H, int T,
                                      const float* __restrict__ G, const float* __restrict__ sinemb,
                                      const float* __restrict__ thpre, const float* __restrict__ temb,
-                                     float* __restrict__ g) {
+                                     float* __restrict__ dte_g, float* __restrict__ g) {
     extern __shared__ float sm[];
-    time_backward_body(blockIdx.x, gridDim.x, sm, false, w, o, A, td, H, T, G, sinemb, thpre, temb, g);
+    time_backward_body(blockIdx.x, sm, w, o, A, td, H, T, G, sinemb, thpre, temb, dte_g, g);
+}
+static inline int time_backward_grid(const Geom& g) { return g.T + (g.H + 31) / 32; }
+static inline size_t time_backward_smem(const Geom& g) { return (size_t)5 * g.T * g.td * sizeof(float); }
+static cudaError_t launch_time_backward(const dppo_handle* h, cudaStream_t s, int net, const float* G, float* gnet) {
+    static bool attr_set_dev[64] = {};
+    const Geom& g = h->g; const ActorDerived& d = h->ad[net];
+    const size_t sm = time_backward_smem(g);
+    if (sm > 48 * 1024 && !attr_set_dev[h->device & 63]) {
+        const cudaError_t e = cudaFuncSetAttribute(time_backward_kernel, cudaFuncAttributeMaxDynamicSharedMemorySize, (int)sm);
+        if (e != cudaSuccess) return e;
+        attr_set_dev[h->device & 63] = true;
+    }
+    time_backward_kernel<<<time_backward_grid(g), 512, sm, s>>>(h->net_w[net], g.ao, g.A, g.td, g.H, g.T, G, d.sinemb, d.thpre, d.temb, d.dte, gnet);
+    return cudaGetLastError();
 }
 __device__ __forceinline__ void unpack_dw0_body(const int bid, const float* __restrict__ dw0p, int A, int skip, int Do, int H, float* __restrict__ gwin) {
     int i = bid * blockDim.x + threadIdx.x;
@@ -713,17 +732,20 @@
     unpack_dw0_body(blockIdx.x, dw0p, A, skip, Do, H, gwin);
 }
 
+__device__ __forceinline__ void adamw_elem(float& p, float& mi, float& vi, float gi, float lr, float alpha, float b1, float b2, float eps, float wd) {
+    if (wd != 0.f) p = p - p * (wd * lr);
+    mi = mi + (gi - mi) * (1.f - b1);
+    vi = vi + (gi * gi - vi) * (1.f - b2);
+    p = p - mi * alpha / (sqrtf(vi) + eps);
+}
 __global__ void adamw_kernel(float* __restrict__ w, const float* __restrict__ g, float* __restrict__ m, float* __restrict__ v,
                              size_t n, float lr, float alpha, float b1, float b2, float eps, float wd,
                              const int* __restrict__ skip0 = nullptr, const int* __restrict__ skip1 = nullptr) {
     size_t i = (size_t)blockIdx.x * blockDim.x + threadIdx.x;
     if (i >= n) return;
     if ((skip0 && *skip0) || (skip1 && *skip1)) return;
-    float p = w[i], gi = g[i], mi = m[i], vi = v[i];
-    if (wd != 0.f) p = p - p * (wd * lr);
-    mi = mi + (gi - mi) * (1.f - b1);
-    vi = vi + (gi * gi - vi) * (1.f - b2);
-    p = p - mi * alpha / (sqrtf(vi) + eps);
+    float p = w[i], mi = m[i], vi = v[i];
+    adamw_elem(p, mi, vi, g[i], lr, alpha, b1, b2, eps, wd);
     w[i] = p; m[i] = mi; v[i] = vi;
 }
 struct VarSegs { unsigned int off[24]; int n; };
diff --git a/diffusionpolicyoptimization_b200/csrc/tc_path.cuh b/diffusionpolicyoptimization_b200/csrc/tc_path.cuh
--- a/diffusionpolicyoptimization_b200/csrc/tc_path.cuh
+++ b/diffusionpolicyoptimization_b200/csrc/tc_path.cuh
@@ -82,7 +82,7 @@
     extern __shared__ float prep_sm[];
     const int b = blockIdx.x;
     if (b < a.T)
-        actor_prep_body(b, prep_sm, a.wa, a.ao, a.A, a.td, a.H, a.sinemb, a.thpre, a.temb, a.bt, a.a_w2w0 + (size_t)a.H * a.H + (size_t)(a.A + a.Do) * a.H);
+        actor_prep_body(b, prep_sm, WRead{a.wa}, a.ao, a.A, a.td, a.H, a.sinemb, a.thpre, a.temb, a.bt, a.a_w2w0 + (size_t)a.H * a.H + (size_t)(a.A + a.Do) * a.H);
     else if (b < a.T + a.na)
         tc_pack_actor_body((size_t)(b - a.T) * blockDim.x + threadIdx.x, (size_t)a.na * blockDim.x, a.wa, a.ao, a.A, a.td, a.Do, a.T, a.H, a.KP0, nullptr,
                            a.a_w2w0, a.a_w1, a.a_w3t, a.a_w3p, a.a_w1t, a.a_w2t);
@@ -211,10 +211,11 @@
     const float* colb3; int ncol3; float* b3a; int split3; float* b3c;
     const float* cpa; int rows_a; int HA; float* b2a; float* b1a;
     const float* cpc; int rows_c; int HC; float* b2c; float* b1c;
-    const float* w; ActorOff ao; int A, td, T, Do; int tb_staged; const float* Gt; const float* sinemb; const float* thpre; const float* temb; float* gr;
+    const float* w; ActorOff ao; int A, td, T, Do; const float* Gt; const float* sinemb; const float* thpre; const float* temb; float* dte; float* gr;
     const float* dw0a; float* gwin_a; const float* dw0c_obs; float* gwin_c; const float* dw0c_bias; float* gbin_c;
 };
 __global__ void __launch_bounds__(512) tc_ppo_tail_kernel(const TcTailArgs a) {
+    pdl_grid_begin();
     extern __shared__ float tail_sm[];
     const int b = blockIdx.x;
     if (b < a.first[1]) ppo_metrics_body(a.bsum, a.blocks_done, a.inv_nglobal, a.frac_local, a.metrics);
@@ -229,8 +230,7 @@
         if (a.wide) tc_reduce_cols_wide_body(b - a.first[3], a.cpc, a.rows_c, (size_t)2 * a.HC, 2 * a.HC, a.b2c, a.HC, a.b1c);
         else tc_reduce_cols_body(b - a.first[3], a.cpc, a.rows_c, (size_t)2 * a.HC, 2 * a.HC, a.b2c, a.HC, a.b1c);
     }
-    else if (b < a.first[5]) time_backward_body(b - a.first[4], a.first[5] - a.first[4], tail_sm, a.tb_staged != 0, a.w, a.ao, a.A, a.td, a.HA, a.T,
-                                                a.Gt, a.sinemb, a.thpre, a.temb, a.gr);
+    else if (b < a.first[5]) time_backward_body(b - a.first[4], tail_sm, a.w, a.ao, a.A, a.td, a.HA, a.T, a.Gt, a.sinemb, a.thpre, a.temb, a.dte, a.gr);
     else if (b < a.first[6]) unpack_dw0_body(b - a.first[5], a.dw0a, a.A, a.td, a.Do, a.HA, a.gwin_a);
     else if (b < a.first[7]) unpack_dw0_body(b - a.first[6], a.dw0c_obs, 0, 0, a.Do, a.HC, a.gwin_c);
     else { const int i = (b - a.first[7]) * blockDim.x + threadIdx.x; if (i < a.HC) a.gbin_c[i] = a.dw0c_bias[i]; }
@@ -885,11 +885,10 @@
 
 static int tc_actor_grads(dppo_handle* h, cudaStream_t s, int net, const TcMlp& m, const float* deps, const bf16* depsb, int N,
                           float* part, float* dw0, float* gnet) {
-    const Geom& g = h->g; const float* w = h->net_w[net]; const ActorDerived& d = h->ad[net];
+    const Geom& g = h->g;
     DPPO_TRY(tc_mlp_backward(h, s, m, depsb, N, part, gnet, g.ao.w1, g.ao.b1, g.ao.w2, g.ao.b2, g.ao.w3, dw0));
     if (deps) DPPO_TRY(colsum(h, s, deps, g.A, N, g.A, nullptr, 1, part, gnet + g.ao.b3));
-    const size_t sm = (size_t)(g.T * g.td * 3) * sizeof(float);
-    time_backward_kernel<<<1, 512, sm, s>>>(w, g.ao, g.A, g.td, g.H, g.T, dw0 + (size_t)(g.A + g.Do) * g.H, d.sinemb, d.thpre, d.temb, gnet);
+    CUDA_TRY(launch_time_backward(h, s, net, dw0 + (size_t)(g.A + g.Do) * g.H, gnet));
     TC_KCHECK(h);
     unpack_dw0_kernel<<<tc_nblk((size_t)(g.A + g.Do) * g.H, 256), 256, 0, s>>>(dw0, g.A, g.td, g.Do, g.H, gnet + g.ao.win);
     TC_KCHECK(h);
@@ -1069,9 +1068,8 @@
     const size_t nA = g.ao.n, nC = g.co.n;
     float* gr = h->grads;
     const float* w = h->net_w[DPPO_NET_ACTOR_FT]; const ActorDerived& d = h->ad[DPPO_NET_ACTOR_FT];
-    const size_t sm = (size_t)(g.T * g.td * 3) * sizeof(float);
-    const size_t sm_staged = sm + (size_t)(g.T + g.td) * g.H * sizeof(float);
-    const bool staged = sm_staged <= 160 * 1024;
+    const size_t sm = time_backward_smem(g);
+    if (sm > 160 * 1024) DPPO_FAIL(-7, "tc_launch_tail: time_dim x denoising_steps too large");
     static bool attr_set_dev[64] = {};
     bool& attr_set = attr_set_dev[h->device & 63];
     if (!attr_set) { CUDA_TRY(cudaFuncSetAttribute(tc_ppo_tail_kernel, cudaFuncAttributeMaxDynamicSharedMemorySize, 160 * 1024)); attr_set = true; }
@@ -1081,7 +1079,7 @@
     const int cpb = wide ? 32 : wpb;
     const bool wide3 = blocks_done >= 256;
     a.wide = wide ? 1 : 0; a.wide3 = wide3 ? 1 : 0;
-    const int nb[8] = {1, tc_nblk(g.A + 1, wide3 ? 32 : wpb), tc_nblk(2 * g.H, cpb), tc_nblk(2 * g.Hc, cpb), 1 + (g.H + 127) / 128,
+    const int nb[8] = {1, tc_nblk(g.A + 1, wide3 ? 32 : wpb), tc_nblk(2 * g.H, cpb), tc_nblk(2 * g.Hc, cpb), time_backward_grid(g),
                        tc_nblk((size_t)(g.A + g.Do) * g.H, nthr), tc_nblk((size_t)g.Do * g.Hc, nthr), tc_nblk(g.Hc, nthr)};
     a.first[0] = 0;
     for (int r = 0; r < 8; ++r) a.first[r + 1] = a.first[r] + nb[r];
@@ -1089,11 +1087,11 @@
     a.colb3 = colb3; a.ncol3 = g.A + 1; a.b3a = gr + g.ao.b3; a.split3 = g.A; a.b3c = gr + nA + g.co.b3;
     a.cpa = cpa; a.rows_a = rows_a; a.HA = g.H; a.b2a = b2a_out ? b2a_out : gr + g.ao.b2; a.b1a = gr + g.ao.b1;
     a.cpc = cpc; a.rows_c = rows_c; a.HC = g.Hc; a.b2c = b2c_out ? b2c_out : gr + nA + g.co.b2; a.b1c = gr + nA + g.co.b1;
-    a.w = w; a.ao = g.ao; a.A = g.A; a.td = g.td; a.T = g.T; a.Do = g.Do; a.tb_staged = staged ? 1 : 0;
-    a.Gt = dw0a + (size_t)(g.A + g.Do) * g.H; a.sinemb = d.sinemb; a.thpre = d.thpre; a.temb = d.temb; a.gr = gr;
+    a.w = w; a.ao = g.ao; a.A = g.A; a.td = g.td; a.T = g.T; a.Do = g.Do;
+    a.Gt = dw0a + (size_t)(g.A + g.Do) * g.H; a.sinemb = d.sinemb; a.thpre = d.thpre; a.temb = d.temb; a.dte = d.dte; a.gr = gr;
     a.dw0a = dw0a; a.gwin_a = gr + g.ao.win; a.dw0c_obs = dw0c + (size_t)g.A * g.Hc; a.gwin_c = gr + nA + g.co.win;
     a.dw0c_bias = dw0c + (size_t)(g.A + g.Do + g.T) * g.Hc; a.gbin_c = gr + nA + g.co.bin;
-    tc_ppo_tail_kernel<<<a.first[8], nthr, staged ? sm_staged : sm, s>>>(a); TC_KCHECK(h);
+    CUDA_TRY(launch_pdl(tc_ppo_tail_kernel, dim3(a.first[8]), dim3(nthr), sm, s, a)); TC_KCHECK(h);
     return 0;
 }
 static int tc_ppo_finish(dppo_handle* h, cudaStream_t s) {
@@ -1102,13 +1100,11 @@
     TcPpoPlan& P = tc_plan(h);
     float* gr = h->grads;
     const bool defer = P.ma.fused && P.mc.fused && !h->deterministic;
-    const float* w = h->net_w[DPPO_NET_ACTOR_FT]; const ActorDerived& d = h->ad[DPPO_NET_ACTOR_FT];
-    const size_t sm = (size_t)(g.T * g.td * 3) * sizeof(float);
     if (defer) return tc_launch_tail(h, s, P.bsum, P.blocks_done, P.hp.inv_nglobal, (float)((double)P.N / (double)P.N_global), P.colb3,
                                      P.cpa, P.nchunks * h->sm_count, P.cpc, P.nchunks * h->sm_count, P.dw0a, P.dw0c);
     ppo_metrics_kernel<<<1, 256, 0, s>>>(P.bsum, P.blocks_done, P.hp.inv_nglobal, (float)((double)P.N / (double)P.N_global), gr + nA + nC); TC_KCHECK(h);
     tc_reduce_cols_kernel<<<tc_nblk(g.A + 1, 8), 256, 0, s>>>(P.colb3, P.blocks_done, (size_t)(g.A + 1), g.A + 1, gr + g.ao.b3, g.A, gr + nA + g.co.b3); TC_KCHECK(h);
-    time_backward_kernel<<<1 + (g.H + 127) / 128, 512, sm, s>>>(w, g.ao, g.A, g.td, g.H, g.T, P.dw0a + (size_t)(g.A + g.Do) * g.H, d.sinemb, d.thpre, d.temb, gr);
+    CUDA_TRY(launch_time_backward(h, s, DPPO_NET_ACTOR_FT, P.dw0a + (size_t)(g.A + g.Do) * g.H, gr));
     TC_KCHECK(h);
     unpack_dw0_kernel<<<tc_nblk((size_t)(g.A + g.Do) * g.H, 256), 256, 0, s>>>(P.dw0a, g.A, g.td, g.Do, g.H, gr + g.ao.win); TC_KCHECK(h);
     unpack_dw0_kernel<<<tc_nblk((size_t)g.Do * g.Hc, 256), 256, 0, s>>>(P.dw0c + (size_t)g.A * g.Hc, 0, 0, g.Do, g.Hc, gr + nA + g.co.win); TC_KCHECK(h);
diff --git a/diffusionpolicyoptimization_b200/csrc/ts_path.cuh b/diffusionpolicyoptimization_b200/csrc/ts_path.cuh
--- a/diffusionpolicyoptimization_b200/csrc/ts_path.cuh
+++ b/diffusionpolicyoptimization_b200/csrc/ts_path.cuh
@@ -1082,14 +1082,16 @@
     int A, Do, T, H, NO, KP0, f16;
 };
 __global__ void __launch_bounds__(256) ts_fold_kernel(const TsFoldArgs f, const TsW F, float* __restrict__ bfold, const TsW B23) {
+    pdl_grid_begin();
     extern __shared__ float w3t[];
-    const int H = f.H, NO = f.NO, ld = f.H + f.KP0, HP = f.H + 1;
-    for (int i0 = threadIdx.x; i0 < H * NO; i0 += blockDim.x * 8) {
+    const int H = f.H, NO = f.NO, ld = f.H + f.KP0, HP = f.H + 1, a0 = 8 * blockIdx.y;
+    const int nq = min(8, NO - a0);
+    for (int i0 = threadIdx.x; i0 < H * 8; i0 += blockDim.x * 8) {
         float t8[8];
 #pragma unroll
-        for (int u = 0; u < 8; ++u) { const int i = i0 + u * blockDim.x; t8[u] = i < H * NO ? __ldg(f.w3 + i) : 0.f; }
-#pragma unroll
-        for (int u = 0; u < 8; ++u) { const int i = i0 + u * blockDim.x; if (i < H * NO) w3t[(size_t)(i % NO) * HP + i / NO] = t8[u]; }
+        for (int u = 0; u < 8; ++u) { const int i = i0 + u * blockDim.x; t8[u] = (i < H * 8 && i % 8 < nq) ? __ldg(f.w3 + (size_t)(i / 8) * NO + a0 + i % 8) : 0.f; }
+#pragma unroll
+        for (int u = 0; u < 8; ++u) { const int i = i0 + u * blockDim.x; if (i < H * 8) w3t[(size_t)(i % 8) * HP + i / 8] = t8[u]; }
     }
     __syncthreads();
     const int lane = threadIdx.x & 31, k = blockIdx.x * (blockDim.x >> 5) + (threadIdx.x >> 5);
@@ -1102,14 +1104,15 @@
         else if (k0 < f.A + f.Do) row = f.win + (size_t)(k0 - f.A + f.obs_skip) * H;
         else if (k0 < f.A + f.Do + f.T) { if (f.bt) row = f.bt + (size_t)(k0 - f.A - f.Do) * H; }
     } else { row = f.b2; bias_row = true; }
+    if (a0 >= NO) row = nullptr;
     float rv[32];
 #pragma unroll
     for (int q = 0; q < 32; ++q) {
         const int j = lane + 32 * q;
         rv[q] = (row && j < H) ? row[j] : 0.f;
-        if (bias_row && f.b0 && j < H) rv[q] += f.b0[j];
-    }
-    for (int a0 = 0; a0 < 64; a0 += 8) {
+        if (row && bias_row && f.b0 && j < H) rv[q] += f.b0[j];
+    }
+    {
         float acc[8];
 #pragma unroll
         for (int q = 0; q < 8; ++q) acc[q] = 0.f;
@@ -1119,7 +1122,7 @@
                 const int j = lane + 32 * qq;
                 if (j < H) {
 #pragma unroll
-                    for (int q = 0; q < 8; ++q) if (a0 + q < NO) acc[q] = fmaf(rv[qq], w3t[(size_t)(a0 + q) * HP + j], acc[q]);
+                    for (int q = 0; q < 8; ++q) if (a0 + q < NO) acc[q] = fmaf(rv[qq], w3t[(size_t)q * HP + j], acc[q]);
                 }
             }
 #pragma unroll
@@ -1183,6 +1186,118 @@
     if (net == DPPO_NET_CRITIC) ts_pack_critic_kernel<<<128, 256, 0, s>>>(h->net_w[net], g.co, g.A, g.Do, g.Hc, h->ts->KP0, w);
     else ts_pack_actor_kernel<<<256, 256, 0, s>>>(h->net_w[net], g.ao, g.A, g.td, g.Do, g.T, g.H, h->ts->KP0, h->ad[net].bt, w);
     TC_KCHECK(h);
+    return 0;
+}
+
+static int ts_ensure_fold(dppo_handle* h, int net, cudaStream_t s);
+struct TsUpdateArgs {
+    float* w; const float* g; float* m; float* v; size_t n, nA;
+    float lr, alpha, b1, b2, eps, wd; const int *skip0, *skip1;
+    ActorOff ao; CriticOff co; int A, td, Do, T, H, Hc, elem_blocks;
+    TsNetW wa, wc;
+    float *sinemb, *thpre, *temb, *bt; int* done;
+};
+__device__ __forceinline__ bool ts_update_time_param(const TsUpdateArgs& a, size_t i) {
+    const size_t wt0 = a.ao.win + (size_t)a.A * a.H, wt1 = wt0 + (size_t)a.td * a.H;
+    return i < a.ao.win || (i >= wt0 && i < wt1) || (i >= a.ao.bin && i < a.ao.bin + a.H);
+}
+__device__ __forceinline__ float ts_update_new(const TsUpdateArgs& a, size_t i, float* mo = nullptr, float* vo = nullptr) {
+    float p = a.w[i], mi = a.m[i], vi = a.v[i];
+    adamw_elem(p, mi, vi, a.g[i], a.lr, a.alpha, a.b1, a.b2, a.eps, a.wd);
+    if (mo) { *mo = mi; *vo = vi; }
+    return p;
+}
+__device__ __forceinline__ size_t ts_update_time_count(const TsUpdateArgs& a) { return a.ao.win + (size_t)(a.td + 1) * a.H; }
+__device__ __forceinline__ size_t ts_update_time_index(const TsUpdateArgs& a, size_t q) {
+    const size_t nmlp = a.ao.win, ntd = (size_t)a.td * a.H;
+    return q < nmlp ? q : (q < nmlp + ntd ? a.ao.win + (size_t)a.A * a.H + (q - nmlp) : a.ao.bin + (q - nmlp - ntd));
+}
+template <bool WRITE_BACK>
+__device__ __forceinline__ void ts_update_time_params(const TsUpdateArgs& a, float* sm) {
+    const size_t nq = ts_update_time_count(a);
+    for (size_t q0 = threadIdx.x; q0 < nq; q0 += 8 * (size_t)blockDim.x) {
+        float p[8], mi[8], vi[8], gi[8]; size_t idx[8];
+#pragma unroll
+        for (int u = 0; u < 8; ++u) {
+            const size_t q = q0 + (size_t)u * blockDim.x;
+            idx[u] = q < nq ? ts_update_time_index(a, q) : 0;
+            p[u] = a.w[idx[u]]; mi[u] = a.m[idx[u]]; vi[u] = a.v[idx[u]]; gi[u] = a.g[idx[u]];
+        }
+#pragma unroll
+        for (int u = 0; u < 8; ++u) {
+            const size_t q = q0 + (size_t)u * blockDim.x;
+            if (q >= nq) break;
+            adamw_elem(p[u], mi[u], vi[u], gi[u], a.lr, a.alpha, a.b1, a.b2, a.eps, a.wd);
+            if (WRITE_BACK) { a.w[idx[u]] = p[u]; a.m[idx[u]] = mi[u]; a.v[idx[u]] = vi[u]; }
+            else sm[q] = p[u];
+        }
+    }
+}
+struct WUpdated {
+    const TsUpdateArgs* a; const float* tp;
+    __device__ __forceinline__ float operator()(size_t i) const {
+        const size_t nmlp = a->ao.win, wt0 = a->ao.win + (size_t)a->A * a->H, ntd = (size_t)a->td * a->H;
+        return i < nmlp ? tp[i] : (i < a->ao.bin ? tp[nmlp + (i - wt0)] : tp[nmlp + ntd + (i - a->ao.bin)]);
+    }
+};
+__global__ void __launch_bounds__(512) ts_update_kernel(const TsUpdateArgs a) {
+    pdl_grid_begin();
+    if ((a.skip0 && *a.skip0) || (a.skip1 && *a.skip1)) return;
+    const int tid = threadIdx.x;
+    if ((int)blockIdx.x >= a.T) {
+        const size_t i = (size_t)(blockIdx.x - a.T) * blockDim.x + tid;
+        if (i >= a.n || (i < a.nA && ts_update_time_param(a, i))) return;
+        float mi, vi;
+        const float p = ts_update_new(a, i, &mi, &vi);
+        a.w[i] = p; a.m[i] = mi; a.v[i] = vi;
+        if (i < a.nA) {
+            const size_t H = a.H;
+            if (i >= a.ao.w1 && i < a.ao.w1 + H * H) ts_put2(a.wa.w1, a.wa.fw1, i - a.ao.w1, p);
+            else if (i >= a.ao.win && i < a.ao.win + (size_t)(a.A + a.td + a.Do) * H) {
+                const size_t r = (i - a.ao.win) / H, c = (i - a.ao.win) % H;
+                ts_put2(a.wa.w0, a.wa.fw0, (r < (size_t)a.A ? r : r - a.td) * H + c, p);
+            }
+        } else {
+            const size_t j = i - a.nA, Hc = a.Hc;
+            if (j >= a.co.w1 && j < a.co.w1 + Hc * Hc) ts_put2(a.wc.w1, a.wc.fw1, j - a.co.w1, p);
+            else if (j >= a.co.win && j < a.co.win + (size_t)a.Do * Hc) ts_put2(a.wc.w0, a.wc.fw0, (size_t)a.A * Hc + (j - a.co.win), p);
+        }
+        return;
+    }
+    const int t = blockIdx.x;
+    extern __shared__ float upd_sm[];
+    ts_update_time_params<false>(a, upd_sm);
+    __syncthreads();
+    actor_prep_body(t, upd_sm + ts_update_time_count(a), WUpdated{&a, upd_sm}, a.ao, a.A, a.td, a.H, a.sinemb, a.thpre, a.temb, a.bt, nullptr);
+    for (int c = tid; c < a.H; c += blockDim.x)
+        ts_put2(a.wa.w0, a.wa.fw0, (size_t)(a.A + a.Do + t) * a.H + c, a.bt[(size_t)t * a.H + c]);
+    __shared__ int last_flag;
+    __threadfence();
+    __syncthreads();
+    if (tid == 0) last_flag = (atomicAdd(a.done, 1) == a.T - 1) ? 1 : 0;
+    __syncthreads();
+    if (!last_flag) return;
+    ts_update_time_params<true>(a, nullptr);
+    if (tid == 0) *a.done = 0;
+}
+static size_t ts_update_smem(const Geom& g) { return (g.ao.win + (size_t)(g.td + 1) * g.H + 4 * (size_t)g.td) * sizeof(float); }
+static bool ts_update_ok(const dppo_handle* h) {
+    return h->cfg.precision == DPPO_PREC_BF16X3 && ts_shapes_ok(h) && 2 * h->g.td <= 512 && h->g.ao.tw1 == 0 && ts_update_smem(h->g) <= 48 * 1024;
+}
+static int ts_apply_update(dppo_handle* h, cudaStream_t s, const float* g, float lr, float alpha, float wd, const int* skip1) {
+    const Geom& gm = h->g; OptState& o = h->opt[DPPO_OPT_FINETUNE]; ActorDerived& d = h->ad[DPPO_NET_ACTOR_FT];
+    TsUpdateArgs a;
+    a.w = h->net_w[DPPO_NET_ACTOR_FT]; a.g = g; a.m = o.m; a.v = o.v; a.nA = gm.ao.n; a.n = gm.ao.n + gm.co.n;
+    a.lr = lr; a.alpha = alpha; a.b1 = h->cfg.adam_beta1; a.b2 = h->cfg.adam_beta2; a.eps = h->cfg.adam_eps; a.wd = wd;
+    a.skip0 = h->skip_update; a.skip1 = skip1;
+    a.ao = gm.ao; a.co = gm.co; a.A = gm.A; a.td = gm.td; a.Do = gm.Do; a.T = gm.T; a.H = gm.H; a.Hc = gm.Hc;
+    a.elem_blocks = tc_nblk(a.n, 512);
+    a.wa = h->ts->net[DPPO_NET_ACTOR_FT]; a.wc = h->ts->net[DPPO_NET_CRITIC];
+    a.sinemb = d.sinemb; a.thpre = d.thpre; a.temb = d.temb; a.bt = d.bt;
+    a.done = reinterpret_cast<int*>(d.dte + (size_t)gm.T * gm.td) + 1;
+    CUDA_TRY(launch_pdl(ts_update_kernel, dim3(a.elem_blocks + gm.T), dim3(512), ts_update_smem(gm), s, a)); TC_KCHECK(h);
+    for (int net : {DPPO_NET_ACTOR_FT, DPPO_NET_CRITIC}) { h->w0p_dirty[net] = 1; h->w23_dirty[net] = 1; h->ts->fold_dirty[net] = 1; }
+    DPPO_TRY(ts_ensure_fold(h, DPPO_NET_ACTOR_FT, s)); DPPO_TRY(ts_ensure_fold(h, DPPO_NET_CRITIC, s));
     return 0;
 }
 
@@ -1212,9 +1327,9 @@
     }
     static bool attr_set_dev[64] = {};
     if (!attr_set_dev[h->device & 63]) { CUDA_TRY(cudaFuncSetAttribute(ts_fold_kernel, cudaFuncAttributeMaxDynamicSharedMemorySize, 96 * 1024)); attr_set_dev[h->device & 63] = true; }
-    const size_t sm = (size_t)(f.H + 1) * f.NO * sizeof(float);
-    if (sm > 96 * 1024 || f.H > 1024) DPPO_FAIL(-7, "ts_ensure_fold: output layer too wide for the fold kernel");
-    ts_fold_kernel<<<tc_nblk((size_t)(f.H + f.KP0 + 1), 8), 256, sm, s>>>(f, W.ffold, W.bfold, W.w23p);
+    const size_t sm = (size_t)(f.H + 1) * 8 * sizeof(float);
+    if (sm > 96 * 1024 || f.H > 1024 || f.NO > 64) DPPO_FAIL(-7, "ts_ensure_fold: output layer too wide for the fold kernel");
+    CUDA_TRY(launch_pdl(ts_fold_kernel, dim3(tc_nblk((size_t)(f.H + f.KP0 + 1), 8), 8), dim3(256), sm, s, f, W.ffold, W.bfold, W.w23p));
     TC_KCHECK(h);
     h->ts->fold_dirty[net] = 0;
     return 0;
@@ -1460,6 +1575,7 @@
 }
 __global__ void __launch_bounds__(512) ts_dw3_assemble_kernel(const TsDw3Args fa, int blocks_a, const TsDw3Args fc, int blocks_c,
                                                               float* __restrict__ part, int* __restrict__ done, int rank_a, int rank_c, int phase) {
+    pdl_grid_begin();
     extern __shared__ float dw3_sm[];
     int b = blockIdx.x;
     if (phase == 1) {
@@ -1526,7 +1642,7 @@
     }
     int* done = reinterpret_cast<int*>(st->dw3_buf);
     float* partb = reinterpret_cast<float*>(st->dw3_buf + 1024);
-    ts_dw3_assemble_kernel<<<(phase == 1 ? nba + nbc : 0) + nra + nrc, 512, sm, s>>>(fa, nba, fc, nbc, partb, done, nra, nrc, phase);
+    CUDA_TRY(launch_pdl(ts_dw3_assemble_kernel, dim3((phase == 1 ? nba + nbc : 0) + nra + nrc), dim3(512), sm, s, fa, nba, fc, nbc, partb, done, nra, nrc, phase));
     TC_KCHECK(h);
     return 0;
 }
@@ -1675,9 +1791,7 @@
     DPPO_TRY(colsum(h, s, dval, 1, N, 1, nullptr, 1, part, gr + nA + g.co.b3));
     tc_reduce_cols_kernel<<<tc_nblk(2 * g.H, 8), 256, 0, s>>>(cpa, nrb, (size_t)2 * g.H, 2 * g.H, b2scr, g.H, gr + g.ao.b1); TC_KCHECK(h);
     tc_reduce_cols_kernel<<<tc_nblk(2 * g.Hc, 8), 256, 0, s>>>(cpc, nrb, (size_t)2 * g.Hc, 2 * g.Hc, b2scr + g.H, g.Hc, gr + nA + g.co.b1); TC_KCHECK(h);
-    const float* w = h->net_w[DPPO_NET_ACTOR_FT]; const ActorDerived& d = h->ad[DPPO_NET_ACTOR_FT];
-    const size_t sm = (size_t)(g.T * g.td * 3) * sizeof(float);
-    time_backward_kernel<<<1 + (g.H + 127) / 128, 512, sm, s>>>(w, g.ao, g.A, g.td, g.H, g.T, dw0a + (size_t)(g.A + g.Do) * g.H, d.sinemb, d.thpre, d.temb, gr); TC_KCHECK(h);
+    CUDA_TRY(launch_time_backward(h, s, DPPO_NET_ACTOR_FT, dw0a + (size_t)(g.A + g.Do) * g.H, gr)); TC_KCHECK(h);
     unpack_dw0_kernel<<<tc_nblk((size_t)(g.A + g.Do) * g.H, 256), 256, 0, s>>>(dw0a, g.A, g.td, g.Do, g.H, gr + g.ao.win); TC_KCHECK(h);
     unpack_dw0_kernel<<<tc_nblk((size_t)g.Do * g.Hc, 256), 256, 0, s>>>(dw0c + (size_t)g.A * g.Hc, 0, 0, g.Do, g.Hc, gr + nA + g.co.win); TC_KCHECK(h);
     CUDA_TRY(cudaMemcpyAsync(gr + nA + g.co.bin, dw0c + (size_t)(g.A + g.Do + g.T) * g.Hc, g.Hc * sizeof(float), cudaMemcpyDeviceToDevice, s));
@@ -1723,9 +1837,7 @@
     DPPO_TRY(ts_dw3_assemble(h, s, DPPO_NET_ACTOR, ga1, ga0, gr, dw0, nullptr, nullptr, nullptr, nullptr));
     tc_reduce_cols_kernel<<<tc_nblk(2 * g.H, 8), 256, 0, s>>>(cpa, nrb, (size_t)2 * g.H, 2 * g.H, ga1 + (size_t)(g.H + KP0) * 32, g.H, gr + g.ao.b1); TC_KCHECK(h);
     DPPO_TRY(colsum(h, s, deps, g.A, N, g.A, nullptr, 1, part, gr + g.ao.b3));
-    const float* w = h->net_w[DPPO_NET_ACTOR]; const ActorDerived& d = h->ad[DPPO_NET_ACTOR];
-    const size_t sm = (size_t)(g.T * g.td * 3) * sizeof(float);
-    time_backward_kernel<<<1 + (g.H + 127) / 128, 512, sm, s>>>(w, g.ao, g.A, g.td, g.H, g.T, dw0 + (size_t)(g.A + g.Do) * g.H, d.sinemb, d.thpre, d.temb, gr); TC_KCHECK(h);
+    CUDA_TRY(launch_time_backward(h, s, DPPO_NET_ACTOR, dw0 + (size_t)(g.A + g.Do) * g.H, gr)); TC_KCHECK(h);
     unpack_dw0_kernel<<<tc_nblk((size_t)(g.A + g.Do) * g.H, 256), 256, 0, s>>>(dw0, g.A, g.td, g.Do, g.H, gr + g.ao.win); TC_KCHECK(h);
     return 0;
 }
```

After: 76.89 million (median of 6 runs). 6.8% higher.
